# kdu3613/Multimodal_GAR

Hardware: AMD Instinct MI355X
Metric: clips/sec (fwd+bwd) at 32 actors x 16k pts x 15 frames (higher is better)
Workload: dtype f32; 1 GPU; c3: 8 clips x 15 frames x 32 actors x 16384 pts, 720x1280 RGB, fp32 fwd+bwd+Adam, LiDAR route pointnet2, GAT on; global_clips=8, clips_per_gpu=8, parallelism=dp1, launch=hip_graph, geometry=in step, gradient_exchange=none, trainable_params=29692332

## Files before the change

include/mgar_ops.h:

```cpp
#ifndef MGAR_OPS_H
#define MGAR_OPS_H

#ifdef __cplusplus
extern "C" {
#endif

#define MGAR_OK 0
#define MGAR_EINVAL (-1)
#define MGAR_ELAUNCH (-2)
#define MGAR_EUNSUPPORTED (-3)

#define MGAR_MAX_NSAMPLE 128

int mgar_abi_version(void);
const char *mgar_last_error(void);

int mgar_ktimer_enable(int on);
int mgar_ktimer_count(void);
const char *mgar_ktimer_name(int id);
int mgar_ktimer_read(int id, double *total_ms, long long *launches, double *total_bytes, double *total_flops,
                     int reset);
int mgar_ktimer_add_flops(int id, double flops);
int mgar_ktimer_add_bytes(int id, double bytes);


int mgar_ball_query_batch(int b, int n, int m, float radius, int nsample,
                          const float *new_xyz, const float *xyz, int *idx, void *stream);

int mgar_ball_query_multi_batch(int b, int n, int m, int nr, const float *radii, const int *nsamples,
                                const float *new_xyz, const float *xyz, int *const *idx, void *stream);
int mgar_ball_query_multi_stack(int B, int M, int nr, const float *radii, const int *nsamples, const float *new_xyz,
                                const int *new_xyz_batch_cnt, const float *xyz, const int *xyz_batch_cnt,
                                int *const *idx, void *stream);

int mgar_group_points_batch(int b, int c, int n, int npoints, int nsample,
                            const float *points, const int *idx, float *out, void *stream);
int mgar_group_points_grad_batch(int b, int c, int n, int npoints, int nsample,
                                 const float *grad_out, const int *idx, float *grad_points, void *stream);

int mgar_gather_points_batch(int b, int c, int n, int npoints,
                             const float *points, const int *idx, float *out, void *stream);
int mgar_gather_points_grad_batch(int b, int c, int n, int npoints,
                                  const float *grad_out, const int *idx, float *grad_points, void *stream);

int mgar_fps_batch(int b, int n, int m, const float *points, float *temp, int *idx, void *stream);

int mgar_morton_codes(int b, int n, const float *points, int *codes, void *stream);
int mgar_fps_batch_perm(int b, int n, int m, const float *points, float *temp, const int *perm, int *idx,
                        void *stream);
long long mgar_fps_batch_buckets_workspace_floats(int b, int n);
int mgar_fps_batch_buckets(int b, int n, int m, const float *points, float *temp, const int *perm, float *workspace, int *idx,
                           void *stream);

long long mgar_point_grid_workspace_bytes(int B, long long n_total);
int mgar_point_grid_build(int B, int n_batch, long long n_total, const float *xyz, const int *xyz_batch_cnt, float cell,
                          void *workspace, void *stream);
int mgar_ball_query_grid_batch(int b, int n, int m, float radius, int nsample, const float *new_xyz, const void *grid, int *idx,
                               void *stream);
int mgar_ball_query_grid_stack(int B, int M, long long n_total, float radius, int nsample, const float *new_xyz,
                               const int *new_xyz_batch_cnt, const void *grid, int *idx, void *stream);
int mgar_three_nn_grid_batch(int b, int n, int m, const float *unknown, const void *grid, float *dist2, int *idx, void *stream);
int mgar_three_nn_grid_stack(int B, int N, long long m_total, const float *unknown, const int *unknown_batch_cnt, const void *grid,
                             float *dist2, int *idx, void *stream);

int mgar_three_nn_batch(int b, int n, int m, const float *unknown, const float *known,
                        float *dist2, int *idx, void *stream);

int mgar_three_interpolate_batch(int b, int c, int m, int n, const float *points, const int *idx,
                                 const float *weight, float *out, void *stream);
int mgar_three_interpolate_grad_batch(int b, int c, int n, int m, const float *grad_out, const int *idx,
                                      const float *weight, float *grad_points, void *stream);

int mgar_three_interpolate_grad_sorted_batch(int b, int c, int n, int m, const float *grad_out, const int *list,
                                             float *grad_points, void *stream);
int mgar_three_interpolate_batch_into(int b, int c, int m, int n, const float *points, const int *idx, const float *weight,
                                      float *out, long long out_bstride, void *stream);
int mgar_three_interpolate_batch_add(int b, int c, int m, int n, const float *points, const int *idx, const float *weight,
                                     float *out, void *stream);
int mgar_three_interpolate_grad_batch_strided(int b, int c, int n, int m, const float *grad_out, long long grad_out_bstride,
                                              const int *idx, const float *weight, float *grad_points, void *stream);
int mgar_three_interpolate_grad_sorted_batch_strided(int b, int c, int n, int m, const float *grad_out,
                                                     long long grad_out_bstride, const int *list, float *grad_points,
                                                     void *stream);


int mgar_ball_query_stack(int B, int M, float radius, int nsample,
                          const float *new_xyz, const int *new_xyz_batch_cnt,
                          const float *xyz, const int *xyz_batch_cnt, int *idx, void *stream);

int mgar_voxel_query_stack(int M, int R1, int R2, int R3, int nsample, float radius,
                           int z_range, int y_range, int x_range,
                           const float *new_xyz, const float *xyz, const int *new_coords,
                           const int *point_indices, int *idx, void *stream);

int mgar_voxel_query_hash_stack(int M, int R1, int R2, int R3, int nsample, float radius,
                                int z_range, int y_range, int x_range,
                                const float *new_xyz, const float *xyz, const int *new_coords,
                                const long long *table_keys, const int *table_vals, int capacity, int *idx,
                                void *stream);

int mgar_fps_stack(int batch_size, int N, const float *points, float *temp, const int *xyz_batch_cnt,
                   int *idx, const int *num_sampled_points, void *stream);

int mgar_group_points_stack(int B, int M, int C, int nsample, const float *features,
                            const int *features_batch_cnt, const int *idx, const int *idx_batch_cnt,
                            float *out, void *stream);
int mgar_group_points_grad_stack(int B, int M, int C, int N, int nsample, const float *grad_out,
                                 const int *idx, const int *idx_batch_cnt, const int *features_batch_cnt,
                                 float *grad_features, void *stream);

int mgar_three_nn_stack(int batch_size, int N, int M, const float *unknown, const int *unknown_batch_cnt,
                        const float *known, const int *known_batch_cnt, float *dist2, int *idx, void *stream);

int mgar_three_interpolate_stack(int N, int C, const float *features, const int *idx, const float *weight,
                                 float *out, void *stream);
int mgar_three_interpolate_grad_stack(int N, int C, const float *grad_out, const int *idx, const float *weight,
                                      float *grad_features, void *stream);


int mgar_query_group_batch_fwd(int b, int c, int n, int npoints, int nsample, const float *xyz,
                               const float *new_xyz, const float *features, const int *idx, float *out,
                               void *stream);
int mgar_query_group_batch_bwd(int b, int c, int n, int npoints, int nsample, const float *grad_out,
                               const int *idx, float *grad_features, void *stream);

int mgar_query_group_stack_fwd(int B, int M, int C, int nsample, const float *xyz, const int *xyz_batch_cnt,
                               const float *new_xyz, const int *new_xyz_batch_cnt, const float *features,
                               const int *idx, float *out, void *stream);
int mgar_query_group_stack_bwd(int B, int M, int C, int nsample, const float *grad_out, const int *idx,
                               const int *new_xyz_batch_cnt, const int *xyz_batch_cnt, float *grad_features,
                               void *stream);

int mgar_query_group_proj_batch_fwd(int b, int c, int n, int npoints, int nsample, const float *xyz,
                                    const float *new_xyz, const float *zf, const float *wx, const int *idx,
                                    float *rel_out, float *y_out, void *stream);
int mgar_query_group_proj_batch_bwd(int b, int c, int n, int npoints, int nsample, const float *grad_y,
                                    const int *idx, float *grad_zf, void *stream);
int mgar_query_group_proj_stack_fwd(int B, int M, int C, int nsample, const float *xyz, const int *xyz_batch_cnt,
                                    const float *new_xyz, const int *new_xyz_batch_cnt, const float *zf, int zf_ld,
                                    const float *wx, const int *idx, float *rel_out, float *y_out, void *stream);
int mgar_query_group_proj_stack_fwd_stats(int B, int M, int C, int nsample, const float *xyz, const int *xyz_batch_cnt,
                                          const float *new_xyz, const int *new_xyz_batch_cnt, const float *zf, int zf_ld,
                                          const float *wx, const int *idx, float *rel_out, float *y_out, float *out_stats,
                                          void *stream);
int mgar_query_group_proj_stack_bwd(int B, int M, int C, int nsample, const float *grad_y, const int *idx,
                                    const int *new_xyz_batch_cnt, const int *xyz_batch_cnt, float *grad_zf,
                                    int zf_ld, void *stream);
long long mgar_query_group_stack_inverse_items(int B, int N, long long total);
long long mgar_query_group_stack_inverse_workspace_ints(int B, int N, long long total);
int mgar_query_group_stack_inverse_index(int B, int M, int nsample, int N, const int *idx, const int *new_xyz_batch_cnt,
                                         const int *xyz_batch_cnt, int *workspace, int *list, int *items, int *row_item,
                                         void *stream);
int mgar_query_group_stack_bwd_rows(int n_items, int N, int C, int nsample, const int *workspace, const int *items,
                                    const int *row_item, const int *list, const float *g_t, const float *xyz,
                                    const float *new_xyz, float *grad_zf, int zf_ld, float *part_rows, float *wx_part,
                                    long long total, void *stream);

int mgar_rowmajor_dw_workspace_floats(long long N, int Co, int Ci);
int mgar_rowmajor_dw(const float *a, int lda, const float *f, int ldf, long long N, int Co, int Ci,
                     float *workspace, float *dw, void *stream);


int mgar_bn_workspace_floats(int B, int C, int P);
int mgar_bn_train_stats(const float *x, int B, int C, int P, float eps, float momentum, float *workspace,
                        float *mean, float *invstd, float *running_mean, float *running_var,
                        long long *num_batches_tracked, void *stream);
int mgar_bn_train_stats_grouped(const float *x, int G, int C, int P, float eps, float momentum, float *workspace,
                                float *mean, float *invstd, float *running_mean, float *running_var,
                                long long *num_batches_tracked, void *stream);
int mgar_bn_act_fwd_grouped(const float *x, int G, int C, int P, const float *mean, const float *invstd,
                            const float *gamma, const float *beta, int relu, float *y, void *stream);
int mgar_bn_act_fwd(const float *x, int B, int C, int P, const float *mean, const float *invstd,
                    const float *gamma, const float *beta, int relu, float *y, void *stream);
long long mgar_bn_cl_workspace_floats(int S, int R, int C, int per_sample);
int mgar_bn_cl_train_stats(const float *x, int S, int R, int C, int per_sample, float eps, float momentum, float *workspace,
                           float *mean, float *invstd, float *running_mean, float *running_var,
                           long long *num_batches_tracked, void *stream);
int mgar_bn_cl_act_fwd(const float *x, int S, int R, int C, int per_sample, const float *mean, const float *invstd,
                       const float *gamma, const float *beta, int relu, float *y, int ldy, void *stream);
long long mgar_bn_rows_bwd_workspace_floats(int rows, int C);
int mgar_bn_rows_bwd(const float *dy, const float *x, int rows, int C, const float *mean, const float *invstd, const float *gamma,
                     const float *beta, int relu, float *workspace, float *dgamma, float *dbeta, float *dx, void *stream);
int mgar_bn_act_fwd_to_cl(const float *x, int S, int C, int R, int per_sample, const float *mean, const float *invstd,
                          const float *gamma, const float *beta, int relu, float *y, int ldy, void *stream);
int mgar_maxpool3d_same_fwd_cl(const float *x, int N, int T, int H, int W, int C, int kt, int kh, int kw, int st, int sh, int sw,
                               float *y, void *stream);
int mgar_bn_act_small(const float *x, int B, int C, int P, int per_sample, float eps, float momentum, const float *gamma,
                      const float *beta, int relu, float *workspace, float *mean, float *invstd, float *running_mean,
                      float *running_var, long long *num_batches_tracked, float *y, long long y_bstride, void *stream);
int mgar_bn_act_fwd_into(const float *x, int B, int C, int P, const float *mean, const float *invstd, const float *gamma,
                         const float *beta, int relu, int stats_per_sample, float *y, long long y_bstride, void *stream);
int mgar_bn_act_maxpool_fwd(const float *x, int B, int C, int M, int nsample, const float *mean,
                            const float *invstd, const float *gamma, const float *beta, int relu, float *out,
                            unsigned char *arg, float *xarg, void *stream);
int mgar_bn_act_bwd(const float *dy, const float *x, int B, int C, int P, const float *mean, const float *invstd,
                    const float *gamma, const float *beta, int relu, float *workspace, float *dgamma,
                    float *dbeta, float *dx, void *stream);
long long mgar_bn_stats_from_partials_workspace_floats(int nchunk, int C);
int mgar_bn_stats_from_partials(const float *partial, int nchunk, int C, long long n, int chunk, float eps, float momentum,
                                float *workspace, float *mean, float *invstd, float *running_mean, float *running_var,
                                long long *num_batches_tracked, void *stream);
int mgar_bn_act_maxpool_bwd_strided(const float *dpool, long long sb, long long sc, long long sm, const float *pooled,
                                    const unsigned char *arg, const float *x, const float *xarg, int B, int C, int M,
                                    int nsample, const float *mean, const float *invstd, const float *gamma, int relu,
                                    float *workspace, float *dgamma, float *dbeta, float *dx, void *stream);
int mgar_bn_act_bwd_apply(const float *dy, const float *x, int B, int C, int P, const float *mean, const float *invstd,
                          const float *gamma, const float *beta, int relu, const float *coef, int rowmajor, float *dx,
                          void *stream);
int mgar_bn_act_bwd_rowmajor(const float *dy, const float *x, int B, int C, int P, const float *mean, const float *invstd,
                             const float *gamma, const float *beta, int relu, float *workspace, float *dgamma,
                             float *dbeta, float *dx_t, void *stream);
int mgar_bn_act_maxpool_bwd(const float *dpool, const float *pooled, const unsigned char *arg, const float *x,
                            const float *xarg, int B, int C, int M, int nsample, const float *mean, const float *invstd,
                            const float *gamma, int relu, float *workspace, float *dgamma, float *dbeta,
                            float *dx, void *stream);

int mgar_pointwise_dw_workspace_floats(int B, int Cin, int Cout, int P);
int mgar_pointwise_conv_dw(const float *x, const float *dy, int B, int Cin, int Cout, int P, float *workspace,
                           float *dw, void *stream);

int mgar_pointwise_conv_dw_act(const float *x, const float *dy, int B, int Cin, int Cout, int P,
                               const float *in_mean, const float *in_invstd, const float *in_gamma,
                               const float *in_beta, int in_relu, float *workspace, float *dw, void *stream);

int mgar_pointwise_conv_fwd(const float *x, int B, int Cin, int P, const float *w, int w_row_stride,
                            int w_col_stride, int Cout, const float *in_mean, const float *in_invstd,
                            const float *in_gamma, const float *in_beta, int in_relu, float *y, void *stream);
int mgar_pointwise_dw_bnbwd_workspace_floats(int B, int Cin, int Cout, int P);
int mgar_pointwise_conv_dw_bnbwd(const float *x, const float *dy, const float *w, int B, int Cin, int Cout, int P,
                                 const float *in_mean, const float *in_invstd, const float *in_gamma, const float *in_beta,
                                 int in_relu, float *workspace, float *dw, float *dgamma, float *dbeta, float *coef, void *stream);
int mgar_pointwise_conv_fwd_stats(const float *x, int B, int Cin, int P, const float *w, int w_row_stride, int w_col_stride,
                                  int Cout, const float *in_mean, const float *in_invstd, const float *in_gamma,
                                  const float *in_beta, int in_relu, float *y, float *out_stats, void *stream);

int mgar_maxpool3d_same_fwd(const float *x, int NC, int T, int H, int W, int kt, int kh, int kw, int st, int sh,
                            int sw, float *y, void *stream);
int mgar_maxpool3d_valid_fwd(const float *x, int NC, int T, int H, int W, int kt, int kh, int kw, int st, int sh, int sw, float *y,
                             void *stream);

int mgar_stem_conv3d_workspace_floats(void);
int mgar_stem_conv3d_fwd(const float *x, int N, int T, int H, int W, const float *w, float *w_packed, float *y,
                         void *stream);
int mgar_stem_conv3d_set_minimal_filtering(int on);

long long mgar_conv3d_k3_workspace_floats(int Cin, int Cout);
int mgar_conv3d_k3_set_lds_pad(int bytes);
int mgar_conv3d_k3_fwd(const float *x, int N, int Cin, int D, int H, int W, const float *w, int Cout, float *w_packed, float *y,
                       void *stream);

int mgar_delay_us(int us, void *stream);


int mgar_roi_align_fwd(const float *input, int N, int C, int H, int W, const float *rois, int K,
                       int pooled_h, int pooled_w, float spatial_scale, int sampling_ratio, int aligned,
                       float *out, void *stream);
int mgar_roi_align_bwd(const float *grad_out, int N, int C, int H, int W, const float *rois, int K,
                       int pooled_h, int pooled_w, float spatial_scale, int sampling_ratio, int aligned,
                       float *grad_input, void *stream);

#define MGAR_DAFM_MAX_N 128
int mgar_dafm_attn_fwd(int S, int total_rows, int D, const int *scene_off, const int *de_off, const float *q, const float *k,
                       const float *v, const float *de, float sigma, float scale, float *att, float *out,
                       void *stream);
int mgar_dafm_attn_bwd(int S, int total_rows, int D, const int *scene_off, const int *de_off, const float *q, const float *k,
                       const float *v, const float *de, float sigma, float scale, const float *att,
                       const float *grad_out, float *gmat, float *grad_q, float *grad_k, float *grad_v,
                       void *stream);

int mgar_gatv2_fwd(int n_nodes, int H, int C, const int *rowptr, const int *col, const float *xl,
                   const float *xr, const float *att, float slope, const float *edge_scale, float *alpha,
                   float *out, void *stream);
int mgar_gatv2_bwd(int n_nodes, int H, int C, const int *rowptr, const int *col, const int *src_rowptr, const int *src_edge,
                   const int *src_dst, const float *xl, const float *xr, const float *att, float slope, const float *edge_scale,
                   const float *alpha, const float *grad_out, float *workspace, float *grad_xl, float *grad_xr, float *grad_att,
                   void *stream);
long long mgar_gatv2_bwd_workspace_floats(int n_nodes, int H, int C, int n_edges);

long long mgar_voxel_roi_pool_stats_workspace_doubles(int M, int nsample);
long long mgar_voxel_roi_pool_bwd_workspace_floats(int M, int C);
int mgar_voxel_roi_pool_stats(int M, int nsample, int C, const float *xyz, const float *new_xyz, const int *idx,
                              const float *w_pos, float eps, float momentum, double *workspace, double *moments,
                              float *mean, float *invstd, float *running_mean, float *running_var,
                              long long *num_batches_tracked, void *stream);
int mgar_voxel_roi_pool_fwd(int M, int nsample, int C, const float *xyz, const float *new_xyz, const float *feats,
                            int ld_f, const int *idx, const float *w_pos, const float *mean, const float *invstd,
                            const float *gamma, const float *beta, float *pooled, unsigned char *arg, void *stream);
int mgar_voxel_roi_pool_bwd(int M, int nsample, int C, const float *xyz, const float *new_xyz, const int *idx,
                            const float *w_pos, const float *mean, const float *invstd, const float *gamma,
                            const double *moments, int train_stats, const float *dpooled, const float *pooled,
                            const unsigned char *arg, float *workspace, float *dfeats, int ld_f, float *dgamma,
                            float *dbeta, float *dw_pos, void *stream);

int mgar_voxel_hash_build(int N, const int *coords, int Z, int Y, int X, long long *table_keys, int *table_vals,
                          int capacity, void *stream);
int mgar_voxel_hash_lookup(int M, const int *coords, int Z, int Y, int X, const long long *table_keys,
                           const int *table_vals, int capacity, int *rows, void *stream);
int mgar_spconv_rulebook(int n_sites, const int *site_coords, const int *geom, const long long *table_keys,
                         const int *table_vals, int capacity, int inverse, int *nbr, void *stream);
int mgar_spconv_output_keys(int n_in, const int *in_coords, const int *geom, long long *keys, void *stream);
int mgar_spconv_gather_gemm(int No, int K, int Cin, int Cout, const float *in, const int *nbr, const float *w,
                            int flip_k, float *out, void *stream);
int mgar_spconv_dw_chunks(int No);
int mgar_spconv_set_register_gather(int on);
int mgar_spconv_pair_chunk(void);
int mgar_spconv_pairs_blocks(int No);
int mgar_spconv_pairs_count(int No, int K, const int *nbr, int *blk, int *total, void *stream);
int mgar_spconv_pairs_fill(int No, int K, const int *nbr, const int *blk, const long long *offset_start, int *pair_i, int *pair_o,
                           void *stream);
int mgar_spconv_pairs_gemm(int K, int Cs, int Cd, const float *src, const int *pair_src, const int *pair_dst, const int *items,
                           const int *item_start_host, const float *w, float *dst, void *stream);
int mgar_spconv_pairs_dw(int n_items, int K, int Cin, int Cout, const float *in, const float *dout, const int *pair_i,
                         const int *pair_o, const int *items, const int *item_start, float *partial, float *dw, void *stream);
int mgar_spconv_dw(int No, int K, int Cin, int Cout, const float *in, const int *nbr, const float *dout,
                   float *partial, void *stream);

int mgar_points_in_boxes(int batch_size, int boxes_num, int pts_num, const float *boxes, const float *pts,
                         int *box_idx_of_points, void *stream);
int mgar_roipoint_pool3d_fwd(int batch_size, int pts_num, int boxes_num, int feature_in_len, int sampled_pts_num,
                             const float *xyz, const float *boxes3d, const float *pts_feature, float *pooled_features,
                             int *pooled_empty_flag, void *stream);

int mgar_image_resample_ksize(int in_size, int out_size);
int mgar_image_resample_coeffs(int in_size, int out_size, int *bounds, int *kk);
int mgar_image_resize_normalize_u8(int frames, int in_h, int in_w, int out_h, int out_w, const unsigned char *src,
                                   const int *xbounds, const int *xkk, const int *ybounds, const int *ykk, const float *lut,
                                   void *dst, long long dst_frame_stride, long long dst_channel_stride, int dst_kind,
                                   void *stream);
long long mgar_velodyne_merge_crop_workspace_ints(int n_upper, int n_lower);
int mgar_velodyne_merge_crop(int n_upper, int n_lower, int C, const float *upper, const float *lower, const float *tf_upper,
                             const float *tf_lower, const float *xy_range, int *workspace, float *out, int *count,
                             void *stream);

int mgar_query_group_batch_fwd_bf16(int b, int c, int n, int npoints, int nsample, const float *xyz, const float *new_xyz,
                                    const void *features, const int *idx, void *out, void *stream);
int mgar_query_group_stack_fwd_bf16(int B, int M, int C, int nsample, const float *xyz, const int *xyz_batch_cnt,
                                    const float *new_xyz, const int *new_xyz_batch_cnt, const void *features,
                                    const int *idx, void *out, void *stream);
int mgar_query_group_proj_batch_fwd_bf16(int b, int c, int n, int npoints, int nsample, const float *xyz,
                                         const float *new_xyz, const void *zf, const float *wx, const int *idx,
                                         void *rel_out, void *y_out, void *stream);
int mgar_query_group_proj_stack_fwd_bf16(int B, int M, int C, int nsample, const float *xyz, const int *xyz_batch_cnt,
                                         const float *new_xyz, const int *new_xyz_batch_cnt, const void *zf, int zf_ld,
                                         const float *wx, const int *idx, void *rel_out, void *y_out, void *stream);
int mgar_bn_train_stats_bf16(const void *x, int B, int C, int P, float eps, float momentum, float *workspace,
                             float *mean, float *invstd, float *running_mean, float *running_var,
                             long long *num_batches_tracked, void *stream);
int mgar_bn_train_stats_grouped_bf16(const void *x, int G, int C, int P, float eps, float momentum, float *workspace,
                                     float *mean, float *invstd, float *running_mean, float *running_var,
                                     long long *num_batches_tracked, void *stream);
int mgar_bn_act_fwd_bf16(const void *x, int B, int C, int P, const float *mean, const float *invstd,
                         const float *gamma, const float *beta, int relu, void *y, void *stream);
int mgar_three_interpolate_batch_into_bf16(int b, int c, int m, int n, const void *points, const int *idx, const float *weight,
                                           void *out, long long out_bstride, void *stream);
int mgar_three_interpolate_batch_add_bf16(int b, int c, int m, int n, const void *points, const int *idx, const float *weight,
                                          void *out, void *stream);
int mgar_bn_cl_train_stats_bf16(const void *x, int S, int R, int C, int per_sample, float eps, float momentum, float *workspace,
                                float *mean, float *invstd, float *running_mean, float *running_var,
                                long long *num_batches_tracked, void *stream);
int mgar_bn_cl_act_fwd_bf16(const void *x, int S, int R, int C, int per_sample, const float *mean, const float *invstd,
                            const float *gamma, const float *beta, int relu, void *y, int ldy, void *stream);
int mgar_bn_act_fwd_to_cl_bf16(const void *x, int S, int C, int R, int per_sample, const float *mean, const float *invstd,
                               const float *gamma, const float *beta, int relu, void *y, int ldy, void *stream);
int mgar_maxpool3d_same_fwd_cl_bf16(const void *x, int N, int T, int H, int W, int C, int kt, int kh, int kw, int st, int sh,
                                    int sw, void *y, void *stream);
int mgar_bn_act_small_bf16(const void *x, int B, int C, int P, int per_sample, float eps, float momentum, const float *gamma,
                           const float *beta, int relu, float *workspace, float *mean, float *invstd, float *running_mean,
                           float *running_var, long long *num_batches_tracked, void *y, long long y_bstride, void *stream);
int mgar_bn_act_fwd_into_bf16(const void *x, int B, int C, int P, const float *mean, const float *invstd, const float *gamma,
                              const float *beta, int relu, int stats_per_sample, void *y, long long y_bstride, void *stream);
int mgar_bn_act_fwd_grouped_bf16(const void *x, int G, int C, int P, const float *mean, const float *invstd,
                                 const float *gamma, const float *beta, int relu, void *y, void *stream);
int mgar_bn_act_maxpool_fwd_bf16(const void *x, int B, int C, int M, int nsample, const float *mean,
                                 const float *invstd, const float *gamma, const float *beta, int relu, void *out,
                                 unsigned char *arg, void *xarg, void *stream);
int mgar_bn_act_bwd_bf16(const void *dy, const void *x, int B, int C, int P, const float *mean, const float *invstd,
                         const float *gamma, const float *beta, int relu, float *workspace, float *dgamma,
                         float *dbeta, void *dx, void *stream);
int mgar_bn_act_maxpool_bwd_bf16(const void *dpool, const void *pooled, const unsigned char *arg, const void *x,
                                 const void *xarg, int B, int C, int M, int nsample, const float *mean, const float *invstd,
                                 const float *gamma, int relu, float *workspace, float *dgamma, float *dbeta,
                                 void *dx, void *stream);
int mgar_pointwise_conv_fwd_bf16(const void *x, int B, int Cin, int P, const float *w, int w_row_stride,
                                 int w_col_stride, int Cout, const float *in_mean, const float *in_invstd,
                                 const float *in_gamma, const float *in_beta, int in_relu, void *y, void *stream);
int mgar_three_interpolate_batch_bf16(int b, int c, int m, int n, const void *points, const int *idx,
                                      const float *weight, void *out, void *stream);
int mgar_three_interpolate_stack_bf16(int N, int C, const void *features, const int *idx, const float *weight,
                                      void *out, void *stream);
int mgar_maxpool3d_same_fwd_bf16(const void *x, int NC, int T, int H, int W, int kt, int kh, int kw, int st, int sh,
                                 int sw, void *y, void *stream);
int mgar_maxpool3d_valid_fwd_bf16(const void *x, int NC, int T, int H, int W, int kt, int kh, int kw, int st, int sh, int sw, void *y,
                                  void *stream);
int mgar_roi_align_fwd_bf16(const void *input, int N, int C, int H, int W, const float *rois, int K,
                            int pooled_h, int pooled_w, float spatial_scale, int sampling_ratio, int aligned,
                            void *out, void *stream);
int mgar_stem_conv3d_fwd_bf16(const void *x, int N, int T, int H, int W, const float *w, float *w_packed, void *y,
                              void *stream);
int mgar_voxel_roi_pool_fwd_bf16(int M, int nsample, int C, const float *xyz, const float *new_xyz, const void *feats,
                                 int ld_f, const int *idx, const float *w_pos, const float *mean, const float *invstd,
                                 const float *gamma, const float *beta, void *pooled, unsigned char *arg, void *stream);

#ifdef __cplusplus
}
#endif
#endif
```

multimodal_gar_amd/_lib.py:

```python
import ctypes
import os

import torch

_HERE = os.path.dirname(os.path.abspath(__file__))
LIB_PATH = os.path.join(_HERE, "csrc", "libmgar_hip.so")
ABI_VERSION = 12

if not os.path.exists(LIB_PATH):
    raise ImportError(
        "multimodal_gar_amd: %s is missing -- build it with `python -m multimodal_gar_amd.build` "
        "(hipcc --offload-arch=gfx950). There is no CPU fallback." % LIB_PATH)

_cdll = ctypes.CDLL(LIB_PATH)

_I, _F, _P, _LL = ctypes.c_int, ctypes.c_float, ctypes.c_void_p, ctypes.c_longlong

_PROTOS = {
    "mgar_ball_query_batch": [_I, _I, _I, _F, _I, _P, _P, _P, _P],
    "mgar_group_points_batch": [_I, _I, _I, _I, _I, _P, _P, _P, _P],
    "mgar_group_points_grad_batch": [_I, _I, _I, _I, _I, _P, _P, _P, _P],
    "mgar_gather_points_batch": [_I, _I, _I, _I, _P, _P, _P, _P],
    "mgar_gather_points_grad_batch": [_I, _I, _I, _I, _P, _P, _P, _P],
    "mgar_ball_query_multi_batch": [_I, _I, _I, _I, _P, _P, _P, _P, _P, _P],
    "mgar_ball_query_multi_stack": [_I, _I, _I, _P, _P, _P, _P, _P, _P, _P, _P],
    "mgar_fps_batch": [_I, _I, _I, _P, _P, _P, _P],
    "mgar_morton_codes": [_I, _I, _P, _P, _P],
    "mgar_fps_batch_perm": [_I, _I, _I, _P, _P, _P, _P, _P],
    "mgar_point_grid_workspace_bytes": [_I, ctypes.c_longlong],
    "mgar_point_grid_build": [_I, _I, ctypes.c_longlong, _P, _P, _F, _P, _P],
    "mgar_ball_query_grid_batch": [_I, _I, _I, _F, _I, _P, _P, _P, _P],
    "mgar_ball_query_grid_stack": [_I, _I, ctypes.c_longlong, _F, _I, _P, _P, _P, _P, _P],
    "mgar_three_nn_grid_batch": [_I, _I, _I, _P, _P, _P, _P, _P],
    "mgar_three_nn_grid_stack": [_I, _I, ctypes.c_longlong, _P, _P, _P, _P, _P, _P],
    "mgar_fps_batch_buckets": [_I, _I, _I, _P, _P, _P, _P, _P, _P],
    "mgar_fps_batch_buckets_workspace_floats": [_I, _I],
    "mgar_three_nn_batch": [_I, _I, _I, _P, _P, _P, _P, _P],
    "mgar_three_interpolate_batch": [_I, _I, _I, _I, _P, _P, _P, _P, _P],
    "mgar_three_interpolate_batch_add": [_I, _I, _I, _I, _P, _P, _P, _P, _P],
    "mgar_three_interpolate_grad_batch": [_I, _I, _I, _I, _P, _P, _P, _P, _P],
    "mgar_three_interpolate_grad_sorted_batch": [_I, _I, _I, _I, _P, _P, _P, _P],
    "mgar_three_interpolate_batch_into": [_I, _I, _I, _I, _P, _P, _P, _P, _LL, _P],
    "mgar_three_interpolate_grad_batch_strided": [_I, _I, _I, _I, _P, _LL, _P, _P, _P, _P],
    "mgar_three_interpolate_grad_sorted_batch_strided": [_I, _I, _I, _I, _P, _LL, _P, _P, _P],
    "mgar_ball_query_stack": [_I, _I, _F, _I, _P, _P, _P, _P, _P, _P],
    "mgar_voxel_query_stack": [_I, _I, _I, _I, _I, _F, _I, _I, _I, _P, _P, _P, _P, _P, _P],
    "mgar_voxel_query_hash_stack": [_I, _I, _I, _I, _I, _F, _I, _I, _I, _P, _P, _P, _P, _P, _I, _P, _P],
    "mgar_fps_stack": [_I, _I, _P, _P, _P, _P, _P, _P],
    "mgar_group_points_stack": [_I, _I, _I, _I, _P, _P, _P, _P, _P, _P],
    "mgar_group_points_grad_stack": [_I, _I, _I, _I, _I, _P, _P, _P, _P, _P, _P],
    "mgar_three_nn_stack": [_I, _I, _I, _P, _P, _P, _P, _P, _P, _P],
    "mgar_three_interpolate_stack": [_I, _I, _P, _P, _P, _P, _P],
    "mgar_three_interpolate_grad_stack": [_I, _I, _P, _P, _P, _P, _P],
    "mgar_query_group_batch_fwd": [_I, _I, _I, _I, _I, _P, _P, _P, _P, _P, _P],
    "mgar_query_group_batch_bwd": [_I, _I, _I, _I, _I, _P, _P, _P, _P],
    "mgar_query_group_stack_fwd": [_I, _I, _I, _I, _P, _P, _P, _P, _P, _P, _P, _P],
    "mgar_query_group_stack_bwd": [_I, _I, _I, _I, _P, _P, _P, _P, _P, _P],
    "mgar_query_group_proj_batch_fwd": [_I, _I, _I, _I, _I, _P, _P, _P, _P, _P, _P, _P, _P],
    "mgar_query_group_proj_batch_bwd": [_I, _I, _I, _I, _I, _P, _P, _P, _P],
    "mgar_query_group_proj_stack_fwd": [_I, _I, _I, _I, _P, _P, _P, _P, _P, _I, _P, _P, _P, _P, _P],
    "mgar_query_group_proj_stack_bwd": [_I, _I, _I, _I, _P, _P, _P, _P, _P, _I, _P],
    "mgar_rowmajor_dw_workspace_floats": [_LL, _I, _I],
    "mgar_ktimer_enable": [_I],
    "mgar_ktimer_count": [],
    "mgar_ktimer_add_flops": [_I, ctypes.c_double],
    "mgar_ktimer_add_bytes": [_I, ctypes.c_double],
    "mgar_ktimer_read": [_I, _P, _P, _P, _P, _I],
    "mgar_rowmajor_dw": [_P, _I, _P, _I, _LL, _I, _I, _P, _P, _P],
    "mgar_bn_workspace_floats": [_I, _I, _I],
    "mgar_bn_train_stats": [_P, _I, _I, _I, _F, _F, _P, _P, _P, _P, _P, _P, _P],
    "mgar_bn_train_stats_grouped": [_P, _I, _I, _I, _F, _F, _P, _P, _P, _P, _P, _P, _P],
    "mgar_bn_act_fwd_grouped": [_P, _I, _I, _I, _P, _P, _P, _P, _I, _P, _P],
    "mgar_bn_act_fwd": [_P, _I, _I, _I, _P, _P, _P, _P, _I, _P, _P],
    "mgar_bn_act_maxpool_fwd": [_P, _I, _I, _I, _I, _P, _P, _P, _P, _I, _P, _P, _P, _P],
    "mgar_bn_act_bwd": [_P, _P, _I, _I, _I, _P, _P, _P, _P, _I, _P, _P, _P, _P, _P],
    "mgar_bn_stats_from_partials_workspace_floats": [_I, _I],
    "mgar_bn_stats_from_partials": [_P, _I, _I, _LL, _I, _F, _F, _P, _P, _P, _P, _P, _P, _P],
    "mgar_pointwise_conv_fwd_stats": [_P, _I, _I, _I, _P, _I, _I, _I, _P, _P, _P, _P, _I, _P, _P, _P],
    "mgar_query_group_proj_stack_fwd_stats": [_I, _I, _I, _I, _P, _P, _P, _P, _P, _I, _P, _P, _P, _P, _P, _P],
    "mgar_bn_act_maxpool_bwd_strided": [_P, _LL, _LL, _LL, _P, _P, _P, _P, _I, _I, _I, _I, _P, _P, _P, _I, _P, _P, _P, _P, _P],
    "mgar_bn_cl_workspace_floats": [_I, _I, _I, _I],
    "mgar_bn_cl_train_stats": [_P, _I, _I, _I, _I, _F, _F, _P, _P, _P, _P, _P, _P, _P],
    "mgar_bn_cl_act_fwd": [_P, _I, _I, _I, _I, _P, _P, _P, _P, _I, _P, _I, _P],
    "mgar_bn_rows_bwd_workspace_floats": [_I, _I],
    "mgar_bn_rows_bwd": [_P, _P, _I, _I, _P, _P, _P, _P, _I, _P, _P, _P, _P, _P],
    "mgar_bn_act_fwd_to_cl": [_P, _I, _I, _I, _I, _P, _P, _P, _P, _I, _P, _I, _P],
    "mgar_maxpool3d_same_fwd_cl": [_P, _I, _I, _I, _I, _I, _I, _I, _I, _I, _I, _I, _P, _P],
    "mgar_bn_act_small": [_P, _I, _I, _I, _I, _F, _F, _P, _P, _I, _P, _P, _P, _P, _P, _P, _P, _LL, _P],
    "mgar_bn_act_fwd_into": [_P, _I, _I, _I, _P, _P, _P, _P, _I, _I, _P, _LL, _P],
    "mgar_bn_act_bwd_rowmajor": [_P, _P, _I, _I, _I, _P, _P, _P, _P, _I, _P, _P, _P, _P, _P],
    "mgar_query_group_stack_inverse_items": [_I, _I, _LL],
    "mgar_query_group_stack_inverse_workspace_ints": [_I, _I, _LL],
    "mgar_query_group_stack_inverse_index": [_I, _I, _I, _I, _P, _P, _P, _P, _P, _P, _P, _P],
    "mgar_query_group_stack_bwd_rows": [_I, _I, _I, _I, _P, _P, _P, _P, _P, _P, _P, _P, _I, _P, _P, _LL, _P],
    "mgar_bn_act_maxpool_bwd": [_P, _P, _P, _P, _P, _I, _I, _I, _I, _P, _P, _P, _I, _P, _P, _P, _P, _P],
    "mgar_pointwise_conv_dw": [_P, _P, _I, _I, _I, _I, _P, _P, _P],
    "mgar_pointwise_dw_workspace_floats": [_I, _I, _I, _I],
    "mgar_pointwise_dw_bnbwd_workspace_floats": [_I, _I, _I, _I],
    "mgar_pointwise_conv_dw_bnbwd": [_P, _P, _P, _I, _I, _I, _I, _P, _P, _P, _P, _I, _P, _P, _P, _P, _P, _P],
    "mgar_bn_act_bwd_apply": [_P, _P, _I, _I, _I, _P, _P, _P, _P, _I, _P, _I, _P, _P],
    "mgar_pointwise_conv_dw_act": [_P, _P, _I, _I, _I, _I, _P, _P, _P, _P, _I, _P, _P, _P],
    "mgar_pointwise_conv_fwd": [_P, _I, _I, _I, _P, _I, _I, _I, _P, _P, _P, _P, _I, _P, _P],
    "mgar_stem_conv3d_workspace_floats": [],
    "mgar_stem_conv3d_set_minimal_filtering": [_I],
    "mgar_stem_conv3d_fwd": [_P, _I, _I, _I, _I, _P, _P, _P, _P],
    "mgar_delay_us": [_I, _P],
    "mgar_conv3d_k3_workspace_floats": [_I, _I],
    "mgar_conv3d_k3_set_lds_pad": [_I],
    "mgar_conv3d_k3_fwd": [_P, _I, _I, _I, _I, _I, _P, _I, _P, _P, _P],
    "mgar_maxpool3d_same_fwd": [_P, _I, _I, _I, _I, _I, _I, _I, _I, _I, _I, _P, _P],
    "mgar_maxpool3d_valid_fwd": [_P, _I, _I, _I, _I, _I, _I, _I, _I, _I, _I, _P, _P],
    "mgar_roi_align_fwd": [_P, _I, _I, _I, _I, _P, _I, _I, _I, _F, _I, _I, _P, _P],
    "mgar_roi_align_bwd": [_P, _I, _I, _I, _I, _P, _I, _I, _I, _F, _I, _I, _P, _P],
    "mgar_dafm_attn_fwd": [_I, _I, _I, _P, _P, _P, _P, _P, _P, _F, _F, _P, _P, _P],
    "mgar_dafm_attn_bwd": [_I, _I, _I, _P, _P, _P, _P, _P, _P, _F, _F, _P, _P, _P, _P, _P, _P, _P],
    "mgar_gatv2_fwd": [_I, _I, _I, _P, _P, _P, _P, _P, _F, _P, _P, _P, _P],
    "mgar_gatv2_bwd": [_I, _I, _I, _P, _P, _P, _P, _P, _P, _P, _P, _F, _P, _P, _P, _P, _P, _P, _P, _P],
    "mgar_gatv2_bwd_workspace_floats": [_I, _I, _I, _I],
    "mgar_points_in_boxes": [_I, _I, _I, _P, _P, _P, _P],
    "mgar_roipoint_pool3d_fwd": [_I, _I, _I, _I, _I, _P, _P, _P, _P, _P, _P],
    "mgar_image_resample_ksize": [_I, _I],
    "mgar_image_resample_coeffs": [_I, _I, _P, _P],
    "mgar_image_resize_normalize_u8": [_I, _I, _I, _I, _I, _P, _P, _P, _P, _P, _P, _P, _LL, _LL, _I, _P],
    "mgar_velodyne_merge_crop_workspace_ints": [_I, _I],
    "mgar_velodyne_merge_crop": [_I, _I, _I, _P, _P, _P, _P, _P, _P, _P, _P, _P],
    "mgar_voxel_hash_build": [_I, _P, _I, _I, _I, _P, _P, _I, _P],
    "mgar_voxel_hash_lookup": [_I, _P, _I, _I, _I, _P, _P, _I, _P, _P],
    "mgar_spconv_rulebook": [_I, _P, _P, _P, _P, _I, _I, _P, _P],
    "mgar_spconv_output_keys": [_I, _P, _P, _P, _P],
    "mgar_spconv_gather_gemm": [_I, _I, _I, _I, _P, _P, _P, _I, _P, _P],
    "mgar_spconv_dw_chunks": [_I],
    "mgar_spconv_pair_chunk": [],
    "mgar_spconv_set_register_gather": [_I],
    "mgar_spconv_pairs_blocks": [_I],
    "mgar_spconv_pairs_count": [_I, _I, _P, _P, _P, _P],
    "mgar_spconv_pairs_fill": [_I, _I, _P, _P, _P, _P, _P, _P],
    "mgar_spconv_pairs_gemm": [_I, _I, _I, _P, _P, _P, _P, _P, _P, _P, _P],
    "mgar_spconv_pairs_dw": [_I, _I, _I, _I, _P, _P, _P, _P, _P, _P, _P, _P, _P],
    "mgar_spconv_dw": [_I, _I, _I, _I, _P, _P, _P, _P, _P],
    "mgar_voxel_roi_pool_stats_workspace_doubles": [_I, _I],
    "mgar_voxel_roi_pool_bwd_workspace_floats": [_I, _I],
    "mgar_voxel_roi_pool_stats": [_I, _I, _I, _P, _P, _P, _P, _F, _F, _P, _P, _P, _P, _P, _P, _P, _P],
    "mgar_voxel_roi_pool_fwd": [_I, _I, _I, _P, _P, _P, _I, _P, _P, _P, _P, _P, _P, _P, _P, _P],
    "mgar_voxel_roi_pool_bwd": [_I, _I, _I, _P, _P, _P, _P, _P, _P, _P, _P, _I, _P, _P, _P, _P, _P, _I, _P, _P, _P, _P],
}
for _n in ("mgar_query_group_batch_fwd", "mgar_query_group_stack_fwd", "mgar_query_group_proj_batch_fwd",
           "mgar_query_group_proj_stack_fwd", "mgar_bn_train_stats", "mgar_bn_train_stats_grouped", "mgar_bn_act_fwd",
           "mgar_bn_act_fwd_grouped", "mgar_bn_act_fwd_into", "mgar_bn_act_small", "mgar_bn_cl_train_stats", "mgar_bn_cl_act_fwd", "mgar_bn_act_fwd_to_cl",
           "mgar_maxpool3d_same_fwd_cl", "mgar_bn_act_maxpool_fwd", "mgar_bn_act_bwd", "mgar_bn_act_maxpool_bwd",
           "mgar_pointwise_conv_fwd", "mgar_three_interpolate_batch", "mgar_three_interpolate_batch_into", "mgar_three_interpolate_batch_add", "mgar_three_interpolate_stack",
           "mgar_maxpool3d_same_fwd", "mgar_maxpool3d_valid_fwd", "mgar_roi_align_fwd", "mgar_voxel_roi_pool_fwd", "mgar_stem_conv3d_fwd"):
    _PROTOS[_n + "_bf16"] = _PROTOS[_n]
BF16_TWINS = frozenset(n[:-5] for n in _PROTOS if n.endswith("_bf16"))

_LONGLONG_RESULTS = frozenset((
    "mgar_query_group_stack_inverse_items", "mgar_query_group_stack_inverse_workspace_ints", "mgar_bn_cl_workspace_floats",
    "mgar_bn_stats_from_partials_workspace_floats", "mgar_voxel_roi_pool_stats_workspace_doubles",
    "mgar_voxel_roi_pool_bwd_workspace_floats", "mgar_velodyne_merge_crop_workspace_ints", "mgar_gatv2_bwd_workspace_floats",
    "mgar_fps_batch_buckets_workspace_floats", "mgar_point_grid_workspace_bytes",
    "mgar_bn_rows_bwd_workspace_floats", "mgar_conv3d_k3_workspace_floats"))

_fns = {}
for _name, _args in _PROTOS.items():
    _fn = getattr(_cdll, _name)
    _fn.argtypes = _args
    _fn.restype = ctypes.c_longlong if _name in _LONGLONG_RESULTS else ctypes.c_int
    _fns[_name] = _fn

_cdll.mgar_abi_version.restype = ctypes.c_int
_cdll.mgar_last_error.restype = ctypes.c_char_p
if _cdll.mgar_abi_version() != ABI_VERSION:
    raise ImportError("libmgar_hip.so ABI %d != expected %d: rebuild" % (_cdll.mgar_abi_version(), ABI_VERSION))


class MgarError(RuntimeError):
    pass


def dev_ptr(t, dtype=None):
    if t is None:
        return None
    if not t.is_cuda:
        raise MgarError("expected a device (HIP) tensor, got %s -- there is no CPU path" % t.device)
    if not t.is_contiguous():
        raise MgarError("tensor must be contiguous")
    if dtype is not None and t.dtype != dtype:
        raise MgarError("expected dtype %s, got %s" % (dtype, t.dtype))
    return t.data_ptr()


def fptr(t):
    return dev_ptr(t, torch.float32)


def pptr(t, dtype):
    return dev_ptr(t, dtype)


def payload_call(name, dtype, *args):
    if dtype == torch.float32:
        return call(name, *args)
    if dtype == torch.bfloat16 and name in BF16_TWINS:
        return call(name + "_bf16", *args)
    raise MgarError("%s: unsupported payload dtype %s" % (name, dtype))


def iptr(t):
    return dev_ptr(t, torch.int32)


def stream_of(t):
    return torch.cuda.current_stream(t.device).cuda_stream


def raw(name, *args):
    return _fns[name](*args)


def call(name, *args):
    rc = _fns[name](*args)
    if rc != 0:
        raise MgarError("%s failed with code %d: %s" % (name, rc, _cdll.mgar_last_error().decode()))
    return rc


def host_arrays(radii, nsamples, idx_tensors):
    n = len(radii)
    fa = (ctypes.c_float * n)(*[float(r) for r in radii])
    ia = (ctypes.c_int * n)(*[int(s) for s in nsamples])
    pa = (ctypes.c_void_p * n)(*[iptr(t) for t in idx_tensors])
    return fa, ia, pa


def kernel_timers(enable=None, reset=True):
    if enable is not None:
        call("mgar_ktimer_enable", int(bool(enable)))
        _KT_STATE["on"] = bool(enable)
        return None
    _cdll.mgar_ktimer_name.restype = ctypes.c_char_p
    _cdll.mgar_ktimer_name.argtypes = [ctypes.c_int]
    out = {}
    for i in range(raw("mgar_ktimer_count")):
        ms, by, fl, n = ctypes.c_double(), ctypes.c_double(), ctypes.c_double(), ctypes.c_longlong()
        call("mgar_ktimer_read", i, ctypes.byref(ms), ctypes.byref(n), ctypes.byref(by), ctypes.byref(fl), int(reset))
        if n.value:
            out[_cdll.mgar_ktimer_name(i).decode()] = (ms.value, n.value, by.value, fl.value)
    return out


_KT_IDS = {}


_KT_STATE = {"on": False}


def note_work(kernel, flops=0.0, nbytes=0.0):
    if not _KT_STATE["on"]:
        return
    if not _KT_IDS:
        _cdll.mgar_ktimer_name.restype = ctypes.c_char_p
        _cdll.mgar_ktimer_name.argtypes = [ctypes.c_int]
        for i in range(raw("mgar_ktimer_count")):
            _KT_IDS[_cdll.mgar_ktimer_name(i).decode()] = i
    if flops:
        call("mgar_ktimer_add_flops", _KT_IDS[kernel], float(flops))
    if nbytes:
        call("mgar_ktimer_add_bytes", _KT_IDS[kernel], float(nbytes))


def kernel_timing_on():
    return _KT_STATE["on"]


def note_pair_tests(kernel, pairs):
    note_work(kernel, flops=float(pairs) * 8.0)


def exported_symbols():
    return sorted(_PROTOS) + ["mgar_abi_version", "mgar_last_error", "mgar_ktimer_name"]
```

multimodal_gar_amd/bn_ops.py:

```python
import torch
import torch.nn as nn
from torch.autograd import Function
from torch.autograd.function import once_differentiable

from . import _lib as L


def _u8ptr(t):
    return L.dev_ptr(t, torch.uint8)


def _workspace(x, b, c, p):
    return torch.empty((L.raw("mgar_bn_workspace_floats", b, c, p),), dtype=torch.float32, device=x.device)


_PAYLOADS = (torch.float32, torch.bfloat16)


def _f32(t):
    return t if t is None or t.dtype == torch.float32 else t.float()


STATS_TILE = 128


def stats_partial_buffer(x_like, c, n_per_channel):
    if x_like.dtype != torch.float32 or not x_like.is_cuda or n_per_channel % STATS_TILE != 0 or n_per_channel == 0:
        return None
    return torch.empty((c, n_per_channel // STATS_TILE, 2), dtype=torch.float32, device=x_like.device)


def _train_stats(x3, bn, partial=None):
    b, c, p = x3.shape
    mean = torch.empty((c,), dtype=torch.float32, device=x3.device)
    invstd = torch.empty_like(mean)
    track = bn.track_running_stats and bn.running_mean is not None
    if partial is not None and tuple(partial.shape) == (c, (b * p) // STATS_TILE, 2) and (b * p) % STATS_TILE == 0:
        nws = L.raw("mgar_bn_stats_from_partials_workspace_floats", partial.shape[1], c)
        ws = torch.empty((nws,), dtype=torch.float32, device=x3.device) if nws else None
        L.call("mgar_bn_stats_from_partials", L.fptr(partial), partial.shape[1], c, b * p, STATS_TILE, float(bn.eps),
               float(bn.momentum if bn.momentum is not None else 0.1), L.fptr(ws) if ws is not None else None, L.fptr(mean), L.fptr(invstd),
               L.fptr(bn.running_mean) if track else None, L.fptr(bn.running_var) if track else None,
               L.dev_ptr(bn.num_batches_tracked, torch.int64) if track and bn.num_batches_tracked is not None else None,
               L.stream_of(x3))
        return mean, invstd
    ws = _workspace(x3, b, c, p)
    L.payload_call("mgar_bn_train_stats", x3.dtype, L.pptr(x3, x3.dtype), b, c, p, float(bn.eps),
                   float(bn.momentum if bn.momentum is not None else 0.1),
                   L.fptr(ws), L.fptr(mean), L.fptr(invstd), L.fptr(bn.running_mean) if track else None,
                   L.fptr(bn.running_var) if track else None,
                   L.dev_ptr(bn.num_batches_tracked, torch.int64) if track and bn.num_batches_tracked is not None else None,
                   L.stream_of(x3))
    return mean, invstd


ROWMAJOR_GRAD_MAX_CHANNELS = 64


def _bwd_rowmajor(dy, x3, mean, invstd, gamma, beta, relu, ws, dgamma, dbeta):
    b, c, p = x3.shape
    dx_t = torch.empty((b, p, c), dtype=torch.float32, device=x3.device)
    L.call("mgar_bn_act_bwd_rowmajor", L.fptr(dy), L.fptr(x3), b, c, p, L.fptr(mean), L.fptr(invstd), L.fptr(gamma), L.fptr(beta),
           int(relu), L.fptr(ws), L.fptr(dgamma), L.fptr(dbeta), L.fptr(dx_t), L.stream_of(x3))
    return dx_t.permute(0, 2, 1)


class _BnAct(Function):

    @staticmethod
    def forward(ctx, x3, gamma, beta, mean, invstd, relu, rowmajor_grad=False):
        b, c, p = x3.shape
        ctx.rowmajor = bool(rowmajor_grad) and x3.dtype == torch.float32 and c <= ROWMAJOR_GRAD_MAX_CHANNELS
        y = torch.empty_like(x3)
        dt = x3.dtype
        L.payload_call("mgar_bn_act_fwd", dt, L.pptr(x3, dt), b, c, p, L.fptr(mean), L.fptr(invstd), L.fptr(gamma), L.fptr(beta),
                       int(relu), L.pptr(y, dt), L.stream_of(x3))
        ctx.save_for_backward(x3, gamma, beta, mean, invstd)
        ctx.relu = bool(relu)
        return y

    @staticmethod
    @once_differentiable
    def backward(ctx, dy):
        x3, gamma, beta, mean, invstd = ctx.saved_tensors
        b, c, p = x3.shape
        dgamma, dbeta = torch.empty_like(gamma), torch.empty_like(beta)
        dt = x3.dtype
        dy_c, ws = dy.contiguous().to(dt), _workspace(x3, b, c, p)
        if ctx.rowmajor:
            return _bwd_rowmajor(dy_c, x3, mean, invstd, gamma, beta, ctx.relu, ws, dgamma, dbeta), dgamma, dbeta, None, None, None, None
        dx = torch.empty_like(x3)
        L.payload_call("mgar_bn_act_bwd", dt, L.pptr(dy_c, dt), L.pptr(x3, dt), b, c, p, L.fptr(mean), L.fptr(invstd), L.fptr(gamma),
                       L.fptr(beta), int(ctx.relu), L.fptr(ws), L.fptr(dgamma), L.fptr(dbeta), L.pptr(dx, dt), L.stream_of(x3))
        return dx, dgamma, dbeta, None, None, None, None


class _BnActMaxPool(Function):

    @staticmethod
    def forward(ctx, x4, gamma, beta, mean, invstd, relu):
        b, c, m, ns = x4.shape
        dt = x4.dtype
        out = torch.empty((b, c, m), dtype=dt, device=x4.device)
        arg = torch.empty((b, c, m), dtype=torch.uint8, device=x4.device)
        xarg = torch.empty((b, c, m), dtype=dt, device=x4.device) if x4.requires_grad or gamma.requires_grad else None
        L.payload_call("mgar_bn_act_maxpool_fwd", dt, L.pptr(x4, dt), b, c, m, ns, L.fptr(mean), L.fptr(invstd), L.fptr(gamma),
                       L.fptr(beta), int(relu), L.pptr(out, dt), _u8ptr(arg), L.pptr(xarg, dt) if xarg is not None else None,
                       L.stream_of(x4))
        ctx.save_for_backward(x4, gamma, mean, invstd, out, arg, xarg)
        ctx.relu = bool(relu)
        ctx.mark_non_differentiable(arg)
        return out, arg

    @staticmethod
    @once_differentiable
    def backward(ctx, dpool, darg=None):
        x4, gamma, mean, invstd, out, arg, xarg = ctx.saved_tensors
        b, c, m, ns = x4.shape
        dx = torch.empty_like(x4)
        dgamma, dbeta = torch.empty_like(gamma), torch.empty_like(gamma)
        dt = x4.dtype
        ws = _workspace(x4, b, c, m * ns)
        if dt == torch.float32 and dpool.dtype == dt and dpool.dim() == 3 and not dpool.is_contiguous() \
                and (b == 1 or dpool.stride(0) >= 0) and min(dpool.stride(1), dpool.stride(2)) >= 1:
            L.call("mgar_bn_act_maxpool_bwd_strided", dpool.data_ptr(), dpool.stride(0) if b > 1 else 0, dpool.stride(1), dpool.stride(2),
                   L.fptr(out), _u8ptr(arg), L.fptr(x4), L.fptr(xarg) if xarg is not None else None, b, c, m, ns, L.fptr(mean),
                   L.fptr(invstd), L.fptr(gamma), int(ctx.relu), L.fptr(ws), L.fptr(dgamma), L.fptr(dbeta), L.fptr(dx), L.stream_of(x4))
            return dx, dgamma, dbeta, None, None, None
        dpool_c = dpool.contiguous().to(dt)
        L.payload_call("mgar_bn_act_maxpool_bwd", dt, L.pptr(dpool_c, dt), L.pptr(out, dt), _u8ptr(arg), L.pptr(x4, dt),
                       L.pptr(xarg, dt) if xarg is not None else None, b, c, m, ns, L.fptr(mean), L.fptr(invstd), L.fptr(gamma),
                       int(ctx.relu), L.fptr(ws), L.fptr(dgamma), L.fptr(dbeta), L.pptr(dx, dt), L.stream_of(x4))
        return dx, dgamma, dbeta, None, None, None


class _BnActConv(Function):

    @staticmethod
    def forward(ctx, x3, gamma, beta, mean, invstd, relu, w, rowmajor_grad=False, out_stats=None):
        b, c, p = x3.shape
        ctx.rowmajor = bool(rowmajor_grad) and x3.dtype == torch.float32 and c <= ROWMAJOR_GRAD_MAX_CHANNELS
        cout = w.shape[0]
        w = w.contiguous()
        dt = x3.dtype
        y = torch.empty((b, cout, p), dtype=dt, device=x3.device)
        if out_stats is not None:
            L.call("mgar_pointwise_conv_fwd_stats", L.fptr(x3), b, c, p, L.fptr(w), c, 1, cout, L.fptr(mean), L.fptr(invstd),
                   L.fptr(gamma), L.fptr(beta), int(relu), L.fptr(y), L.fptr(out_stats), L.stream_of(x3))
        else:
            L.payload_call("mgar_pointwise_conv_fwd", dt, L.pptr(x3, dt), b, c, p, L.fptr(w), c, 1, cout, L.fptr(mean), L.fptr(invstd),
                           L.fptr(gamma), L.fptr(beta), int(relu), L.pptr(y, dt), L.stream_of(x3))
        ctx.save_for_backward(x3, gamma, beta, mean, invstd, w)
        ctx.relu = relu
        return y

    @staticmethod
    @once_differentiable
    def backward(ctx, gy):
        x3, gamma, beta, mean, invstd, w = ctx.saved_tensors
        b, c, p = x3.shape
        cout = w.shape[0]
        gy = gy.contiguous()
        st = L.stream_of(x3)
        ga = torch.empty_like(x3)
        L.call("mgar_pointwise_conv_fwd", L.fptr(gy), b, cout, p, L.fptr(w), 1, c, c, None, None, None, None, 0,
               L.fptr(ga), st)
        dgamma, dbeta = torch.empty_like(gamma), torch.empty_like(gamma)
        if FUSED_DW_BN_REDUCE and ctx.needs_input_grad[6]:
            dw = torch.empty_like(w)
            coef = torch.empty((2 * c,), dtype=torch.float32, device=x3.device)
            wsd = torch.empty((max(1, L.raw("mgar_pointwise_dw_bnbwd_workspace_floats", b, c, cout, p)),), dtype=torch.float32,
                              device=x3.device)
            L.call("mgar_pointwise_conv_dw_bnbwd", L.fptr(x3), L.fptr(gy), L.fptr(w), b, c, cout, p, L.fptr(mean), L.fptr(invstd),
                   L.fptr(gamma), L.fptr(beta), int(ctx.relu), L.fptr(wsd), L.fptr(dw), L.fptr(dgamma), L.fptr(dbeta), L.fptr(coef), st)
            dx = torch.empty((b, p, c) if ctx.rowmajor else (b, c, p), dtype=torch.float32, device=x3.device)
            L.call("mgar_bn_act_bwd_apply", L.fptr(ga), L.fptr(x3), b, c, p, L.fptr(mean), L.fptr(invstd), L.fptr(gamma), L.fptr(beta),
                   int(ctx.relu), L.fptr(coef), int(ctx.rowmajor), L.fptr(dx), st)
            return (dx.permute(0, 2, 1) if ctx.rowmajor else dx), dgamma, dbeta, None, None, None, dw, None, None
        dw = None
        if ctx.needs_input_grad[6]:
            dw = torch.empty_like(w)
            wsd = torch.empty((max(1, L.raw("mgar_pointwise_dw_workspace_floats", b, c, cout, p)),), dtype=torch.float32,
                              device=x3.device)
            L.call("mgar_pointwise_conv_dw_act", L.fptr(x3), L.fptr(gy), b, c, cout, p, L.fptr(mean), L.fptr(invstd),
                   L.fptr(gamma), L.fptr(beta), int(ctx.relu), L.fptr(wsd), L.fptr(dw), st)
        ws = _workspace(x3, b, c, p)
        if ctx.rowmajor:
            return _bwd_rowmajor(ga, x3, mean, invstd, gamma, beta, ctx.relu, ws, dgamma, dbeta), dgamma, dbeta, None, None, None, dw, None, None
        dx = torch.empty_like(x3)
        L.call("mgar_bn_act_bwd", L.fptr(ga), L.fptr(x3), b, c, p, L.fptr(mean), L.fptr(invstd), L.fptr(gamma),
               L.fptr(beta), int(ctx.relu), L.fptr(ws), L.fptr(dgamma), L.fptr(dbeta), L.fptr(dx), st)
        return dx, dgamma, dbeta, None, None, None, dw, None, None


class _PlainConv(Function):

    @staticmethod
    def forward(ctx, x3, w, out_stats=None):
        b, c, p = x3.shape
        cout = w.shape[0]
        w = w.contiguous()
        dt = x3.dtype
        y = torch.empty((b, cout, p), dtype=dt, device=x3.device)
        if out_stats is not None:
            L.call("mgar_pointwise_conv_fwd_stats", L.fptr(x3), b, c, p, L.fptr(w), c, 1, cout, None, None, None, None, 0,
                   L.fptr(y), L.fptr(out_stats), L.stream_of(x3))
        else:
            L.payload_call("mgar_pointwise_conv_fwd", dt, L.pptr(x3, dt), b, c, p, L.fptr(w), c, 1, cout, None, None, None, None, 0,
                           L.pptr(y, dt), L.stream_of(x3))
        ctx.save_for_backward(x3, w)
        return y

    @staticmethod
    @once_differentiable
    def backward(ctx, gy):
        x3, w = ctx.saved_tensors
        b, c, p = x3.shape
        cout = w.shape[0]
        gy = gy.contiguous()
        dx = dw = None
        if ctx.needs_input_grad[0]:
            dx = torch.empty_like(x3)
            L.call("mgar_pointwise_conv_fwd", L.fptr(gy), b, cout, p, L.fptr(w), 1, c, c, None, None, None, None, 0, L.fptr(dx),
                   L.stream_of(x3))
        if ctx.needs_input_grad[1]:
            dw = torch.empty_like(w)
            wsd = torch.empty((max(1, L.raw("mgar_pointwise_dw_workspace_floats", b, c, cout, p)),), dtype=torch.float32,
                              device=x3.device)
            L.call("mgar_pointwise_conv_dw", L.fptr(x3), L.fptr(gy), b, c, cout, p, L.fptr(wsd), L.fptr(dw), L.stream_of(x3))
        return dx, dw, None


PLAIN_CONV_MAX_OUT = 32
PLAIN_CONV_MAX_IN = 32


def plain_conv(x, conv, want_out_stats=False):
    if not (x.is_cuda and x.dtype in _PAYLOADS and x.dim() >= 3 and conv.bias is None):
        return None
    if x.dtype != torch.float32 and torch.is_grad_enabled() and (x.requires_grad or conv.weight.requires_grad):
        return None
    c, cout = x.shape[1], conv.out_channels
    x3 = x.contiguous().flatten(2)
    if c > PLAIN_CONV_MAX_IN or cout > PLAIN_CONV_MAX_OUT or x3.shape[2] % 4 != 0 or x3.shape[0] * x3.shape[2] < (1 << 16):
        return None
    out_stats = stats_partial_buffer(x3, cout, x3.shape[0] * x3.shape[2]) if want_out_stats and x3.shape[2] % STATS_TILE == 0 else None
    y = _PlainConv.apply(x3, _f32(conv.weight).view(cout, c), out_stats).view(x.shape[0], cout, *x.shape[2:])
    return (y, out_stats) if want_out_stats else y


FUSED_DW_BN_REDUCE = False
FUSED_CONV_MAX_CHANNELS = 64


FUSED_STATS_MAX_CHANNELS = 32


def bn_act_conv(x, bn, relu, conv, rowmajor_grad=False, in_stats=None, want_out_stats=False):
    if not (x.is_cuda and x.dtype in _PAYLOADS and bn.training and x.dim() >= 3 and conv.bias is None):
        return None
    if x.dtype != torch.float32 and torch.is_grad_enabled() and (x.requires_grad or conv.weight.requires_grad):
        return None
    c, cout = x.shape[1], conv.out_channels
    x3 = x.contiguous().flatten(2)
    if c > FUSED_CONV_MAX_CHANNELS or cout > FUSED_CONV_MAX_CHANNELS or x3.shape[2] % 4 != 0 \
            or x3.shape[0] * x3.shape[2] < (1 << 16):
        return None
    mean, invstd = _stats(x3, bn, in_stats)
    gamma, beta = _affine(bn, c, x.device)
    out_stats = stats_partial_buffer(x3, cout, x3.shape[0] * x3.shape[2]) \
        if want_out_stats and cout <= FUSED_STATS_MAX_CHANNELS and x3.shape[2] % STATS_TILE == 0 else None
    y = _BnActConv.apply(x3, gamma, beta, mean, invstd, relu, _f32(conv.weight).view(cout, c), rowmajor_grad, out_stats)
    y = y.view(x.shape[0], cout, *x.shape[2:])
    return (y, out_stats) if want_out_stats else y


def _affine(bn, c, device):
    if bn.affine:
        return _f32(bn.weight), _f32(bn.bias)
    return torch.ones(c, device=device), torch.zeros(c, device=device)


def _stats(x3, bn, partial=None):
    if bn.training or not bn.track_running_stats:
        return _train_stats(x3, bn, partial)
    return _f32(bn.running_mean), torch.rsqrt(_f32(bn.running_var) + bn.eps)


def _slice_stride(out, x):
    if out is None or out.shape != x.shape or out.dtype != x.dtype or not out.is_cuda:
        return None
    inner = 1
    for size, stride in zip(reversed(out.shape[1:]), reversed(out.stride()[1:])):
        if size != 1 and stride != inner:
            return None
        inner *= size
    return out.stride(0) if out.stride(0) >= inner else None


def is_channels_last_3d(x):
    return x.dim() == 5 and not x.is_contiguous() and x.is_contiguous(memory_format=torch.channels_last_3d)


def _cl_out_slice(out, x):
    if out is None or out.shape != x.shape or out.dtype != x.dtype or not out.is_cuda:
        return None
    n, c, t, h, w = out.shape
    ld = out.stride(4)
    ok = out.stride(1) == 1 and ld >= c and out.stride(3) == w * ld and out.stride(2) == h * w * ld and out.stride(0) == t * h * w * ld
    return ld if ok and ld % 4 == 0 and (out.data_ptr() // out.element_size()) % 4 == 0 else None


def _cl_stats(x, bn, per_sample):
    n, c, t, h, w = x.shape
    r = t * h * w
    rows = n * c if per_sample else c
    mean = torch.empty((rows,), dtype=torch.float32, device=x.device)
    invstd = torch.empty_like(mean)
    ws = torch.empty((max(L.raw("mgar_bn_cl_workspace_floats", n, r, c, int(per_sample)), 1),), dtype=torch.float32, device=x.device)
    track = bn.track_running_stats and bn.running_mean is not None
    L.payload_call("mgar_bn_cl_train_stats", x.dtype, x.data_ptr(), n, r, c, int(per_sample), float(bn.eps),
                   float(bn.momentum if bn.momentum is not None else 0.1), L.fptr(ws), L.fptr(mean), L.fptr(invstd),
                   L.fptr(bn.running_mean) if track else None, L.fptr(bn.running_var) if track else None,
                   L.dev_ptr(bn.num_batches_tracked, torch.int64) if track and bn.num_batches_tracked is not None else None,
                   L.stream_of(x))
    return mean, invstd


def bn_act_channels_last(x, bn, relu, per_sample, out=None):
    n, c, t, h, w = x.shape
    if c % 4 != 0 or c > 1024 or x.dtype not in _PAYLOADS or (per_sample and n * c > 65535) or not bn.training:
        return None
    mean, invstd = _cl_stats(x, bn, per_sample)
    gamma, beta = _affine(bn, c, x.device)
    ld = _cl_out_slice(out, x)
    y = out if ld is not None else torch.empty_like(x)
    L.payload_call("mgar_bn_cl_act_fwd", x.dtype, x.data_ptr(), n, t * h * w, c, int(per_sample), L.fptr(mean), L.fptr(invstd),
                   L.fptr(gamma), L.fptr(beta), int(relu), y.data_ptr(), ld if ld is not None else c, L.stream_of(x))
    return y


def bn_act_to_channels_last(x, bn, relu, per_sample):
    x = x.contiguous()
    n, c, t, h, w = x.shape
    if x.dtype not in _PAYLOADS or not bn.training or (per_sample and n * c > 65535):
        return None
    x3 = x.flatten(2)
    if per_sample:
        mean = torch.empty((n * c,), dtype=torch.float32, device=x.device)
        invstd = torch.empty_like(mean)
        track = bn.track_running_stats and bn.running_mean is not None
        ws = _workspace(x3, 1, n * c, x3.shape[2])
        L.payload_call("mgar_bn_train_stats_grouped", x.dtype, L.pptr(x3, x.dtype), n, c, x3.shape[2], float(bn.eps),
                       float(bn.momentum if bn.momentum is not None else 0.1), L.fptr(ws), L.fptr(mean), L.fptr(invstd),
                       L.fptr(bn.running_mean) if track else None, L.fptr(bn.running_var) if track else None,
                       L.dev_ptr(bn.num_batches_tracked, torch.int64) if track and bn.num_batches_tracked is not None else None,
                       L.stream_of(x))
    else:
        mean, invstd = _train_stats(x3, bn)
    gamma, beta = _affine(bn, c, x.device)
    y = torch.empty(x.shape, dtype=x.dtype, device=x.device, memory_format=torch.channels_last_3d)
    L.payload_call("mgar_bn_act_fwd_to_cl", x.dtype, L.pptr(x3, x.dtype), n, c, t * h * w, int(per_sample), L.fptr(mean), L.fptr(invstd),
                   L.fptr(gamma), L.fptr(beta), int(relu), y.data_ptr(), c, L.stream_of(x))
    return y


class _BnActRows(Function):

    @staticmethod
    def forward(ctx, x, gamma, beta, mean, invstd, relu):
        rows, c = x.shape
        y = torch.empty_like(x)
        L.call("mgar_bn_cl_act_fwd", L.fptr(x), 1, rows, c, 0, L.fptr(mean), L.fptr(invstd), L.fptr(gamma), L.fptr(beta), int(relu),
               L.fptr(y), c, L.stream_of(x))
        ctx.save_for_backward(x, gamma, beta, mean, invstd)
        ctx.relu = bool(relu)
        return y

    @staticmethod
    @once_differentiable
    def backward(ctx, dy):
        x, gamma, beta, mean, invstd = ctx.saved_tensors
        rows, c = x.shape
        dy = dy.contiguous()
        dx, dgamma, dbeta = torch.empty_like(x), torch.empty_like(gamma), torch.empty_like(gamma)
        ws = torch.empty((L.raw("mgar_bn_rows_bwd_workspace_floats", rows, c),), dtype=torch.float32, device=x.device)
        L.call("mgar_bn_rows_bwd", L.fptr(dy), L.fptr(x), rows, c, L.fptr(mean), L.fptr(invstd), L.fptr(gamma), L.fptr(beta),
               int(ctx.relu), L.fptr(ws), L.fptr(dgamma), L.fptr(dbeta), L.fptr(dx), L.stream_of(x))
        return dx, dgamma, dbeta, None, None, None


def bn_act_rows(x, bn, relu):
    if not (x.is_cuda and x.dim() == 2 and x.dtype == torch.float32 and bn.training and x.shape[1] % 4 == 0 and x.shape[1] <= 1024
            and x.shape[0] > 0):
        return None
    x = x.contiguous()
    rows, c = x.shape
    mean = torch.empty((c,), dtype=torch.float32, device=x.device)
    invstd = torch.empty_like(mean)
    ws = torch.empty((max(L.raw("mgar_bn_cl_workspace_floats", 1, rows, c, 0), 1),), dtype=torch.float32, device=x.device)
    track = bn.track_running_stats and bn.running_mean is not None
    L.call("mgar_bn_cl_train_stats", L.fptr(x), 1, rows, c, 0, float(bn.eps), float(bn.momentum if bn.momentum is not None else 0.1),
           L.fptr(ws), L.fptr(mean), L.fptr(invstd), L.fptr(bn.running_mean) if track else None, L.fptr(bn.running_var) if track else None,
           L.dev_ptr(bn.num_batches_tracked, torch.int64) if track and bn.num_batches_tracked is not None else None, L.stream_of(x))
    gamma, beta = _affine(bn, c, x.device)
    return _BnActRows.apply(x, gamma, beta, mean, invstd, relu)


SMALL_CHANNEL_MAX = 16384


def _small_fused(x, x3, bn, relu, per_sample, out):
    b, c, p = x3.shape
    if (p if per_sample else b * p) > SMALL_CHANNEL_MAX or p % 4 != 0 or x3.dtype not in _PAYLOADS:
        return None
    bstride = _slice_stride(out, x)
    y = out if bstride is not None else torch.empty_like(x)
    track = bn.track_running_stats and bn.running_mean is not None
    rows = b * c if per_sample else c
    need = per_sample and track
    mean = torch.empty((rows,), dtype=torch.float32, device=x.device) if need else None
    ws = torch.empty((rows,), dtype=torch.float32, device=x.device) if need else None
    gamma, beta = _affine(bn, c, x.device)
    dt = x3.dtype
    L.payload_call("mgar_bn_act_small", dt, L.pptr(x3, dt), b, c, p, int(per_sample), float(bn.eps),
                   float(bn.momentum if bn.momentum is not None else 0.1), L.fptr(gamma), L.fptr(beta), int(relu),
                   L.fptr(ws) if ws is not None else None, L.fptr(mean) if mean is not None else None, None,
                   L.fptr(bn.running_mean) if track else None, L.fptr(bn.running_var) if track else None,
                   L.dev_ptr(bn.num_batches_tracked, torch.int64) if track and bn.num_batches_tracked is not None else None,
                   y.data_ptr(), bstride if bstride is not None else -1, L.stream_of(x3))
    return y


def _apply_into(x3, bn, relu, mean, invstd, per_sample, out, bstride):
    b, c, p = x3.shape
    gamma, beta = _affine(bn, c, x3.device)
    dt = x3.dtype
    L.payload_call("mgar_bn_act_fwd_into", dt, L.pptr(x3, dt), b, c, p, L.fptr(mean), L.fptr(invstd), L.fptr(gamma), L.fptr(beta),
                   int(relu), int(per_sample), out.data_ptr(), bstride, L.stream_of(x3))
    return out


def bn_act(x, bn, relu, rowmajor_grad=False, out=None, in_stats=None, to_channels_last=False):
    if x.is_cuda and x.dim() == 5 and not (torch.is_grad_enabled() and (x.requires_grad or (bn.affine and bn.weight.requires_grad))):
        y = bn_act_channels_last(x, bn, relu, False, out) if is_channels_last_3d(x) else \
            (bn_act_to_channels_last(x, bn, relu, False) if to_channels_last else None)
        if y is not None:
            return y
    x3 = x.contiguous().flatten(2) if x.dim() > 2 else x.contiguous().unsqueeze(-1)
    if not bn.training and torch.is_grad_enabled() and x.requires_grad:
        return None
    forward_only = not (torch.is_grad_enabled() and (x.requires_grad or (bn.affine and bn.weight.requires_grad)))
    if forward_only and bn.training and x.is_cuda and in_stats is None:
        y = _small_fused(x, x3, bn, relu, False, out)
        if y is not None:
            return y
    mean, invstd = _stats(x3, bn, in_stats)
    bstride = _slice_stride(out, x)
    if bstride is not None and x.dtype in _PAYLOADS and not (torch.is_grad_enabled() and (x.requires_grad or bn.weight.requires_grad)):
        return _apply_into(x3, bn, relu, mean, invstd, False, out, bstride)
    gamma, beta = _affine(bn, x3.shape[1], x.device)
    return _BnAct.apply(x3, gamma, beta, mean, invstd, relu, rowmajor_grad).view(x.shape)


def bn_act_per_sample(x, bn, relu, out=None, to_channels_last=False):
    if not (x.is_cuda and x.dtype in _PAYLOADS and bn.training and x.dim() >= 3) or (torch.is_grad_enabled() and
                                                                                        (x.requires_grad or bn.weight.requires_grad)):
        return None
    if x.dim() == 5:
        y = bn_act_channels_last(x, bn, relu, True, out) if is_channels_last_3d(x) else \
            (bn_act_to_channels_last(x, bn, relu, True) if to_channels_last else None)
        if y is not None:
            return y
    x3 = x.contiguous().flatten(2)
    g, c, p = x3.shape
    if g * c > 65535:
        return None
    y = _small_fused(x, x3, bn, relu, True, out)
    if y is not None:
        return y
    mean = torch.empty((g * c,), dtype=torch.float32, device=x.device)
    invstd = torch.empty_like(mean)
    track = bn.track_running_stats and bn.running_mean is not None
    ws = _workspace(x3, 1, g * c, p)
    st = L.stream_of(x3)
    dt = x3.dtype
    L.payload_call("mgar_bn_train_stats_grouped", dt, L.pptr(x3, dt), g, c, p, float(bn.eps),
                   float(bn.momentum if bn.momentum is not None else 0.1),
                   L.fptr(ws), L.fptr(mean), L.fptr(invstd), L.fptr(bn.running_mean) if track else None,
                   L.fptr(bn.running_var) if track else None,
                   L.dev_ptr(bn.num_batches_tracked, torch.int64) if track and bn.num_batches_tracked is not None else None, st)
    bstride = _slice_stride(out, x)
    if bstride is not None:
        return _apply_into(x3, bn, relu, mean, invstd, True, out, bstride)
    gamma, beta = _affine(bn, c, x.device)
    y = torch.empty_like(x3)
    L.payload_call("mgar_bn_act_fwd_grouped", dt, L.pptr(x3, dt), g, c, p, L.fptr(mean), L.fptr(invstd), L.fptr(gamma), L.fptr(beta),
                   int(relu), L.pptr(y, dt), st)
    return y.view(x.shape)


def bn_train_stats_only(x, bn, per_sample=False):
    x3 = x.contiguous().flatten(2)
    g, c, p = x3.shape
    if not per_sample:
        return _train_stats(x3, bn)
    if g * c > 65535:
        return None
    mean = torch.empty((g * c,), dtype=torch.float32, device=x.device)
    invstd = torch.empty_like(mean)
    track = bn.track_running_stats and bn.running_mean is not None
    ws = _workspace(x3, 1, g * c, p)
    dt = x3.dtype
    L.payload_call("mgar_bn_train_stats_grouped", dt, L.pptr(x3, dt), g, c, p, float(bn.eps),
                   float(bn.momentum if bn.momentum is not None else 0.1),
                   L.fptr(ws), L.fptr(mean), L.fptr(invstd), L.fptr(bn.running_mean) if track else None,
                   L.fptr(bn.running_var) if track else None,
                   L.dev_ptr(bn.num_batches_tracked, torch.int64) if track and bn.num_batches_tracked is not None else None, L.stream_of(x3))
    return mean, invstd


def bn_apply_with_stats(x, bn, relu, stats, per_sample=False):
    mean, invstd = stats
    x3 = x.contiguous().flatten(2)
    g, c, p = x3.shape
    gamma, beta = _affine(bn, c, x.device)
    y = torch.empty_like(x3)
    dt = x3.dtype
    if per_sample:
        L.payload_call("mgar_bn_act_fwd_grouped", dt, L.pptr(x3, dt), g, c, p, L.fptr(mean), L.fptr(invstd), L.fptr(gamma), L.fptr(beta),
                       int(relu), L.pptr(y, dt), L.stream_of(x3))
    else:
        L.payload_call("mgar_bn_act_fwd", dt, L.pptr(x3, dt), g, c, p, L.fptr(mean), L.fptr(invstd), L.fptr(gamma), L.fptr(beta),
                       int(relu), L.pptr(y, dt), L.stream_of(x3))
    return y.view(x.shape)


def bn_act_maxpool(x, bn, relu, in_stats=None):
    x4 = x.contiguous()
    if x4.shape[-1] > 255 or (not bn.training and torch.is_grad_enabled() and x.requires_grad):
        return None
    mean, invstd = _stats(x4.flatten(2), bn, in_stats)
    gamma, beta = _affine(bn, x4.shape[1], x.device)
    return _BnActMaxPool.apply(x4, gamma, beta, mean, invstd, relu)[0]
```

multimodal_gar_amd/csrc/bn_act.hip:

```cpp
#include "common.hpp"
#include "payload.hpp"

namespace mgar {

constexpr int BN_THREADS = 256;
constexpr int BN_CHUNK = 65536;

__device__ __forceinline__ float block_sum(float v, float *scratch) {
    v = wave_sum(v);
    const int lane = threadIdx.x & 63, w = threadIdx.x >> 6;
    __syncthreads();
    if (lane == 0) scratch[w] = v;
    __syncthreads();
    float t = 0.f;
    for (int i = 0; i < BN_THREADS / 64; ++i) t += scratch[i];
    return t;
}

__device__ __forceinline__ size_t chan_off(long long e, int c, int C, int P) {
    const long long b = e / P;
    return ((size_t)b * C + c) * P + (size_t)(e - b * P);
}

template <typename T>
__global__ __launch_bounds__(BN_THREADS) void bn_partial_kernel(const T *__restrict__ x, int B, int C, int P, int chunk,
                                                                float *__restrict__ partial) {
    __shared__ float scratch[BN_THREADS / 64];
    const int c = blockIdx.y;
    const long long n = (long long)B * P;
    const long long e0 = (long long)blockIdx.x * chunk;
    const long long e1 = min(e0 + chunk, n);
    const long long npiv = min((long long)BN_THREADS, e1 - e0);
    float pv = threadIdx.x < npiv ? Payload<T>::ld(x + chan_off(e0 + threadIdx.x, c, C, P)) : 0.f;
    const float pivot = block_sum(pv, scratch) / (float)npiv;
    float s = 0.f, q = 0.f;
    if ((P & 3) == 0) {
#pragma unroll 4
        for (long long e = e0 + (long long)threadIdx.x * 4; e < e1; e += BN_THREADS * 4) {
            float4 v = Payload<T>::ld4(x + chan_off(e, c, C, P));
            v.x -= pivot; v.y -= pivot; v.z -= pivot; v.w -= pivot;
            s += (v.x + v.y) + (v.z + v.w);
            q += (v.x * v.x + v.y * v.y) + (v.z * v.z + v.w * v.w);
        }
    } else {
        for (long long e = e0 + threadIdx.x; e < e1; e += BN_THREADS) {
            const float v = Payload<T>::ld(x + chan_off(e, c, C, P)) - pivot;
            s += v;
            q += v * v;
        }
    }
    s = block_sum(s, scratch);
    q = block_sum(q, scratch);
    if (threadIdx.x == 0) {
        const double nk = (double)(e1 - e0), sd = (double)s;
        double m2 = (double)q - sd * sd / nk;
        if (m2 < 0.0) m2 = 0.0;
        partial[((size_t)c * gridDim.x + blockIdx.x) * 2 + 0] = (float)((double)pivot + sd / nk);
        partial[((size_t)c * gridDim.x + blockIdx.x) * 2 + 1] = (float)m2;
    }
}

__device__ __forceinline__ double wave_sum_f64(double v) {
#pragma unroll
    for (int d = 32; d >= 1; d >>= 1) v += __shfl_xor(v, d);
    return v;
}
__global__ __launch_bounds__(64) void bn_finalize_kernel(const float *__restrict__ partial, int nchunk, int C, double n, int chunk,
                                                         float eps, float momentum, float *__restrict__ mean,
                                                         float *__restrict__ invstd, float *__restrict__ running_mean,
                                                         float *__restrict__ running_var,
                                                         long long *__restrict__ num_batches_tracked,
                                                         float *__restrict__ var_out) {
    const int c = blockIdx.x;
    auto count = [&](int i) { return i + 1 < nchunk ? (double)chunk : n - (double)chunk * (nchunk - 1); };
    double s = 0.0;
    for (int i = threadIdx.x; i < nchunk; i += 64) s += count(i) * (double)partial[((size_t)c * nchunk + i) * 2 + 0];
    const double m = wave_sum_f64(s) / n;
    double q = 0.0;
    for (int i = threadIdx.x; i < nchunk; i += 64) {
        const double d = (double)partial[((size_t)c * nchunk + i) * 2 + 0] - m;
        q += (double)partial[((size_t)c * nchunk + i) * 2 + 1] + count(i) * d * d;
    }
    q = wave_sum_f64(q);
    if (threadIdx.x != 0) return;
    double var = q / n;
    if (var < 0.0) var = 0.0;
    mean[c] = (float)m;
    invstd[c] = (float)(1.0 / sqrt(var + (double)eps));
    if (var_out) var_out[c] = (float)var;
    if (running_mean) running_mean[c] = (1.f - momentum) * running_mean[c] + momentum * (float)m;
    if (running_var) running_var[c] = (1.f - momentum) * running_var[c] + momentum * (float)(n > 1.0 ? var * n / (n - 1.0) : var);
    if (num_batches_tracked && c == 0) *num_batches_tracked += 1;
}

constexpr int BN_SMALL_V = 16, BN_SMALL_MAX = BN_THREADS * 4 * BN_SMALL_V;
template <bool RELU, typename T>
__global__ __launch_bounds__(BN_THREADS) void bn_small_fused_kernel(const T *__restrict__ x, int B, int C, int P, int per_sample,
                                                                    float eps, float momentum, const float *__restrict__ gamma,
                                                                    const float *__restrict__ beta, float *__restrict__ mean_out,
                                                                    float *__restrict__ invstd_out, float *__restrict__ var_out,
                                                                    float *__restrict__ running_mean, float *__restrict__ running_var,
                                                                    long long *__restrict__ num_batches_tracked, T *__restrict__ y,
                                                                    long long y_bstride) {
    __shared__ float scratch[BN_THREADS / 64];
    const int row = blockIdx.x;
    const int c = per_sample ? row % C : row;
    const int nb = per_sample ? 1 : B;
    const long long n = (long long)nb * P;
    float4 v[BN_SMALL_V];
    float s = 0.f;
#pragma unroll
    for (int u = 0; u < BN_SMALL_V; ++u) {
        const long long e = ((long long)u * BN_THREADS + threadIdx.x) * 4;
        if (e < n) {
            const size_t o = per_sample ? (size_t)row * P + e : chan_off(e, c, C, P);
            v[u] = Payload<T>::ld4(x + o);
            s += (v[u].x + v[u].y) + (v[u].z + v[u].w);
        } else {
            v[u] = make_float4(0.f, 0.f, 0.f, 0.f);
        }
    }
    const float mu = block_sum(s, scratch) / (float)n;
    float q = 0.f;
#pragma unroll
    for (int u = 0; u < BN_SMALL_V; ++u) {
        const long long e = ((long long)u * BN_THREADS + threadIdx.x) * 4;
        if (e < n) {
            const float dx = v[u].x - mu, dy = v[u].y - mu, dz = v[u].z - mu, dw = v[u].w - mu;
            q += (dx * dx + dy * dy) + (dz * dz + dw * dw);
        }
    }
    __syncthreads();
    const float var = fmaxf(block_sum(q, scratch) / (float)n, 0.f);
    const float is = (float)(1.0 / sqrt((double)var + (double)eps));
    if (threadIdx.x == 0) {
        if (mean_out) mean_out[row] = mu;
        if (invstd_out) invstd_out[row] = is;
        if (var_out) var_out[row] = var;
        if (!per_sample) {
            if (running_mean) running_mean[c] = (1.f - momentum) * running_mean[c] + momentum * mu;
            if (running_var) running_var[c] = (1.f - momentum) * running_var[c] + momentum * (n > 1 ? var * (float)n / (float)(n - 1) : var);
            if (num_batches_tracked && c == 0) *num_batches_tracked += 1;
        }
    }
    const float sc = is * (gamma ? gamma[c] : 1.f), sh = beta ? beta[c] : 0.f;
#pragma unroll
    for (int u = 0; u < BN_SMALL_V; ++u) {
        const long long e = ((long long)u * BN_THREADS + threadIdx.x) * 4;
        if (e < n) {
            float4 r = v[u];
            r.x = (r.x - mu) * sc + sh; r.y = (r.y - mu) * sc + sh; r.z = (r.z - mu) * sc + sh; r.w = (r.w - mu) * sc + sh;
            if (RELU) { r.x = fmaxf(r.x, 0.f); r.y = fmaxf(r.y, 0.f); r.z = fmaxf(r.z, 0.f); r.w = fmaxf(r.w, 0.f); }
            size_t o;
            if (per_sample) {
                o = (size_t)(row / C) * y_bstride + (size_t)c * P + e;
            } else {
                const long long b = e / P;
                o = (size_t)b * y_bstride + (size_t)c * P + (size_t)(e - b * P);
            }
            Payload<T>::st4(y + o, r);
        }
    }
}

constexpr int BN_APPLY_V = 4;

template <bool RELU, typename T>
__global__ __launch_bounds__(BN_THREADS) void bn_apply_kernel(const T *__restrict__ x, int C, int P,
                                                              const float *__restrict__ mean, const float *__restrict__ invstd,
                                                              const float *__restrict__ gamma, const float *__restrict__ beta,
                                                              T *__restrict__ y, int stats_per_row, long long y_bstride) {
    const int row = blockIdx.x;
    const int c = row % C;
    const int sidx = stats_per_row ? row : c;
    const float sc = invstd[sidx] * (gamma ? gamma[c] : 1.f);
    const float mu = mean[sidx], sh = beta ? beta[c] : 0.f;
    const T *xr = x + (size_t)row * P;
    T *yr = y + (size_t)(row / C) * y_bstride + (size_t)c * P;
    const int base = blockIdx.y * (BN_THREADS * 4 * BN_APPLY_V);
    if ((P & 3) == 0) {
#pragma unroll
        for (int u = 0; u < BN_APPLY_V; ++u) {
            const int p = base + (u * BN_THREADS + threadIdx.x) * 4;
            if (p < P) {
                float4 v = Payload<T>::ld4(xr + p);
                v.x = (v.x - mu) * sc + sh; v.y = (v.y - mu) * sc + sh; v.z = (v.z - mu) * sc + sh; v.w = (v.w - mu) * sc + sh;
                if (RELU) { v.x = fmaxf(v.x, 0.f); v.y = fmaxf(v.y, 0.f); v.z = fmaxf(v.z, 0.f); v.w = fmaxf(v.w, 0.f); }
                Payload<T>::st4(yr + p, v);
            }
        }
    } else {
        for (int p = base + threadIdx.x; p < min(P, base + BN_THREADS * 4 * BN_APPLY_V); p += BN_THREADS) {
            float v = (Payload<T>::ld(xr + p) - mu) * sc + sh;
            Payload<T>::st(yr + p, RELU ? fmaxf(v, 0.f) : v);
        }
    }
}

__device__ __forceinline__ void max_pair(float &v, int &i, float ov, int oi) {
    if (ov > v || (ov == v && oi < i)) { v = ov; i = oi; }
}

template <int CTRL>
__device__ __forceinline__ void dpp_max_step(float &v, int &i) {
    const float ov = __builtin_bit_cast(float, __builtin_amdgcn_update_dpp(0, __builtin_bit_cast(int, v), CTRL, 0xF, 0xF, false));
    const int oi = __builtin_amdgcn_update_dpp(0, i, CTRL, 0xF, 0xF, false);
    max_pair(v, i, ov, oi);
}

constexpr int BN_MAX_V = 4;

template <bool RELU, int G, typename T>
__global__ __launch_bounds__(BN_THREADS) void bn_max_vec_kernel(const T *__restrict__ x, int C, int M, int NS,
                                                                const float *__restrict__ mean, const float *__restrict__ invstd,
                                                                const float *__restrict__ gamma, const float *__restrict__ beta,
                                                                T *__restrict__ out, unsigned char *__restrict__ arg,
                                                                T *__restrict__ xarg) {
    const int row = blockIdx.x;
    const int c = row % C;
    const float sc = invstd[c] * (gamma ? gamma[c] : 1.f);
    const float mu = mean[c], sh = beta ? beta[c] : 0.f;
    const long long nq = (long long)M * G;
    const T *xr = x + (size_t)row * M * NS;
    float4 v[BN_MAX_V];
    long long qs[BN_MAX_V];
#pragma unroll
    for (int u = 0; u < BN_MAX_V; ++u) {
        qs[u] = ((long long)blockIdx.y * BN_MAX_V + u) * BN_THREADS + threadIdx.x;
        v[u] = qs[u] < nq ? Payload<T>::ld4(xr + qs[u] * 4) : make_float4(0.f, 0.f, 0.f, 0.f);
    }
#pragma unroll
    for (int u = 0; u < BN_MAX_V; ++u) {
        const long long q = qs[u];
        const bool live = q < nq;
        float best = -__builtin_inff();
        int bi = 0;
        if (live) {
            const int s0 = (int)(q % G) * 4;
            const float a[4] = {(v[u].x - mu) * sc + sh, (v[u].y - mu) * sc + sh, (v[u].z - mu) * sc + sh, (v[u].w - mu) * sc + sh};
#pragma unroll
            for (int w = 0; w < 4; ++w)
                if (a[w] > best) { best = a[w]; bi = s0 + w; }
        }
        if (G >= 2) dpp_max_step<0xB1>(best, bi);
        if (G >= 4) dpp_max_step<0x4E>(best, bi);
        if (G >= 8) dpp_max_step<0x141>(best, bi);
        if (G >= 16) dpp_max_step<0x140>(best, bi);
        if (live && (threadIdx.x & (G - 1)) == 0) {
            const long long m = q / G;
            Payload<T>::st(out + (size_t)row * M + m, RELU ? fmaxf(best, 0.f) : best);
            arg[(size_t)row * M + m] = (unsigned char)bi;
            if (xarg) xarg[(size_t)row * M + m] = xr[m * NS + bi];
        }
    }
}

template <bool RELU, typename T>
__global__ __launch_bounds__(BN_THREADS) void bn_max_kernel(const T *__restrict__ x, int C, int M, int NS,
                                                            const float *__restrict__ mean, const float *__restrict__ invstd,
                                                            const float *__restrict__ gamma, const float *__restrict__ beta,
                                                            T *__restrict__ out, unsigned char *__restrict__ arg,
                                                            T *__restrict__ xarg) {
    const int row = blockIdx.x;
    const int m = blockIdx.y * BN_THREADS + threadIdx.x;
    if (m >= M) return;
    const int c = row % C;
    const float sc = invstd[c] * (gamma ? gamma[c] : 1.f);
    const float mu = mean[c], sh = beta ? beta[c] : 0.f;
    const T *xr = x + ((size_t)row * M + m) * NS;
    float best = -__builtin_inff();
    int bi = 0;
    for (int s = 0; s < NS; ++s) {
        const float a = (Payload<T>::ld(xr + s) - mu) * sc + sh;
        if (a > best) { best = a; bi = s; }
    }
    Payload<T>::st(out + (size_t)row * M + m, RELU ? fmaxf(best, 0.f) : best);
    arg[(size_t)row * M + m] = (unsigned char)bi;
    if (xarg) xarg[(size_t)row * M + m] = xr[bi];
}

template <bool RELU, typename T>
__global__ __launch_bounds__(BN_THREADS) void bn_bwd_partial_kernel(const T *__restrict__ dy, const T *__restrict__ x,
                                                                    int B, int C, int P, const float *__restrict__ mean,
                                                                    const float *__restrict__ invstd,
                                                                    const float *__restrict__ gamma,
                                                                    const float *__restrict__ beta, float *__restrict__ partial,
                                                                    int chunk) {
    __shared__ float scratch[BN_THREADS / 64];
    const int c = blockIdx.y;
    const float mu = mean[c], is = invstd[c];
    const float g = gamma ? gamma[c] : 1.f, b = beta ? beta[c] : 0.f;
    const long long n = (long long)B * P;
    const long long e0 = (long long)blockIdx.x * chunk;
    const long long e1 = min(e0 + chunk, n);
    float s = 0.f, q = 0.f;
    const float sc = is * g;
    auto acc = [&](float xv, float d) {
        const float xh = (xv - mu) * is;
        if (RELU && !((xv - mu) * sc + b > 0.f)) d = 0.f;
        s += d;
        q += d * xh;
    };
    if ((P & 3) == 0) {
        for (long long e = e0 + (long long)threadIdx.x * 4; e < e1; e += BN_THREADS * 4) {
            const size_t o = chan_off(e, c, C, P);
            const float4 xv = Payload<T>::ld4(x + o);
            const float4 dv = Payload<T>::ld4(dy + o);
            acc(xv.x, dv.x); acc(xv.y, dv.y); acc(xv.z, dv.z); acc(xv.w, dv.w);
        }
    } else {
        for (long long e = e0 + threadIdx.x; e < e1; e += BN_THREADS) {
            const size_t o = chan_off(e, c, C, P);
            acc(Payload<T>::ld(x + o), Payload<T>::ld(dy + o));
        }
    }
    s = block_sum(s, scratch);
    q = block_sum(q, scratch);
    if (threadIdx.x == 0) {
        partial[((size_t)c * gridDim.x + blockIdx.x) * 2 + 0] = s;
        partial[((size_t)c * gridDim.x + blockIdx.x) * 2 + 1] = q;
    }
}

struct DpoolStrides {
    long long b, c, m;
};

template <bool RELU, typename T>
__global__ __launch_bounds__(BN_THREADS) void bn_max_bwd_partial_kernel(const T *__restrict__ dpool,
                                                                        const T *__restrict__ pooled,
                                                                        const unsigned char *__restrict__ arg,
                                                                        const T *__restrict__ x,
                                                                        const T *__restrict__ xarg, int B, int C, int M, int NS,
                                                                        const float *__restrict__ mean,
                                                                        const float *__restrict__ invstd,
                                                                        float *__restrict__ partial, DpoolStrides ds, int chunk) {
    __shared__ float scratch[BN_THREADS / 64];
    const int c = blockIdx.y;
    const float mu = mean[c], is = invstd[c];
    const long long n = (long long)B * M;
    const long long e0 = (long long)blockIdx.x * chunk;
    const long long e1 = min(e0 + chunk, n);
    float s = 0.f, q = 0.f;
    for (long long e = e0 + threadIdx.x; e < e1; e += BN_THREADS) {
        const size_t o = chan_off(e, c, C, M);
        const long long eb = e / M;
        float d = Payload<T>::ld(dpool + eb * ds.b + c * ds.c + (e - eb * M) * ds.m);
        if (RELU && !(Payload<T>::ld(pooled + o) > 0.f)) d = 0.f;
        const float xh = ((xarg ? Payload<T>::ld(xarg + o) : Payload<T>::ld(x + o * NS + arg[o])) - mu) * is;
        s += d;
        q += d * xh;
    }
    s = block_sum(s, scratch);
    q = block_sum(q, scratch);
    if (threadIdx.x == 0) {
        partial[((size_t)c * gridDim.x + blockIdx.x) * 2 + 0] = s;
        partial[((size_t)c * gridDim.x + blockIdx.x) * 2 + 1] = q;
    }
}

__global__ __launch_bounds__(64) void bn_bwd_finalize_kernel(const float *__restrict__ partial, int nchunk, int C, double n,
                                                             float *__restrict__ dgamma, float *__restrict__ dbeta,
                                                             float *__restrict__ coef) {
    const int c = blockIdx.x;
    double s = 0.0, q = 0.0;
    for (int i = threadIdx.x; i < nchunk; i += 64) {
        s += (double)partial[((size_t)c * nchunk + i) * 2 + 0];
        q += (double)partial[((size_t)c * nchunk + i) * 2 + 1];
    }
    s = wave_sum_f64(s);
    q = wave_sum_f64(q);
    if (threadIdx.x != 0) return;
    if (dbeta) dbeta[c] = (float)s;
    if (dgamma) dgamma[c] = (float)q;
    coef[2 * c + 0] = (float)(s / n);
    coef[2 * c + 1] = (float)(q / n);
}

template <bool RELU, typename T>
__global__ __launch_bounds__(BN_THREADS) void bn_bwd_apply_kernel(const T *__restrict__ dy, const T *__restrict__ x, int C,
                                                                  int P, const float *__restrict__ mean,
                                                                  const float *__restrict__ invstd, const float *__restrict__ gamma,
                                                                  const float *__restrict__ beta, const float *__restrict__ coef,
                                                                  T *__restrict__ dx) {
    const int row = blockIdx.x;
    const int c = row % C;
    const float mu = mean[c], is = invstd[c];
    const float g = gamma ? gamma[c] : 1.f, b = beta ? beta[c] : 0.f;
    const float m0 = coef[2 * c], m1 = coef[2 * c + 1];
    const float k = is * g;
    const size_t ro = (size_t)row * P;
    auto one = [&](float xv, float d) {
        const float xh = (xv - mu) * is;
        if (RELU && !((xv - mu) * k + b > 0.f)) d = 0.f;
        return k * (d - m0 - xh * m1);
    };
    if ((P & 3) == 0) {
        const int p0 = (blockIdx.y * BN_THREADS + threadIdx.x) * 4;
        if (p0 >= P) return;
        const float4 xv = Payload<T>::ld4(x + ro + p0);
        const float4 dv = Payload<T>::ld4(dy + ro + p0);
        float4 r;
        r.x = one(xv.x, dv.x); r.y = one(xv.y, dv.y); r.z = one(xv.z, dv.z); r.w = one(xv.w, dv.w);
        Payload<T>::st4(dx + ro + p0, r);
    } else {
        const int p0 = blockIdx.y * BN_THREADS + threadIdx.x;
        if (p0 < P) Payload<T>::st(dx + ro + p0, one(Payload<T>::ld(x + ro + p0), Payload<T>::ld(dy + ro + p0)));
    }
}

template <bool RELU>
__global__ __launch_bounds__(BN_THREADS) void bn_bwd_apply_t_kernel(const float *__restrict__ dy, const float *__restrict__ x, int C,
                                                                    int P, const float *__restrict__ mean,
                                                                    const float *__restrict__ invstd, const float *__restrict__ gamma,
                                                                    const float *__restrict__ beta, const float *__restrict__ coef,
                                                                    float *__restrict__ dx_t) {
    __shared__ float tile[64][65];
    const int b = blockIdx.y, p0 = blockIdx.x * 64;
    const int np = min(64, P - p0);
    for (int e = threadIdx.x; e < C * 64; e += BN_THREADS) {
        const int c = e >> 6, pl = e & 63;
        if (pl >= np) continue;
        const size_t o = ((size_t)b * C + c) * P + p0 + pl;
        const float mu = mean[c], is = invstd[c];
        const float g = gamma ? gamma[c] : 1.f, bt = beta ? beta[c] : 0.f;
        const float k = is * g;
        const float xv = x[o];
        float d = dy[o];
        const float xh = (xv - mu) * is;
        if (RELU && !((xv - mu) * k + bt > 0.f)) d = 0.f;
        tile[pl][c] = k * (d - coef[2 * c] - xh * coef[2 * c + 1]);
    }
    __syncthreads();
    float *dst = dx_t + ((size_t)b * P + p0) * C;
    for (int e = threadIdx.x; e < np * C; e += BN_THREADS) dst[e] = tile[e / C][e % C];
}

template <bool RELU, typename T>
__global__ __launch_bounds__(BN_THREADS) void bn_max_bwd_apply_kernel(const T *__restrict__ dpool,
                                                                      const T *__restrict__ pooled,
                                                                      const unsigned char *__restrict__ arg,
                                                                      const T *__restrict__ x, int C, int M, int NS,
                                                                      const float *__restrict__ mean,
                                                                      const float *__restrict__ invstd,
                                                                      const float *__restrict__ gamma,
                                                                      const float *__restrict__ coef, T *__restrict__ dx,
                                                                      DpoolStrides ds) {
    const int row = blockIdx.x;
    const int c = row % C;
    const float mu = mean[c], is = invstd[c];
    const float k = (gamma ? gamma[c] : 1.f) * is;
    const float m0 = coef[2 * c], m1 = coef[2 * c + 1];
    const long long P = (long long)M * NS;
    const size_t ro = (size_t)row * P;
    const size_t go = (size_t)row * M;
    const int step = (NS & 3) == 0 ? 4 : 1;
    const long long p0 = ((long long)blockIdx.y * BN_THREADS + threadIdx.x) * step;
    if (p0 >= P) return;
    const int m = (int)(p0 / NS), s0 = (int)(p0 - (long long)m * NS);
    float d = Payload<T>::ld(dpool + (long long)(row / C) * ds.b + c * ds.c + m * ds.m);
    if (RELU && !(Payload<T>::ld(pooled + go + m) > 0.f)) d = 0.f;
    const int a = arg[go + m];
    if (step == 4) {
        const float4 xv = Payload<T>::ld4(x + ro + p0);
        float4 r;
        r.x = k * ((s0 + 0 == a ? d : 0.f) - m0 - (xv.x - mu) * is * m1);
        r.y = k * ((s0 + 1 == a ? d : 0.f) - m0 - (xv.y - mu) * is * m1);
        r.z = k * ((s0 + 2 == a ? d : 0.f) - m0 - (xv.z - mu) * is * m1);
        r.w = k * ((s0 + 3 == a ? d : 0.f) - m0 - (xv.w - mu) * is * m1);
        Payload<T>::st4(dx + ro + p0, r);
    } else {
        Payload<T>::st(dx + ro + p0, k * ((s0 == a ? d : 0.f) - m0 - (Payload<T>::ld(x + ro + p0) - mu) * is * m1));
    }
}

static inline int bn_chunk(int B, int C, long long P) {
    const long long n = (long long)B * P;
    int chunk = BN_CHUNK;
    while (chunk > 4096 && ((n + chunk - 1) / chunk) * C < 2048) chunk >>= 1;
    return chunk;
}
static inline int bn_nchunk_fwd(int B, int C, long long P) {
    const int chunk = bn_chunk(B, C, P);
    return (int)(((long long)B * P + chunk - 1) / chunk);
}
static inline int bn_nchunk(int B, int P) { return (int)(((long long)B * P + BN_CHUNK - 1) / BN_CHUNK); }
static inline int bn_chunk_bwd(int C, long long n) {
    int chunk = BN_CHUNK;
    while (chunk > 4096 && ((n + chunk - 1) / chunk) * C < 2048) chunk >>= 1;
    return chunk;
}

}

using namespace mgar;

#define BN_API extern "C" __attribute__((visibility("default")))

BN_API int mgar_bn_workspace_floats(int B, int C, int P) {
    if (B < 0 || C < 0 || P < 0) return MGAR_EINVAL;
    int nc = bn_nchunk_fwd(B, C, P) > bn_nchunk(B, P) ? bn_nchunk_fwd(B, C, P) : bn_nchunk(B, P);
    const int small = 4096 / (C > 0 ? C : 1) + 2;
    if (nc < small) nc = small;
    return 2 * C * (nc > 0 ? nc : 1) + 2 * C;
}

static int bn_sizes_ok(int B, int C, long long P) { return B >= 0 && C >= 0 && P >= 0 && (long long)B * C <= 2147483647LL; }

template <typename T>
static int bn_train_stats_impl(const T *x, int B, int C, int P, float eps, float momentum, float *workspace, float *mean,
                               float *invstd, float *running_mean, float *running_var, long long *num_batches_tracked,
                               void *stream) {
    MGAR_REQUIRE(bn_sizes_ok(B, C, P), "bn_train_stats: bad sizes");
    if ((long long)B * C * P == 0) return MGAR_OK;
    MGAR_REQUIRE(x && workspace && mean && invstd, "bn_train_stats: null pointer");
    MGAR_REQUIRE(C <= 65535, "bn_train_stats: C > 65535");
    const int chunk = bn_chunk(B, C, P), nchunk = bn_nchunk_fwd(B, C, P);
    hipStream_t st = (hipStream_t)stream;
    { KtScope kt(KT_BN_STATS, st, (double)sizeof(T) * B * C * P);
    hipLaunchKernelGGL(bn_partial_kernel<T>, dim3(nchunk, C), dim3(BN_THREADS), 0, st, x, B, C, P, chunk, workspace);
    }
    hipLaunchKernelGGL(bn_finalize_kernel, dim3(C), dim3(64), 0, st, workspace, nchunk, C, (double)B * P, chunk, eps,
                       momentum, mean, invstd, running_mean, running_var, num_batches_tracked, (float *)nullptr);
    return check_launch("bn_train_stats: launch failed");
}

template <typename T>
static int bn_act_fwd_impl(const T *x, int B, int C, int P, const float *mean, const float *invstd, const float *gamma,
                           const float *beta, int relu, T *y, int stats_per_row, void *stream, long long y_bstride = -1) {
    MGAR_REQUIRE(bn_sizes_ok(B, C, P), "bn_act_fwd: bad sizes");
    if (y_bstride < 0) y_bstride = (long long)C * P;
    MGAR_REQUIRE(y_bstride >= (long long)C * P, "bn_act_fwd: output batch stride smaller than a sample");
    MGAR_REQUIRE((P & 3) != 0 || ((y_bstride * (long long)sizeof(T)) % 16 == 0 && (uintptr_t)y % 16 == 0),
                 "bn_act_fwd: output slice not 16-byte aligned");
    if ((long long)B * C * P == 0) return MGAR_OK;
    MGAR_REQUIRE(x && y && mean && invstd, "bn_act_fwd: null pointer");
    MGAR_REQUIRE((long long)P <= 65535LL * BN_THREADS * 4, "bn_act_fwd: P too large");
    dim3 grid(B * C, ceil_div(P, BN_THREADS * 4 * BN_APPLY_V));
    hipStream_t st = (hipStream_t)stream;
    { KtScope kt(KT_BN_APPLY, st, 2.0 * sizeof(T) * (double)B * C * P);
    if (relu) hipLaunchKernelGGL((bn_apply_kernel<true, T>), grid, dim3(BN_THREADS), 0, st, x, C, P, mean, invstd, gamma, beta, y, stats_per_row, y_bstride);
    else hipLaunchKernelGGL((bn_apply_kernel<false, T>), grid, dim3(BN_THREADS), 0, st, x, C, P, mean, invstd, gamma, beta, y, stats_per_row, y_bstride);
    }
    return check_launch("bn_act_fwd: launch failed");
}

__global__ void bn_running_update_grouped_kernel(const float *__restrict__ mean, const float *__restrict__ var, int G, int C,
                                                 double n, float momentum, float *__restrict__ running_mean,
                                                 float *__restrict__ running_var, long long *__restrict__ num_batches_tracked) {
    const int c = blockIdx.x * blockDim.x + threadIdx.x;
    if (c == 0 && num_batches_tracked) *num_batches_tracked += G;
    if (c >= C) return;
    float rm = running_mean ? running_mean[c] : 0.f, rv = running_var ? running_var[c] : 0.f;
    for (int g = 0; g < G; ++g) {
        rm = (1.f - momentum) * rm + momentum * mean[(size_t)g * C + c];
        const double v = (double)var[(size_t)g * C + c];
        rv = (1.f - momentum) * rv + momentum * (float)(n > 1.0 ? v * n / (n - 1.0) : v);
    }
    if (running_mean) running_mean[c] = rm;
    if (running_var) running_var[c] = rv;
}

template <typename T>
static int bn_train_stats_grouped_impl(const T *x, int G, int C, int P, float eps, float momentum, float *workspace,
                                       float *mean, float *invstd, float *running_mean, float *running_var,
                                       long long *num_batches_tracked, void *stream) {
    MGAR_REQUIRE(bn_sizes_ok(G, C, P), "bn_train_stats_grouped: bad sizes");
    if ((long long)G * C * P == 0) return MGAR_OK;
    MGAR_REQUIRE(x && workspace && mean && invstd, "bn_train_stats_grouped: null pointer");
    const int rows = G * C;
    MGAR_REQUIRE(rows <= 65535, "bn_train_stats_grouped: G*C > 65535");
    const int chunk = bn_chunk(1, rows, P), nchunk = bn_nchunk_fwd(1, rows, P);
    hipStream_t st = (hipStream_t)stream;
    float *var = workspace + (size_t)2 * rows * nchunk;
    { KtScope kt(KT_BN_STATS, st, (double)sizeof(T) * G * C * P);
    hipLaunchKernelGGL(bn_partial_kernel<T>, dim3(nchunk, rows), dim3(BN_THREADS), 0, st, x, 1, rows, P, chunk, workspace);
    }
    hipLaunchKernelGGL(bn_finalize_kernel, dim3(rows), dim3(64), 0, st, workspace, nchunk, rows, (double)P, chunk, eps, momentum, mean,
                       invstd, (float *)nullptr, (float *)nullptr, (long long *)nullptr, var);
    if (running_mean || running_var || num_batches_tracked)
        hipLaunchKernelGGL(bn_running_update_grouped_kernel, dim3(ceil_div(C, 64)), dim3(64), 0, st, mean, var, G, C, (double)P,
                           momentum, running_mean, running_var, num_batches_tracked);
    return check_launch("bn_train_stats_grouped: launch failed");
}

template <typename T>
static int bn_act_maxpool_fwd_impl(const T *x, int B, int C, int M, int nsample, const float *mean, const float *invstd,
                                   const float *gamma, const float *beta, int relu, T *out, unsigned char *arg,
                                   T *xarg, void *stream) {
    MGAR_REQUIRE(bn_sizes_ok(B, C, (long long)M * nsample) && nsample >= 1 && nsample <= 255, "bn_act_maxpool_fwd: bad sizes");
    if ((long long)B * C * M == 0) return MGAR_OK;
    MGAR_REQUIRE(x && out && arg && mean && invstd, "bn_act_maxpool_fwd: null pointer");
    MGAR_REQUIRE((long long)M <= 65535LL * BN_THREADS, "bn_act_maxpool_fwd: M too large");
    hipStream_t st = (hipStream_t)stream;
    KtScope kt(KT_BN_MAX, st, (double)B * C * M * ((double)sizeof(T) * nsample + sizeof(T) + 1.0));
#define BN_MAX_VEC(G)                                                                                                  \
    {                                                                                                                  \
        dim3 gv(B * C, ceil_div((long long)M * (G), BN_THREADS * BN_MAX_V));                                                      \
        if (relu) hipLaunchKernelGGL((bn_max_vec_kernel<true, G, T>), gv, dim3(BN_THREADS), 0, st, x, C, M, nsample, mean, invstd, gamma, beta, out, arg, xarg); \
        else hipLaunchKernelGGL((bn_max_vec_kernel<false, G, T>), gv, dim3(BN_THREADS), 0, st, x, C, M, nsample, mean, invstd, gamma, beta, out, arg, xarg);     \
    }
    if (nsample == 4) BN_MAX_VEC(1)
    else if (nsample == 8) BN_MAX_VEC(2)
    else if (nsample == 16) BN_MAX_VEC(4)
    else if (nsample == 32) BN_MAX_VEC(8)
    else if (nsample == 64) BN_MAX_VEC(16)
    else {
        dim3 grid(B * C, ceil_div(M, BN_THREADS));
        if (relu) hipLaunchKernelGGL((bn_max_kernel<true, T>), grid, dim3(BN_THREADS), 0, st, x, C, M, nsample, mean, invstd, gamma, beta, out, arg, xarg);
        else hipLaunchKernelGGL((bn_max_kernel<false, T>), grid, dim3(BN_THREADS), 0, st, x, C, M, nsample, mean, invstd, gamma, beta, out, arg, xarg);
    }
#undef BN_MAX_VEC
    return check_launch("bn_act_maxpool_fwd: launch failed");
}

template <typename T>
static int bn_act_bwd_impl(const T *dy, const T *x, int B, int C, int P, const float *mean, const float *invstd,
                           const float *gamma, const float *beta, int relu, float *workspace, float *dgamma, float *dbeta,
                           T *dx, void *stream) {
    MGAR_REQUIRE(bn_sizes_ok(B, C, P), "bn_act_bwd: bad sizes");
    if ((long long)B * C * P == 0) return MGAR_OK;
    MGAR_REQUIRE(dy && x && mean && invstd && workspace && dx, "bn_act_bwd: null pointer");
    MGAR_REQUIRE(C <= 65535 && (long long)P <= 65535LL * BN_THREADS * ((P & 3) == 0 ? 4 : 1), "bn_act_bwd: C > 65535 or P too large");
    const int chunk = bn_chunk_bwd(C, (long long)B * P), nchunk = (int)(((long long)B * P + chunk - 1) / chunk);
    float *coef = workspace + (size_t)2 * C * nchunk;
    hipStream_t st = (hipStream_t)stream;
    { KtScope kt(KT_BN_BWD_REDUCE, st, 2.0 * sizeof(T) * (double)B * C * P);
    if (relu) hipLaunchKernelGGL((bn_bwd_partial_kernel<true, T>), dim3(nchunk, C), dim3(BN_THREADS), 0, st, dy, x, B, C, P, mean, invstd, gamma, beta, workspace, chunk);
    else hipLaunchKernelGGL((bn_bwd_partial_kernel<false, T>), dim3(nchunk, C), dim3(BN_THREADS), 0, st, dy, x, B, C, P, mean, invstd, gamma, beta, workspace, chunk);
    }
    hipLaunchKernelGGL(bn_bwd_finalize_kernel, dim3(C), dim3(64), 0, st, workspace, nchunk, C, (double)B * P, dgamma, dbeta, coef);
    dim3 grid(B * C, ceil_div(P, BN_THREADS * ((P & 3) == 0 ? 4 : 1)));
    { KtScope kt(KT_BN_BWD_APPLY, st, 3.0 * sizeof(T) * (double)B * C * P);
    if (relu) hipLaunchKernelGGL((bn_bwd_apply_kernel<true, T>), grid, dim3(BN_THREADS), 0, st, dy, x, C, P, mean, invstd, gamma, beta, coef, dx);
    else hipLaunchKernelGGL((bn_bwd_apply_kernel<false, T>), grid, dim3(BN_THREADS), 0, st, dy, x, C, P, mean, invstd, gamma, beta, coef, dx);
    }
    return check_launch("bn_act_bwd: launch failed");
}

template <typename T>
static int bn_act_maxpool_bwd_impl(const T *dpool, const T *pooled, const unsigned char *arg, const T *x,
                                   const T *xarg, int B, int C, int M, int nsample, const float *mean, const float *invstd,
                                   const float *gamma, int relu, float *workspace, float *dgamma, float *dbeta, T *dx,
                                   void *stream, long long dp_bs = -1, long long dp_cs = -1, long long dp_ms = 1) {
    MGAR_REQUIRE(bn_sizes_ok(B, C, (long long)M * nsample) && nsample >= 1 && nsample <= 255, "bn_act_maxpool_bwd: bad sizes");
    const DpoolStrides ds{dp_bs < 0 ? (long long)C * M : dp_bs, dp_cs < 0 ? (long long)M : dp_cs, dp_ms};
    MGAR_REQUIRE(ds.b >= 0 && ds.c >= 1 && ds.m >= 1, "bn_act_maxpool_bwd: bad dpool strides");
    if ((long long)B * C * M == 0) return MGAR_OK;
    MGAR_REQUIRE(dpool && pooled && arg && x && mean && invstd && workspace && dx, "bn_act_maxpool_bwd: null pointer");
    MGAR_REQUIRE(C <= 65535 && (long long)M * nsample <= 65535LL * BN_THREADS * ((nsample & 3) == 0 ? 4 : 1),
                 "bn_act_maxpool_bwd: C > 65535 or M*nsample too large");
    const int chunk = bn_chunk_bwd(C, (long long)B * M), nchunk = (int)(((long long)B * M + chunk - 1) / chunk);
    float *coef = workspace + (size_t)2 * C * nchunk;
    hipStream_t st = (hipStream_t)stream;
    { KtScope kt(KT_BN_MAX_BWD_REDUCE, st, (3.0 * sizeof(T) + 1.0) * (double)B * C * M);
    if (relu) hipLaunchKernelGGL((bn_max_bwd_partial_kernel<true, T>), dim3(nchunk, C), dim3(BN_THREADS), 0, st, dpool, pooled, arg, x, xarg, B, C, M, nsample, mean, invstd, workspace, ds, chunk);
    else hipLaunchKernelGGL((bn_max_bwd_partial_kernel<false, T>), dim3(nchunk, C), dim3(BN_THREADS), 0, st, dpool, pooled, arg, x, xarg, B, C, M, nsample, mean, invstd, workspace, ds, chunk);
    }
    hipLaunchKernelGGL(bn_bwd_finalize_kernel, dim3(C), dim3(64), 0, st, workspace, nchunk, C, (double)B * M * nsample, dgamma, dbeta, coef);
    dim3 grid(B * C, ceil_div((long long)M * nsample, BN_THREADS * ((nsample & 3) == 0 ? 4 : 1)));
    { KtScope kt(KT_BN_MAX_BWD_APPLY, st, (double)B * C * M * (2.0 * sizeof(T) * nsample + 2.0 * sizeof(T) + 1.0));
    if (relu) hipLaunchKernelGGL((bn_max_bwd_apply_kernel<true, T>), grid, dim3(BN_THREADS), 0, st, dpool, pooled, arg, x, C, M, nsample, mean, invstd, gamma, coef, dx, ds);
    else hipLaunchKernelGGL((bn_max_bwd_apply_kernel<false, T>), grid, dim3(BN_THREADS), 0, st, dpool, pooled, arg, x, C, M, nsample, mean, invstd, gamma, coef, dx, ds);
    }
    return check_launch("bn_act_maxpool_bwd: launch failed");
}

#define BN_BOTH(NAME, PARAMS_F, PARAMS_B, CALL_F, CALL_B)      \
    BN_API int NAME PARAMS_F { return CALL_F; }                  \
    BN_API int NAME##_bf16 PARAMS_B { return CALL_B; }
typedef const bf16_t *cbf;
typedef bf16_t *mbf;

BN_BOTH(mgar_bn_train_stats,
        (const float *x, int B, int C, int P, float eps, float momentum, float *workspace, float *mean, float *invstd,
         float *running_mean, float *running_var, long long *num_batches_tracked, void *stream),
        (const void *x, int B, int C, int P, float eps, float momentum, float *workspace, float *mean, float *invstd,
         float *running_mean, float *running_var, long long *num_batches_tracked, void *stream),
        bn_train_stats_impl<float>(x, B, C, P, eps, momentum, workspace, mean, invstd, running_mean, running_var, num_batches_tracked, stream),
        bn_train_stats_impl<bf16_t>((cbf)x, B, C, P, eps, momentum, workspace, mean, invstd, running_mean, running_var, num_batches_tracked, stream))
BN_BOTH(mgar_bn_train_stats_grouped,
        (const float *x, int G, int C, int P, float eps, float momentum, float *workspace, float *mean, float *invstd,
         float *running_mean, float *running_var, long long *num_batches_tracked, void *stream),
        (const void *x, int G, int C, int P, float eps, float momentum, float *workspace, float *mean, float *invstd,
         float *running_mean, float *running_var, long long *num_batches_tracked, void *stream),
        bn_train_stats_grouped_impl<float>(x, G, C, P, eps, momentum, workspace, mean, invstd, running_mean, running_var, num_batches_tracked, stream),
        bn_train_stats_grouped_impl<bf16_t>((cbf)x, G, C, P, eps, momentum, workspace, mean, invstd, running_mean, running_var, num_batches_tracked, stream))
BN_BOTH(mgar_bn_act_fwd,
        (const float *x, int B, int C, int P, const float *mean, const float *invstd, const float *gamma, const float *beta,
         int relu, float *y, void *stream),
        (const void *x, int B, int C, int P, const float *mean, const float *invstd, const float *gamma, const float *beta,
         int relu, void *y, void *stream),
        bn_act_fwd_impl<float>(x, B, C, P, mean, invstd, gamma, beta, relu, y, 0, stream),
        bn_act_fwd_impl<bf16_t>((cbf)x, B, C, P, mean, invstd, gamma, beta, relu, (mbf)y, 0, stream))
BN_BOTH(mgar_bn_act_fwd_grouped,
        (const float *x, int G, int C, int P, const float *mean, const float *invstd, const float *gamma, const float *beta,
         int relu, float *y, void *stream),
        (const void *x, int G, int C, int P, const float *mean, const float *invstd, const float *gamma, const float *beta,
         int relu, void *y, void *stream),
        bn_act_fwd_impl<float>(x, G, C, P, mean, invstd, gamma, beta, relu, y, 1, stream),
        bn_act_fwd_impl<bf16_t>((cbf)x, G, C, P, mean, invstd, gamma, beta, relu, (mbf)y, 1, stream))
template <typename T>
static int bn_act_small_impl(const T *x, int B, int C, int P, int per_sample, float eps, float momentum, const float *gamma,
                             const float *beta, int relu, float *workspace, float *mean, float *invstd, float *running_mean,
                             float *running_var, long long *num_batches_tracked, T *y, long long y_bstride, void *stream) {
    MGAR_REQUIRE(bn_sizes_ok(B, C, P), "bn_act_small: bad sizes");
    if ((long long)B * C * P == 0) return MGAR_OK;
    const long long n = per_sample ? P : (long long)B * P;
    if (n > BN_SMALL_MAX || (P & 3) != 0) {
        set_error("bn_act_small: needs at most 16384 elements per channel and P % 4 == 0");
        return MGAR_EUNSUPPORTED;
    }
    MGAR_REQUIRE(x && y, "bn_act_small: null pointer");
    if (y_bstride < 0) y_bstride = (long long)C * P;
    MGAR_REQUIRE(y_bstride >= (long long)C * P && (y_bstride * (long long)sizeof(T)) % 16 == 0 && (uintptr_t)y % 16 == 0,
                 "bn_act_small: bad output slice");
    const int rows = per_sample ? B * C : C;
    const bool track = running_mean || running_var || num_batches_tracked;
    MGAR_REQUIRE(!(per_sample && track) || (workspace && mean), "bn_act_small: per-sample running update needs workspace and mean");
    hipStream_t st = (hipStream_t)stream;
    float *var = per_sample && track ? workspace : nullptr;
    if (relu) hipLaunchKernelGGL((bn_small_fused_kernel<true, T>), dim3(rows), dim3(BN_THREADS), 0, st, x, B, C, P, per_sample, eps, momentum, gamma, beta, mean, invstd, var, running_mean, running_var, num_batches_tracked, y, y_bstride);
    else hipLaunchKernelGGL((bn_small_fused_kernel<false, T>), dim3(rows), dim3(BN_THREADS), 0, st, x, B, C, P, per_sample, eps, momentum, gamma, beta, mean, invstd, var, running_mean, running_var, num_batches_tracked, y, y_bstride);
    if (per_sample && track)
        hipLaunchKernelGGL(bn_running_update_grouped_kernel, dim3(ceil_div(C, 64)), dim3(64), 0, st, mean, var, B, C, (double)P, momentum,
                           running_mean, running_var, num_batches_tracked);
    return check_launch("bn_act_small: launch failed");
}
BN_BOTH(mgar_bn_act_small,
        (const float *x, int B, int C, int P, int per_sample, float eps, float momentum, const float *gamma, const float *beta, int relu,
         float *workspace, float *mean, float *invstd, float *running_mean, float *running_var, long long *num_batches_tracked,
         float *y, long long y_bstride, void *stream),
        (const void *x, int B, int C, int P, int per_sample, float eps, float momentum, const float *gamma, const float *beta, int relu,
         float *workspace, float *mean, float *invstd, float *running_mean, float *running_var, long long *num_batches_tracked,
         void *y, long long y_bstride, void *stream),
        bn_act_small_impl<float>(x, B, C, P, per_sample, eps, momentum, gamma, beta, relu, workspace, mean, invstd, running_mean, running_var, num_batches_tracked, y, y_bstride, stream),
        bn_act_small_impl<bf16_t>((cbf)x, B, C, P, per_sample, eps, momentum, gamma, beta, relu, workspace, mean, invstd, running_mean, running_var, num_batches_tracked, (mbf)y, y_bstride, stream))
BN_BOTH(mgar_bn_act_fwd_into,
        (const float *x, int B, int C, int P, const float *mean, const float *invstd, const float *gamma, const float *beta,
         int relu, int stats_per_sample, float *y, long long y_bstride, void *stream),
        (const void *x, int B, int C, int P, const float *mean, const float *invstd, const float *gamma, const float *beta,
         int relu, int stats_per_sample, void *y, long long y_bstride, void *stream),
        bn_act_fwd_impl<float>(x, B, C, P, mean, invstd, gamma, beta, relu, y, stats_per_sample != 0, stream, y_bstride),
        bn_act_fwd_impl<bf16_t>((cbf)x, B, C, P, mean, invstd, gamma, beta, relu, (mbf)y, stats_per_sample != 0, stream, y_bstride))
BN_BOTH(mgar_bn_act_maxpool_fwd,
        (const float *x, int B, int C, int M, int nsample, const float *mean, const float *invstd, const float *gamma,
         const float *beta, int relu, float *out, unsigned char *arg, float *xarg, void *stream),
        (const void *x, int B, int C, int M, int nsample, const float *mean, const float *invstd, const float *gamma,
         const float *beta, int relu, void *out, unsigned char *arg, void *xarg, void *stream),
        bn_act_maxpool_fwd_impl<float>(x, B, C, M, nsample, mean, invstd, gamma, beta, relu, out, arg, xarg, stream),
        bn_act_maxpool_fwd_impl<bf16_t>((cbf)x, B, C, M, nsample, mean, invstd, gamma, beta, relu, (mbf)out, arg, (mbf)xarg, stream))
BN_BOTH(mgar_bn_act_bwd,
        (const float *dy, const float *x, int B, int C, int P, const float *mean, const float *invstd, const float *gamma,
         const float *beta, int relu, float *workspace, float *dgamma, float *dbeta, float *dx, void *stream),
        (const void *dy, const void *x, int B, int C, int P, const float *mean, const float *invstd, const float *gamma,
         const float *beta, int relu, float *workspace, float *dgamma, float *dbeta, void *dx, void *stream),
        bn_act_bwd_impl<float>(dy, x, B, C, P, mean, invstd, gamma, beta, relu, workspace, dgamma, dbeta, dx, stream),
        bn_act_bwd_impl<bf16_t>((cbf)dy, (cbf)x, B, C, P, mean, invstd, gamma, beta, relu, workspace, dgamma, dbeta, (mbf)dx, stream))
BN_BOTH(mgar_bn_act_maxpool_bwd,
        (const float *dpool, const float *pooled, const unsigned char *arg, const float *x, const float *xarg, int B, int C,
         int M, int nsample, const float *mean, const float *invstd, const float *gamma, int relu, float *workspace,
         float *dgamma, float *dbeta, float *dx, void *stream),
        (const void *dpool, const void *pooled, const unsigned char *arg, const void *x, const void *xarg, int B, int C,
         int M, int nsample, const float *mean, const float *invstd, const float *gamma, int relu, float *workspace,
         float *dgamma, float *dbeta, void *dx, void *stream),
        bn_act_maxpool_bwd_impl<float>(dpool, pooled, arg, x, xarg, B, C, M, nsample, mean, invstd, gamma, relu, workspace, dgamma, dbeta, dx, stream),
        bn_act_maxpool_bwd_impl<bf16_t>((cbf)dpool, (cbf)pooled, arg, (cbf)x, (cbf)xarg, B, C, M, nsample, mean, invstd, gamma, relu, workspace, dgamma, dbeta, (mbf)dx, stream))

BN_API int mgar_bn_act_bwd_rowmajor(const float *dy, const float *x, int B, int C, int P, const float *mean, const float *invstd,
                                    const float *gamma, const float *beta, int relu, float *workspace, float *dgamma, float *dbeta,
                                    float *dx_t, void *stream) {
    MGAR_REQUIRE(bn_sizes_ok(B, C, P), "bn_act_bwd_rowmajor: bad sizes");
    if (C > 64) {
        set_error("bn_act_bwd_rowmajor: C <= 64");
        return MGAR_EUNSUPPORTED;
    }
    if ((long long)B * C * P == 0) return MGAR_OK;
    MGAR_REQUIRE(dy && x && mean && invstd && workspace && dx_t, "bn_act_bwd_rowmajor: null pointer");
    MGAR_REQUIRE(B <= 65535, "bn_act_bwd_rowmajor: B > 65535");
    const int chunk = bn_chunk_bwd(C, (long long)B * P), nchunk = (int)(((long long)B * P + chunk - 1) / chunk);
    float *coef = workspace + (size_t)2 * C * nchunk;
    hipStream_t st = (hipStream_t)stream;
    { KtScope kt(KT_BN_BWD_REDUCE, st, 8.0 * (double)B * C * P);
    if (relu) hipLaunchKernelGGL((bn_bwd_partial_kernel<true, float>), dim3(nchunk, C), dim3(BN_THREADS), 0, st, dy, x, B, C, P, mean, invstd, gamma, beta, workspace, chunk);
    else hipLaunchKernelGGL((bn_bwd_partial_kernel<false, float>), dim3(nchunk, C), dim3(BN_THREADS), 0, st, dy, x, B, C, P, mean, invstd, gamma, beta, workspace, chunk);
    }
    hipLaunchKernelGGL(bn_bwd_finalize_kernel, dim3(C), dim3(64), 0, st, workspace, nchunk, C, (double)B * P, dgamma, dbeta, coef);
    dim3 grid(ceil_div(P, 64), B);
    { KtScope kt(KT_BN_BWD_APPLY, st, 12.0 * (double)B * C * P);
    if (relu) hipLaunchKernelGGL(bn_bwd_apply_t_kernel<true>, grid, dim3(BN_THREADS), 0, st, dy, x, C, P, mean, invstd, gamma, beta, coef, dx_t);
    else hipLaunchKernelGGL(bn_bwd_apply_t_kernel<false>, grid, dim3(BN_THREADS), 0, st, dy, x, C, P, mean, invstd, gamma, beta, coef, dx_t);
    }
    return check_launch("bn_act_bwd_rowmajor: launch failed");
}

BN_API int mgar_bn_act_maxpool_bwd_strided(const float *dpool, long long sb, long long sc, long long sm, const float *pooled,
                                           const unsigned char *arg, const float *x, const float *xarg, int B, int C, int M,
                                           int nsample, const float *mean, const float *invstd, const float *gamma, int relu,
                                           float *workspace, float *dgamma, float *dbeta, float *dx, void *stream) {
    MGAR_REQUIRE(sb >= 0 && sc >= 1 && sm >= 1, "bn_act_maxpool_bwd_strided: bad strides");
    return bn_act_maxpool_bwd_impl<float>(dpool, pooled, arg, x, xarg, B, C, M, nsample, mean, invstd, gamma, relu, workspace, dgamma,
                                          dbeta, dx, stream, sb, sc, sm);
}

constexpr int BN_MERGE_PER_LANE = 4, BN_MERGE_G = 64 * BN_MERGE_PER_LANE;
__global__ __launch_bounds__(64) void bn_merge_partials_kernel(const float *__restrict__ in, int nchunk, double n, int chunk,
                                                              float *__restrict__ out) {
    const int c = blockIdx.y, g = blockIdx.x, ngroup = gridDim.x;
    const int i0 = g * BN_MERGE_G, i1 = min(i0 + BN_MERGE_G, nchunk);
    auto count = [&](int i) { return i + 1 < nchunk ? (double)chunk : n - (double)chunk * (nchunk - 1); };
    float2 v[BN_MERGE_PER_LANE];
    double cnt[BN_MERGE_PER_LANE], s = 0.0, tot = 0.0;
#pragma unroll
    for (int k = 0; k < BN_MERGE_PER_LANE; ++k) {
        const int i = i0 + k * 64 + (int)threadIdx.x;
        const bool ok = i < i1;
        v[k] = ok ? *reinterpret_cast<const float2 *>(in + ((size_t)c * nchunk + i) * 2) : make_float2(0.f, 0.f);
        cnt[k] = ok ? count(i) : 0.0;
        s += cnt[k] * (double)v[k].x;
        tot += cnt[k];
    }
    s = wave_sum_f64(s);
    tot = wave_sum_f64(tot);
    const double m = s / tot;
    double q = 0.0;
#pragma unroll
    for (int k = 0; k < BN_MERGE_PER_LANE; ++k) {
        const double d = (double)v[k].x - m;
        q += (double)v[k].y + cnt[k] * d * d;
    }
    q = wave_sum_f64(q);
    if (threadIdx.x == 0) *reinterpret_cast<float2 *>(out + ((size_t)c * ngroup + g) * 2) = make_float2((float)m, (float)q);
}

BN_API long long mgar_bn_stats_from_partials_workspace_floats(int nchunk, int C) {
    if (nchunk < 0 || C < 0) return -1;
    return nchunk > 4 * BN_MERGE_G ? 2ll * C * ((nchunk + BN_MERGE_G - 1) / BN_MERGE_G) : 0;
}
BN_API int mgar_bn_stats_from_partials(const float *partial, int nchunk, int C, long long n, int chunk, float eps, float momentum,
                                       float *workspace, float *mean, float *invstd, float *running_mean, float *running_var,
                                       long long *num_batches_tracked, void *stream) {
    MGAR_REQUIRE(nchunk >= 0 && C >= 0 && n >= 0 && chunk >= 1, "bn_stats_from_partials: bad sizes");
    if (C == 0 || n == 0) return MGAR_OK;
    MGAR_REQUIRE(partial && mean && invstd, "bn_stats_from_partials: null pointer");
    MGAR_REQUIRE((long long)nchunk * chunk >= n && (long long)(nchunk - 1) * chunk < n, "bn_stats_from_partials: nchunk * chunk does not cover n");
    MGAR_REQUIRE(C <= 65535, "bn_stats_from_partials: C > 65535");
    if (nchunk > 4 * BN_MERGE_G) {
        MGAR_REQUIRE(workspace, "bn_stats_from_partials: null workspace");
        MGAR_REQUIRE((long long)chunk * BN_MERGE_G <= 2147483647LL, "bn_stats_from_partials: chunk too large");
        const int ngroup = (nchunk + BN_MERGE_G - 1) / BN_MERGE_G;
        hipLaunchKernelGGL(bn_merge_partials_kernel, dim3(ngroup, C), dim3(64), 0, (hipStream_t)stream, partial, nchunk, (double)n, chunk,
                           workspace);
        partial = workspace;
        nchunk = ngroup;
        chunk *= BN_MERGE_G;
    }
    hipLaunchKernelGGL(bn_finalize_kernel, dim3(C), dim3(64), 0, (hipStream_t)stream, partial, nchunk, C, (double)n, chunk, eps, momentum,
                       mean, invstd, running_mean, running_var, num_batches_tracked, (float *)nullptr);
    return check_launch("bn_stats_from_partials: launch failed");
}

BN_API int mgar_bn_act_bwd_apply(const float *dy, const float *x, int B, int C, int P, const float *mean, const float *invstd,
                                 const float *gamma, const float *beta, int relu, const float *coef, int rowmajor, float *dx,
                                 void *stream) {
    MGAR_REQUIRE(bn_sizes_ok(B, C, P), "bn_act_bwd_apply: bad sizes");
    if ((long long)B * C * P == 0) return MGAR_OK;
    MGAR_REQUIRE(dy && x && mean && invstd && coef && dx, "bn_act_bwd_apply: null pointer");
    hipStream_t st = (hipStream_t)stream;
    KtScope kt(KT_BN_BWD_APPLY, st, 12.0 * (double)B * C * P);
    if (rowmajor) {
        if (C > 64) {
            set_error("bn_act_bwd_apply: rowmajor needs C <= 64");
            return MGAR_EUNSUPPORTED;
        }
        MGAR_REQUIRE(B <= 65535, "bn_act_bwd_apply: B > 65535");
        dim3 grid(ceil_div(P, 64), B);
        if (relu) hipLaunchKernelGGL(bn_bwd_apply_t_kernel<true>, grid, dim3(BN_THREADS), 0, st, dy, x, C, P, mean, invstd, gamma, beta, coef, dx);
        else hipLaunchKernelGGL(bn_bwd_apply_t_kernel<false>, grid, dim3(BN_THREADS), 0, st, dy, x, C, P, mean, invstd, gamma, beta, coef, dx);
    } else {
        MGAR_REQUIRE(C <= 65535 && (long long)P <= 65535LL * BN_THREADS * ((P & 3) == 0 ? 4 : 1), "bn_act_bwd_apply: C > 65535 or P too large");
        dim3 grid(B * C, ceil_div(P, BN_THREADS * ((P & 3) == 0 ? 4 : 1)));
        if (relu) hipLaunchKernelGGL((bn_bwd_apply_kernel<true, float>), grid, dim3(BN_THREADS), 0, st, dy, x, C, P, mean, invstd, gamma, beta, coef, dx);
        else hipLaunchKernelGGL((bn_bwd_apply_kernel<false, float>), grid, dim3(BN_THREADS), 0, st, dy, x, C, P, mean, invstd, gamma, beta, coef, dx);
    }
    return check_launch("bn_act_bwd_apply: launch failed");
}

#include "channels_last.hpp"
```

multimodal_gar_amd/csrc/errors.hip:

```cpp
#include "common.hpp"

#include <mutex>
#include <vector>

namespace mgar {
static thread_local const char *g_last_error = "";
void set_error(const char *msg) { g_last_error = msg; }

int g_kt_on = 0;
namespace {
struct KtLaunch { hipEvent_t a, b; };
struct KtSlot {
    std::vector<KtLaunch> pending;
    hipEvent_t open = nullptr;
    double ms = 0.0, bytes = 0.0, flops = 0.0;
    long long launches = 0;
};
KtSlot g_kt[KT_COUNT];
std::mutex g_kt_mu;
const char *const kKtNames[KT_COUNT] = {
    "fps_kernel", "ball_query_kernel", "three_nn_kernel", "three_interp_fwd", "three_interp_bwd", "query_group_fwd",
    "query_group_bwd", "bn_partial_kernel", "bn_apply_kernel", "bn_max_vec_kernel", "bn_bwd_partial_kernel",
    "bn_bwd_apply_kernel", "bn_max_bwd_partial_kernel", "bn_max_bwd_apply_kernel", "pointwise_fwd_kernel",
    "pointwise_dw_kernel", "rowmajor_dw_kernel", "maxpool3d_same_kernel", "voxel_roi_pool_fwd", "voxel_roi_pool_bwd", "stem_conv3d_kernel", "query_group_inverse_index",
    "image_resize_normalize",
    "dafm_attn_fwd", "dafm_attn_bwd", "gatv2_fwd", "gatv2_bwd", "roi_align_fwd", "roi_align_bwd", "voxel_query_kernel", "points_in_boxes_kernel",
    "roipoint_pool3d_kernel", "spconv_index", "spconv_gemm", "spconv_dw", "point_grid_build", "ball_query_grid_kernel", "three_nn_grid_kernel", "conv3d_wino_kernel"};
}

void kt_begin(int id, hipStream_t st) {
    std::lock_guard<std::mutex> lk(g_kt_mu);
    KtSlot &s = g_kt[id];
    if (hipEventCreate(&s.open) != hipSuccess) { s.open = nullptr; return; }
    (void)hipEventRecord(s.open, st);
}
void kt_end(int id, hipStream_t st, double bytes, double flops) {
    std::lock_guard<std::mutex> lk(g_kt_mu);
    KtSlot &s = g_kt[id];
    if (!s.open) return;
    hipEvent_t b;
    if (hipEventCreate(&b) != hipSuccess) { (void)hipEventDestroy(s.open); s.open = nullptr; return; }
    (void)hipEventRecord(b, st);
    s.pending.push_back({s.open, b});
    s.open = nullptr;
    s.bytes += bytes;
    s.flops += flops;
    s.launches += 1;
}
}

using namespace mgar;

extern "C" __attribute__((visibility("default"))) int mgar_abi_version(void) { return 12; }
extern "C" __attribute__((visibility("default"))) const char *mgar_last_error(void) { return mgar::g_last_error; }

extern "C" __attribute__((visibility("default"))) int mgar_ktimer_enable(int on) {
    g_kt_on = on ? 1 : 0;
    return MGAR_OK;
}
extern "C" __attribute__((visibility("default"))) int mgar_ktimer_count(void) { return KT_COUNT; }
extern "C" __attribute__((visibility("default"))) const char *mgar_ktimer_name(int id) {
    return id >= 0 && id < KT_COUNT ? kKtNames[id] : "";
}
extern "C" __attribute__((visibility("default"))) int mgar_ktimer_add_flops(int id, double flops) {
    MGAR_REQUIRE(id >= 0 && id < KT_COUNT, "ktimer_add_flops: bad kernel id");
    if (!g_kt_on) return MGAR_OK;
    std::lock_guard<std::mutex> lk(g_kt_mu);
    g_kt[id].flops += flops;
    return MGAR_OK;
}
extern "C" __attribute__((visibility("default"))) int mgar_ktimer_add_bytes(int id, double bytes) {
    MGAR_REQUIRE(id >= 0 && id < KT_COUNT, "ktimer_add_bytes: bad kernel id");
    if (!g_kt_on) return MGAR_OK;
    std::lock_guard<std::mutex> lk(g_kt_mu);
    g_kt[id].bytes += bytes;
    return MGAR_OK;
}
extern "C" __attribute__((visibility("default"))) int mgar_ktimer_read(int id, double *total_ms, long long *launches,
                                                                      double *total_bytes, double *total_flops, int reset) {
    MGAR_REQUIRE(id >= 0 && id < KT_COUNT, "ktimer_read: bad kernel id");
    std::lock_guard<std::mutex> lk(g_kt_mu);
    KtSlot &s = g_kt[id];
    for (KtLaunch &l : s.pending) {
        float ms = 0.f;
        if (hipEventSynchronize(l.b) == hipSuccess && hipEventElapsedTime(&ms, l.a, l.b) == hipSuccess) s.ms += ms;
        (void)hipEventDestroy(l.a);
        (void)hipEventDestroy(l.b);
    }
    s.pending.clear();
    if (total_ms) *total_ms = s.ms;
    if (launches) *launches = s.launches;
    if (total_bytes) *total_bytes = s.bytes;
    if (total_flops) *total_flops = s.flops;
    if (reset) { s.ms = s.bytes = s.flops = 0.0; s.launches = 0; }
    return MGAR_OK;
}

namespace mgar {
__global__ void delay_kernel(long long ticks) {
    const long long t0 = wall_clock64();
    while (wall_clock64() - t0 < ticks) __builtin_amdgcn_s_sleep(32);
}
}
extern "C" __attribute__((visibility("default"))) int mgar_delay_us(int us, void *stream) {
    MGAR_REQUIRE(us >= 0 && us <= 1000, "delay_us: 0 .. 1000 microseconds");
    if (us == 0) return MGAR_OK;
    hipLaunchKernelGGL(mgar::delay_kernel, dim3(1), dim3(64), 0, (hipStream_t)stream, (long long)us * 100);
    return check_launch("delay_us: launch failed");
}
```

multimodal_gar_amd/csrc/pointwise_dw.hip:

```cpp
#include "common.hpp"

namespace mgar {

typedef float __attribute__((ext_vector_type(16))) f32x16;

constexpr int DW_TP = 128;
constexpr int DW_LD = DW_TP + 1;

struct DwAct {
    const float *mean, *invstd, *gamma, *beta;
    int relu;
    int pair;
};

template <int OB, int IB>
__global__ __launch_bounds__(256) void pointwise_dw_kernel(const float *__restrict__ x, const float *__restrict__ dy, int B, int Cin,
                                                           int Cout, int P, DwAct act, float *__restrict__ partial) {
    extern __shared__ float lds[];
    __shared__ float act_sc[IB * 32], act_sh[IB * 32], act_mu[IB * 32];
    __shared__ float act_is[IB * 32];
    float *sy = lds;
    float *sx = lds + OB * 32 * DW_LD;
    const int o_base = blockIdx.y * OB * 32, i_base = blockIdx.z * IB * 32;
    const bool has_act = act.mean != nullptr;
    const bool pair = act.pair != 0;
    const int CinV = pair ? 2 * Cin : Cin;
    if (has_act) {
        for (int r = threadIdx.x; r < IB * 32; r += 256) {
            const int chv = i_base + r, ch = (pair && chv >= Cin) ? chv - Cin : chv;
            float sc = 1.f, sh = 0.f, mu = 0.f, is = 0.f;
            if (chv < CinV) {
                sc = act.invstd[ch] * (act.gamma ? act.gamma[ch] : 1.f);
                sh = act.beta ? act.beta[ch] : 0.f;
                mu = act.mean[ch];
                is = act.invstd[ch];
            }
            act_sc[r] = sc;
            act_sh[r] = sh;
            act_mu[r] = mu;
            act_is[r] = is;
        }
        __syncthreads();
    }
    auto pair_of = [&](float v, int r, bool kind) {
        const float mu = act_mu[r];
        const bool on = !act.relu || (v - mu) * act_sc[r] + act_sh[r] > 0.f;
        return on ? (kind ? (v - mu) * act_is[r] : 1.f) : 0.f;
    };
    const int lane = threadIdx.x & 63, wave = threadIdx.x >> 6;
    const int tiles_per_b = (P + DW_TP - 1) / DW_TP;
    const long long total_tiles = (long long)B * tiles_per_b;
    const bool vec = (P & 3) == 0;

    f32x16 acc[OB][IB];
#pragma unroll
    for (int a = 0; a < OB; ++a)
#pragma unroll
        for (int c = 0; c < IB; ++c)
#pragma unroll
            for (int r = 0; r < 16; ++r) acc[a][c][r] = 0.f;

    constexpr int NV = (OB + IB) * 32 * (DW_TP / 4) / 256;
    float4 pre[NV];
    auto fetch = [&](long long tile) {
        const int b = (int)(tile / tiles_per_b);
        const int p0 = (int)(tile - (long long)b * tiles_per_b) * DW_TP;
#pragma unroll
        for (int u = 0; u < NV; ++u) {
            const int e = threadIdx.x + u * 256;
            const int row = e / (DW_TP / 4), c4 = (e - row * (DW_TP / 4)) * 4;
            const bool is_y = row < OB * 32;
            const int chv = is_y ? o_base + row : i_base + row - OB * 32;
            const int ch = (!is_y && pair && chv >= Cin) ? chv - Cin : chv;
            const int cmax = is_y ? Cout : Cin;
            pre[u] = (chv < (is_y ? Cout : CinV) && p0 + c4 < P)
                         ? *reinterpret_cast<const float4 *>((is_y ? dy : x) + ((size_t)b * cmax + ch) * P + p0 + c4)
                         : make_float4(0.f, 0.f, 0.f, 0.f);
        }
    };
    if (vec && (long long)blockIdx.x < total_tiles) fetch(blockIdx.x);

    for (long long tile = blockIdx.x; tile < total_tiles; tile += gridDim.x) {
        const int b = (int)(tile / tiles_per_b);
        const int p0 = (int)(tile - (long long)b * tiles_per_b) * DW_TP;
        if (vec) {
#pragma unroll
            for (int u = 0; u < NV; ++u) {
                const int e = threadIdx.x + u * 256;
                const int row = e / (DW_TP / 4), c4 = (e - row * (DW_TP / 4)) * 4;
                const bool is_y = row < OB * 32;
                const int ch = is_y ? o_base + row : i_base + row - OB * 32;
                float4 v = pre[u];
                if (has_act && !is_y && ch < CinV && p0 + c4 < P) {
                    const int r = row - OB * 32;
                    if (pair) {
                        const bool kind = ch >= Cin;
                        v.x = pair_of(v.x, r, kind); v.y = pair_of(v.y, r, kind); v.z = pair_of(v.z, r, kind); v.w = pair_of(v.w, r, kind);
                    } else {
                        const float sc = act_sc[r], sh = act_sh[r], mu = act_mu[r];
                        v.x = (v.x - mu) * sc + sh; v.y = (v.y - mu) * sc + sh; v.z = (v.z - mu) * sc + sh; v.w = (v.w - mu) * sc + sh;
                        if (act.relu) { v.x = fmaxf(v.x, 0.f); v.y = fmaxf(v.y, 0.f); v.z = fmaxf(v.z, 0.f); v.w = fmaxf(v.w, 0.f); }
                    }
                }
                float *d = lds + row * DW_LD + c4;
                d[0] = v.x; d[1] = v.y; d[2] = v.z; d[3] = v.w;
            }
        } else {
            for (int e = threadIdx.x; e < (OB + IB) * 32 * DW_TP; e += 256) {
                const int row = e / DW_TP, cc = e - row * DW_TP;
                const bool is_y = row < OB * 32;
                const int chv = is_y ? o_base + row : i_base + row - OB * 32;
                const int ch = (!is_y && pair && chv >= Cin) ? chv - Cin : chv;
                const int cmax = is_y ? Cout : Cin;
                float v = 0.f;
                if (chv < (is_y ? Cout : CinV) && p0 + cc < P) {
                    v = (is_y ? dy : x)[((size_t)b * cmax + ch) * P + p0 + cc];
                    if (has_act && !is_y) {
                        if (pair) {
                            v = pair_of(v, row - OB * 32, chv >= Cin);
                        } else {
                            v = (v - act_mu[row - OB * 32]) * act_sc[row - OB * 32] + act_sh[row - OB * 32];
                            if (act.relu) v = fmaxf(v, 0.f);
                        }
                    }
                }
                lds[row * DW_LD + cc] = v;
            }
        }
        __syncthreads();
        if (vec && tile + gridDim.x < total_tiles) fetch(tile + gridDim.x);
        const int colw = wave * 32 + (lane >> 5);
#pragma unroll 4
        for (int ks = 0; ks < 16; ++ks) {
            const int cc = colw + 2 * ks;
            float af[OB], bf[IB];
#pragma unroll
            for (int a = 0; a < OB; ++a) af[a] = sy[(a * 32 + (lane & 31)) * DW_LD + cc];
#pragma unroll
            for (int c = 0; c < IB; ++c) bf[c] = sx[(c * 32 + (lane & 31)) * DW_LD + cc];
#pragma unroll
            for (int a = 0; a < OB; ++a)
#pragma unroll
                for (int c = 0; c < IB; ++c)
                    acc[a][c] = __builtin_amdgcn_mfma_f32_32x32x2f32(af[a], bf[c], acc[a][c], 0, 0, 0);
        }
        __syncthreads();
    }
    if (wave > 0) {
#pragma unroll
        for (int a = 0; a < OB; ++a)
#pragma unroll
            for (int c = 0; c < IB; ++c)
#pragma unroll
                for (int r = 0; r < 16; ++r) lds[(((wave - 1) * OB * IB + a * IB + c) * 16 + r) * 64 + lane] = acc[a][c][r];
    }
    __syncthreads();
    if (wave > 0) return;
#pragma unroll
    for (int a = 0; a < OB; ++a)
#pragma unroll
        for (int c = 0; c < IB; ++c)
#pragma unroll
            for (int r = 0; r < 16; ++r) {
                float v = acc[a][c][r];
#pragma unroll
                for (int w = 0; w < 3; ++w) v += lds[((w * OB * IB + a * IB + c) * 16 + r) * 64 + lane];
                const int o = o_base + a * 32 + (r & 3) + 8 * (r >> 2) + 4 * (lane >> 5);
                const int i = i_base + c * 32 + (lane & 31);
                if (o < Cout && i < CinV) partial[((size_t)blockIdx.x * Cout + o) * CinV + i] = v;
            }
}

constexpr int DWR_SLICES = 16;
__global__ __launch_bounds__(64 * DWR_SLICES) void pointwise_dw_reduce_kernel(const float *__restrict__ partial, int gx, int n_out,
                                                                              float *__restrict__ dw) {
    __shared__ float part[DWR_SLICES][64];
    const int e = blockIdx.x * 64 + (threadIdx.x & 63), slice = threadIdx.x >> 6;
    const int per = (gx + DWR_SLICES - 1) / DWR_SLICES, g0 = min(slice * per, gx), g1 = min(g0 + per, gx);
    float s = 0.f;
    if (e < n_out) {
        int g = g0;
        for (; g + 8 <= g1; g += 8) {
            float v[8];
#pragma unroll
            for (int u = 0; u < 8; ++u) v[u] = partial[(size_t)(g + u) * n_out + e];
#pragma unroll
            for (int u = 0; u < 8; ++u) s += v[u];
        }
        for (; g < g1; ++g) s += partial[(size_t)g * n_out + e];
    }
    part[slice][threadIdx.x & 63] = s;
    __syncthreads();
    if (slice == 0 && e < n_out) {
        float t = 0.f;
#pragma unroll
        for (int i = 0; i < DWR_SLICES; ++i) t += part[i][threadIdx.x];
        dw[e] = t;
    }
}

__global__ void pointwise_dw_pair_finalize_kernel(const float *__restrict__ ab, const float *__restrict__ w, int Cin, int Cout, double n,
                                                  const float *__restrict__ gamma, const float *__restrict__ beta,
                                                  float *__restrict__ dw, float *__restrict__ dgamma, float *__restrict__ dbeta,
                                                  float *__restrict__ coef) {
    const int i = blockIdx.x * blockDim.x + threadIdx.x;
    if (i >= Cin) return;
    const float g = gamma ? gamma[i] : 1.f, b = beta ? beta[i] : 0.f;
    double s = 0.0, q = 0.0;
    for (int o = 0; o < Cout; ++o) {
        const float a = ab[(size_t)o * 2 * Cin + i], bb = ab[(size_t)o * 2 * Cin + Cin + i], wv = w[(size_t)o * Cin + i];
        if (dw) dw[(size_t)o * Cin + i] = g * bb + b * a;
        s += (double)wv * (double)a;
        q += (double)wv * (double)bb;
    }
    if (dbeta) dbeta[i] = (float)s;
    if (dgamma) dgamma[i] = (float)q;
    coef[2 * i + 0] = (float)(s / n);
    coef[2 * i + 1] = (float)(q / n);
}

static int dw_grid_x(int B, int Cin, int Cout, int P, int ob, int ib) {
    const long long tiles = (long long)B * ((P + DW_TP - 1) / DW_TP);
    const int gy = ceil_div(Cout, ob * 32), gz = ceil_div(Cin, ib * 32);
    long long gx = 2048 / (gy * gz);
    if (gx > (tiles + 3) / 4) gx = (tiles + 3) / 4;
    if (gx < 1) gx = 1;
    return (int)gx;
}
static void dw_blocks(int Cin, int Cout, int &ob, int &ib) {
    ob = Cout <= 32 ? 1 : 2;
    ib = Cin <= 32 ? 1 : (Cin <= 64 ? 2 : 4);
}

template <int OB, int IB>
static void launch_dw(const float *x, const float *dy, int B, int Cin, int Cout, int P, const DwAct &act, float *partial,
                      hipStream_t st) {
    static bool attr_set = false;
    const int lds = (OB + IB) * 32 * DW_LD * (int)sizeof(float);
    if (!attr_set) {
        (void)hipFuncSetAttribute((const void *)pointwise_dw_kernel<OB, IB>, hipFuncAttributeMaxDynamicSharedMemorySize, lds);
        attr_set = true;
    }
    const int CinV = act.pair ? 2 * Cin : Cin;
    const int gy = ceil_div(Cout, OB * 32), gz = ceil_div(CinV, IB * 32);
    const int gx = dw_grid_x(B, CinV, Cout, P, OB, IB);
    hipLaunchKernelGGL((pointwise_dw_kernel<OB, IB>), dim3((unsigned)gx, gy, gz), dim3(256), lds, st, x, dy, B, Cin, Cout, P, act, partial);
}

}

using namespace mgar;

extern "C" __attribute__((visibility("default"))) int mgar_pointwise_dw_workspace_floats(int B, int Cin, int Cout, int P) {
    if (B <= 0 || Cin <= 0 || Cout <= 0 || P <= 0) return 0;
    int ob, ib;
    dw_blocks(Cin, Cout, ob, ib);
    return dw_grid_x(B, Cin, Cout, P, ob, ib) * Cout * Cin;
}

extern "C" __attribute__((visibility("default"))) int mgar_pointwise_conv_dw_act(const float *x, const float *dy, int B, int Cin,
                                                                                int Cout, int P, const float *in_mean,
                                                                                const float *in_invstd, const float *in_gamma,
                                                                                const float *in_beta, int in_relu,
                                                                                float *workspace, float *dw, void *stream) {
    MGAR_REQUIRE(B >= 0 && Cin >= 0 && Cout >= 0 && P >= 0, "pointwise_conv_dw: negative size");
    if (Cin == 0 || Cout == 0) return MGAR_OK;
    MGAR_REQUIRE(dw, "pointwise_conv_dw: null pointer");
    MGAR_REQUIRE(in_mean == nullptr || in_invstd != nullptr, "pointwise_conv_dw: in_mean without in_invstd");
    hipStream_t st = (hipStream_t)stream;
    if ((long long)B * P == 0) {
        (void)hipMemsetAsync(dw, 0, sizeof(float) * Cout * Cin, st);
        return check_launch("pointwise_conv_dw: memset failed");
    }
    MGAR_REQUIRE(x && dy && workspace, "pointwise_conv_dw: null pointer");
    const DwAct act{in_mean, in_invstd, in_gamma, in_beta, in_relu, 0};
    int ob, ib;
    dw_blocks(Cin, Cout, ob, ib);
    {
    KtScope kt(KT_POINTWISE_DW, st, 4.0 * (double)B * P * (Cin + Cout), 2.0 * (double)B * P * Cin * Cout);
    if (ob == 1 && ib == 1) launch_dw<1, 1>(x, dy, B, Cin, Cout, P, act, workspace, st);
    else if (ob == 1 && ib == 2) launch_dw<1, 2>(x, dy, B, Cin, Cout, P, act, workspace, st);
    else if (ob == 1 && ib == 4) launch_dw<1, 4>(x, dy, B, Cin, Cout, P, act, workspace, st);
    else if (ob == 2 && ib == 1) launch_dw<2, 1>(x, dy, B, Cin, Cout, P, act, workspace, st);
    else if (ob == 2 && ib == 2) launch_dw<2, 2>(x, dy, B, Cin, Cout, P, act, workspace, st);
    else launch_dw<2, 4>(x, dy, B, Cin, Cout, P, act, workspace, st);
    }
    const int gx = dw_grid_x(B, Cin, Cout, P, ob, ib), n_out = Cout * Cin;
    hipLaunchKernelGGL(pointwise_dw_reduce_kernel, dim3(ceil_div(n_out, 64)), dim3(64 * DWR_SLICES), 0, st, workspace, gx, n_out, dw);
    return check_launch("pointwise_conv_dw: launch failed");
}

extern "C" __attribute__((visibility("default"))) int mgar_pointwise_conv_dw(const float *x, const float *dy, int B, int Cin,
                                                                            int Cout, int P, float *workspace, float *dw,
                                                                            void *stream) {
    return mgar_pointwise_conv_dw_act(x, dy, B, Cin, Cout, P, nullptr, nullptr, nullptr, nullptr, 0, workspace, dw, stream);
}

extern "C" __attribute__((visibility("default"))) int mgar_pointwise_dw_bnbwd_workspace_floats(int B, int Cin, int Cout, int P) {
    if (B <= 0 || Cin <= 0 || Cout <= 0 || P <= 0) return 0;
    int ob, ib;
    dw_blocks(2 * Cin, Cout, ob, ib);
    return dw_grid_x(B, 2 * Cin, Cout, P, ob, ib) * Cout * 2 * Cin + Cout * 2 * Cin;
}
extern "C" __attribute__((visibility("default"))) int mgar_pointwise_conv_dw_bnbwd(const float *x, const float *dy, const float *w, int B,
                                                                                  int Cin, int Cout, int P, const float *in_mean,
                                                                                  const float *in_invstd, const float *in_gamma,
                                                                                  const float *in_beta, int in_relu, float *workspace,
                                                                                  float *dw, float *dgamma, float *dbeta, float *coef,
                                                                                  void *stream) {
    MGAR_REQUIRE(B >= 0 && Cin >= 1 && Cout >= 1 && P >= 0, "pointwise_conv_dw_bnbwd: bad sizes");
    if (Cin > 64 || Cout > 64) {
        set_error("pointwise_conv_dw_bnbwd: Cin <= 64 and Cout <= 64");
        return MGAR_EUNSUPPORTED;
    }
    MGAR_REQUIRE((long long)B * P > 0, "pointwise_conv_dw_bnbwd: empty input");
    MGAR_REQUIRE(x && dy && w && in_mean && in_invstd && workspace && coef, "pointwise_conv_dw_bnbwd: null pointer");
    hipStream_t st = (hipStream_t)stream;
    const DwAct act{in_mean, in_invstd, in_gamma, in_beta, in_relu, 1};
    int ob, ib;
    dw_blocks(2 * Cin, Cout, ob, ib);
    const int gx = dw_grid_x(B, 2 * Cin, Cout, P, ob, ib), n_out = Cout * 2 * Cin;
    float *ab = workspace + (size_t)gx * n_out;
    {
        KtScope kt(KT_POINTWISE_DW, st, 4.0 * (double)B * P * (Cin + Cout), 4.0 * (double)B * P * Cin * Cout);
        if (ob == 1 && ib == 1) launch_dw<1, 1>(x, dy, B, Cin, Cout, P, act, workspace, st);
        else if (ob == 1 && ib == 2) launch_dw<1, 2>(x, dy, B, Cin, Cout, P, act, workspace, st);
        else if (ob == 1 && ib == 4) launch_dw<1, 4>(x, dy, B, Cin, Cout, P, act, workspace, st);
        else if (ob == 2 && ib == 1) launch_dw<2, 1>(x, dy, B, Cin, Cout, P, act, workspace, st);
        else if (ob == 2 && ib == 2) launch_dw<2, 2>(x, dy, B, Cin, Cout, P, act, workspace, st);
        else launch_dw<2, 4>(x, dy, B, Cin, Cout, P, act, workspace, st);
    }
    hipLaunchKernelGGL(pointwise_dw_reduce_kernel, dim3(ceil_div(n_out, 64)), dim3(64 * DWR_SLICES), 0, st, workspace, gx, n_out, ab);
    hipLaunchKernelGGL(pointwise_dw_pair_finalize_kernel, dim3(ceil_div(Cin, 64)), dim3(64), 0, st, ab, w, Cin, Cout, (double)B * P, in_gamma,
                       in_beta, dw, dgamma, dbeta, coef);
    return check_launch("pointwise_conv_dw_bnbwd: launch failed");
}
```

multimodal_gar_amd/csrc/pointwise_fwd.hip:

```cpp
#include <type_traits>

#include "common.hpp"
#include "payload.hpp"

namespace mgar {

typedef float __attribute__((ext_vector_type(16))) f32x16;

constexpr int PF_COLS = 128;
template <int OB> struct PfSlab { static constexpr int KC = OB == 1 ? 16 : 8; };

template <typename T>
struct PfArgs {
    const T *x;
    const float *w;
    const float *mean, *invstd, *gamma, *beta;
    T *y;
    int B, Cin, Cout, P;
    int w_rs, w_cs;
    int relu;
    float *stats;
};

template <int OB, typename T, bool STATS = false>
__global__ __launch_bounds__(256, 2) void pointwise_fwd_kernel(PfArgs<T> a) {
    constexpr int PF_KC = PfSlab<OB>::KC, KS = PF_KC / 2;
    constexpr int WLD = OB == 1 ? 32 : 96;
    extern __shared__ float lds[];
    const int nkc = (a.Cin + PF_KC - 1) / PF_KC;
    float *wl = lds;
    float *act = lds + (size_t)nkc * PF_KC * WLD;
    for (int e = threadIdx.x; e < nkc * PF_KC * WLD; e += 256) {
        const int ch = e / WLD, o = e - ch * WLD;
        wl[e] = (ch < a.Cin && o < a.Cout) ? a.w[(size_t)o * a.w_rs + (size_t)ch * a.w_cs] : 0.f;
    }
    for (int ch = threadIdx.x; ch < nkc * PF_KC; ch += 256) {
        float sc = 1.f, sh = 0.f, mu = 0.f;
        if (a.mean && ch < a.Cin) {
            sc = a.invstd[ch] * (a.gamma ? a.gamma[ch] : 1.f);
            sh = a.beta ? a.beta[ch] : 0.f;
            mu = a.mean[ch];
        }
        *reinterpret_cast<float4 *>(act + 4 * ch) = make_float4(sc, sh, mu, 0.f);
    }
    __syncthreads();

    const int lane = threadIdx.x & 63, wave = threadIdx.x >> 6;
    const int l = lane & 31, h = lane >> 5;
    const int tiles_per_b = (a.P + PF_COLS - 1) / PF_COLS;
    const long long ntiles = (long long)a.B * tiles_per_b;
    const long long wave_id = (long long)blockIdx.x * 4 + wave, nwaves = (long long)gridDim.x * 4;
    if (wave_id >= ntiles) return;
    const long long my_tiles = (ntiles - wave_id + nwaves - 1) / nwaves;
    const long long steps = my_tiles * nkc;
    const bool has_act = a.mean != nullptr, relu = a.relu != 0;

    f32x16 acc[OB][4];
#pragma unroll
    for (int ob = 0; ob < OB; ++ob)
#pragma unroll
        for (int j = 0; j < 4; ++j)
#pragma unroll
            for (int r = 0; r < 16; ++r) acc[ob][j][r] = 0.f;

    auto issue = [&](long long s, float4 (&buf)[KS]) {
        const long long t = wave_id + (s / nkc) * nwaves;
        const int kc = (int)(s % nkc);
        const int b = (int)(t / tiles_per_b);
        const int p = (int)(t - (long long)b * tiles_per_b) * PF_COLS + 4 * l;
        const T *src = a.x + ((size_t)b * a.Cin + kc * PF_KC + h) * a.P + p;
#pragma unroll
        for (int ks = 0; ks < KS; ++ks) {
            const int ch = kc * PF_KC + 2 * ks + h;
            buf[ks] = (ch < a.Cin && p < a.P) ? Payload<T>::ld4(src + (size_t)2 * ks * a.P)
                                              : make_float4(0.f, 0.f, 0.f, 0.f);
        }
    };
    auto compute = [&](long long s, float4 (&buf)[KS]) {
        const int kc = (int)(s % nkc);
#pragma unroll
        for (int ks = 0; ks < KS; ++ks) {
            const int ch = kc * PF_KC + 2 * ks + h;
            float4 v = buf[ks];
            if (has_act) {
                const float4 ac = *reinterpret_cast<const float4 *>(act + 4 * ch);
                const float sc = ac.x, sh = ac.y, mu = ac.z;
                v.x = (v.x - mu) * sc + sh; v.y = (v.y - mu) * sc + sh; v.z = (v.z - mu) * sc + sh; v.w = (v.w - mu) * sc + sh;
                if (relu) { v.x = fmaxf(v.x, 0.f); v.y = fmaxf(v.y, 0.f); v.z = fmaxf(v.z, 0.f); v.w = fmaxf(v.w, 0.f); }
                if (ch >= a.Cin) v = make_float4(0.f, 0.f, 0.f, 0.f);
            }
#pragma unroll
            for (int ob = 0; ob < OB; ++ob) {
                const float wa = wl[ch * WLD + ob * 32 + l];
                acc[ob][0] = __builtin_amdgcn_mfma_f32_32x32x2f32(wa, v.x, acc[ob][0], 0, 0, 0);
                acc[ob][1] = __builtin_amdgcn_mfma_f32_32x32x2f32(wa, v.y, acc[ob][1], 0, 0, 0);
                acc[ob][2] = __builtin_amdgcn_mfma_f32_32x32x2f32(wa, v.z, acc[ob][2], 0, 0, 0);
                acc[ob][3] = __builtin_amdgcn_mfma_f32_32x32x2f32(wa, v.w, acc[ob][3], 0, 0, 0);
            }
        }
        if (kc == nkc - 1) {
            const long long t = wave_id + (s / nkc) * nwaves;
            const int b = (int)(t / tiles_per_b);
            const int p = (int)(t - (long long)b * tiles_per_b) * PF_COLS + 4 * l;
            if (STATS) {
#pragma unroll
                for (int ob = 0; ob < OB; ++ob)
#pragma unroll
                    for (int r = 0; r < 16; ++r) {
                        const float v0 = acc[ob][0][r], v1 = acc[ob][1][r], v2 = acc[ob][2][r], v3 = acc[ob][3][r];
                        float sum = (v0 + v1) + (v2 + v3);
#pragma unroll
                        for (int d = 1; d < 32; d <<= 1) sum += __shfl_xor(sum, d, 32);
                        const float mean = sum * (1.f / PF_COLS);
                        const float d0 = v0 - mean, d1 = v1 - mean, d2 = v2 - mean, d3 = v3 - mean;
                        float m2 = (d0 * d0 + d1 * d1) + (d2 * d2 + d3 * d3);
#pragma unroll
                        for (int d = 1; d < 32; d <<= 1) m2 += __shfl_xor(m2, d, 32);
                        const int o = ob * 32 + (r & 3) + 8 * (r >> 2) + 4 * h;
                        if (l == 0 && o < a.Cout)
                            *reinterpret_cast<float2 *>(a.stats + ((size_t)o * ntiles + t) * 2) = make_float2(mean, m2);
                    }
            }
#pragma unroll
            for (int ob = 0; ob < OB; ++ob)
#pragma unroll
                for (int r = 0; r < 16; ++r) {
                    const int o = ob * 32 + (r & 3) + 8 * (r >> 2) + 4 * h;
                    if (o < a.Cout && p < a.P)
                        Payload<T>::st4(a.y + ((size_t)b * a.Cout + o) * a.P + p,
                                        make_float4(acc[ob][0][r], acc[ob][1][r], acc[ob][2][r], acc[ob][3][r]));
                    acc[ob][0][r] = 0.f; acc[ob][1][r] = 0.f; acc[ob][2][r] = 0.f; acc[ob][3][r] = 0.f;
                }
        }
    };

    float4 buf0[KS], buf1[KS];
    issue(0, buf0);
    for (long long s = 0; s < steps; s += 2) {
        if (s + 1 < steps) issue(s + 1, buf1);
        compute(s, buf0);
        if (s + 1 < steps) {
            if (s + 2 < steps) issue(s + 2, buf0);
            compute(s + 1, buf1);
        }
    }
}

template <int OB, typename T, bool STATS = false>
static void launch_pf(const PfArgs<T> &a, hipStream_t st) {
    constexpr int WLD = OB == 1 ? 32 : 96, PF_KC = PfSlab<OB>::KC;
    const int nkc = (a.Cin + PF_KC - 1) / PF_KC;
    const int lds = nkc * PF_KC * (WLD + 4) * (int)sizeof(float);
    static int attr_lds = 0;
    if (lds > 65536 && lds > attr_lds) {
        (void)hipFuncSetAttribute((const void *)pointwise_fwd_kernel<OB, T, STATS>, hipFuncAttributeMaxDynamicSharedMemorySize, lds);
        attr_lds = lds;
    }
    const long long ntiles = (long long)a.B * ((a.P + PF_COLS - 1) / PF_COLS);
    long long wgs = (ntiles + 3) / 4;
    if (wgs > 2048) wgs = 2048;
    hipLaunchKernelGGL((pointwise_fwd_kernel<OB, T, STATS>), dim3((unsigned)wgs), dim3(256), lds, st, a);
}

}

using namespace mgar;

template <typename T>
static int pointwise_conv_fwd_impl(const T *x, int B, int Cin, int P, const float *w, int w_row_stride, int w_col_stride, int Cout,
                                   const float *in_mean, const float *in_invstd, const float *in_gamma, const float *in_beta,
                                   int in_relu, T *y, void *stream, float *out_stats = nullptr) {
    MGAR_REQUIRE(B >= 0 && Cin >= 0 && Cout >= 0 && P >= 0, "pointwise_conv_fwd: negative size");
    if ((long long)B * P == 0 || Cout == 0) return MGAR_OK;
    MGAR_REQUIRE(x && w && y, "pointwise_conv_fwd: null pointer");
    MGAR_REQUIRE(in_mean == nullptr || in_invstd != nullptr, "pointwise_conv_fwd: in_mean without in_invstd");
    if (Cout > 64 || Cin > 256 || Cin == 0 || (P & 3) != 0) {
        set_error("pointwise_conv_fwd: needs 1 <= Cin <= 256, Cout <= 64 and P % 4 == 0 (use the library GEMM otherwise)");
        return MGAR_EUNSUPPORTED;
    }
    MGAR_REQUIRE(out_stats == nullptr || P % PF_COLS == 0, "pointwise_conv_fwd: output statistics need P % 128 == 0");
    PfArgs<T> a{x, w, in_mean, in_invstd, in_gamma, in_beta, y, B, Cin, Cout, P, w_row_stride, w_col_stride, in_relu, out_stats};
    hipStream_t st = (hipStream_t)stream;
    KtScope kt(KT_POINTWISE_FWD, st, (double)sizeof(T) * B * P * (Cin + Cout), 2.0 * (double)B * P * Cin * Cout);
    if (out_stats) {
        if constexpr (std::is_same<T, float>::value) launch_pf<1, float, true>(a, st);
    } else if (Cout <= 32) launch_pf<1, T>(a, st);
    else launch_pf<2, T>(a, st);
    return check_launch("pointwise_conv_fwd: launch failed");
}

#define PF_API extern "C" __attribute__((visibility("default")))
PF_API int mgar_pointwise_conv_fwd(const float *x, int B, int Cin, int P, const float *w, int w_row_stride, int w_col_stride, int Cout,
                                   const float *in_mean, const float *in_invstd, const float *in_gamma, const float *in_beta,
                                   int in_relu, float *y, void *stream) {
    return pointwise_conv_fwd_impl<float>(x, B, Cin, P, w, w_row_stride, w_col_stride, Cout, in_mean, in_invstd, in_gamma, in_beta,
                                          in_relu, y, stream);
}
PF_API int mgar_pointwise_conv_fwd_bf16(const void *x, int B, int Cin, int P, const float *w, int w_row_stride, int w_col_stride,
                                        int Cout, const float *in_mean, const float *in_invstd, const float *in_gamma,
                                        const float *in_beta, int in_relu, void *y, void *stream) {
    return pointwise_conv_fwd_impl<bf16_t>((const bf16_t *)x, B, Cin, P, w, w_row_stride, w_col_stride, Cout, in_mean, in_invstd,
                                           in_gamma, in_beta, in_relu, (bf16_t *)y, stream);
}

PF_API int mgar_pointwise_conv_fwd_stats(const float *x, int B, int Cin, int P, const float *w, int w_row_stride, int w_col_stride,
                                         int Cout, const float *in_mean, const float *in_invstd, const float *in_gamma,
                                         const float *in_beta, int in_relu, float *y, float *out_stats, void *stream) {
    MGAR_REQUIRE(out_stats, "pointwise_conv_fwd_stats: null pointer");
    if (Cout > 32) {
        set_error("pointwise_conv_fwd_stats: Cout <= 32 (run mgar_pointwise_conv_fwd and the BatchNorm's own statistics pass)");
        return MGAR_EUNSUPPORTED;
    }
    return pointwise_conv_fwd_impl<float>(x, B, Cin, P, w, w_row_stride, w_col_stride, Cout, in_mean, in_invstd, in_gamma, in_beta,
                                          in_relu, y, stream, out_stats);
}
```

multimodal_gar_amd/nn_utils.py:

```python
import torch
import torch.nn as nn


class _PointwiseConv(torch.autograd.Function):

    @staticmethod
    def forward(ctx, x3, w):
        ctx.save_for_backward(x3, w)
        return torch.bmm(w.unsqueeze(0).expand(x3.shape[0], -1, -1), x3)

    @staticmethod
    def backward(ctx, dy):
        from . import _lib as L
        x3, w = ctx.saved_tensors
        dy = dy.contiguous()
        dx = dw = None
        if ctx.needs_input_grad[0]:
            dx = torch.bmm(w.t().unsqueeze(0).expand(dy.shape[0], -1, -1), dy)
        if ctx.needs_input_grad[1]:
            dw = pointwise_dw(x3, dy)
        return dx, dw


_DW_MIN_COLUMNS = 1 << 16


def pointwise_dw(x3, dy):
    from . import _lib as L
    x3, dy = x3.contiguous(), dy.contiguous()
    b, cin, p = x3.shape
    cout = dy.shape[1]
    dw = torch.empty((cout, cin), dtype=torch.float32, device=dy.device)
    ws = torch.empty((max(1, L.raw("mgar_pointwise_dw_workspace_floats", b, cin, cout, p)),), dtype=torch.float32, device=dy.device)
    L.call("mgar_pointwise_conv_dw", L.fptr(x3), L.fptr(dy), b, cin, cout, p, L.fptr(ws), L.fptr(dw), L.stream_of(dy))
    return dw


def conv1x1(conv, x):
    w = conv.weight.view(1, conv.out_channels, conv.in_channels)
    x3 = x.flatten(2)
    if (x3.is_cuda and x3.dtype == torch.float32 and x3.shape[0] * x3.shape[2] >= _DW_MIN_COLUMNS
            and conv.out_channels <= 64 and conv.in_channels <= 128
            and torch.is_grad_enabled() and conv.weight.requires_grad):
        y = _PointwiseConv.apply(x3, w[0].contiguous())
    else:
        y = torch.bmm(w.expand(x3.shape[0], -1, -1), x3)
    if conv.bias is not None:
        y = y + conv.bias.view(1, -1, 1)
    return y.view(x.shape[0], conv.out_channels, *x.shape[2:])


def _is_pointwise(m):
    return isinstance(m, (nn.Conv1d, nn.Conv2d, nn.Conv3d)) and all(k == 1 for k in m.kernel_size) \
        and all(s == 1 for s in m.stride) and all(p == 0 for p in m.padding) and m.groups == 1


_BN_TYPES = (nn.BatchNorm1d, nn.BatchNorm2d, nn.BatchNorm3d)


class PointwiseSequential(nn.Sequential):

    fuse_bn_conv = True

    def _run(self, x, pool_last, start=0, rowmajor_input_grad=False, input_stats=None):
        from . import bn_ops
        layers = list(self)
        i, n = start, len(layers)
        pooled = False
        stats = input_stats
        while i < n:
            layer = layers[i]
            rm = rowmajor_input_grad and i == start and x.dim() == 4
            if _is_pointwise(layer):
                feeds_bn = i + 1 < n and isinstance(layers[i + 1], _BN_TYPES) and layers[i + 1].training
                y = bn_ops.plain_conv(x, layer, want_out_stats=feeds_bn) if x.is_cuda and self.fuse_bn_conv else None
                if y is not None:
                    x, stats = y if feeds_bn else (y, None)
                else:
                    x, stats = conv1x1(layer, x), None
                i += 1
            elif isinstance(layer, _BN_TYPES) and x.is_cuda:
                relu = i + 1 < n and isinstance(layers[i + 1], nn.ReLU)
                last = i + (2 if relu else 1) >= n
                y = None
                nxt = i + (2 if relu else 1)
                if nxt < n and _is_pointwise(layers[nxt]) and self.fuse_bn_conv:
                    feeds_bn = nxt + 1 < n and isinstance(layers[nxt + 1], _BN_TYPES) and layers[nxt + 1].training
                    y = bn_ops.bn_act_conv(x, layer, relu, layers[nxt], rowmajor_grad=rm, in_stats=stats, want_out_stats=feeds_bn)
                    if y is not None:
                        x, stats = y if feeds_bn else (y, None)
                        i = nxt + 1
                        continue
                if pool_last and last and x.dim() == 4:
                    y = bn_ops.bn_act_maxpool(x, layer, relu, in_stats=stats)
                    pooled = y is not None
                if y is None:
                    y = bn_ops.bn_act(x, layer, relu, rowmajor_grad=rm, in_stats=stats)
                if y is None:
                    y = layer(x)
                    relu = False
                x, stats = y, None
                i += 2 if relu else 1
            else:
                x = layer(x)
                stats = None
                i += 1
        return x, pooled

    def forward(self, x):
        return self._run(x, False)[0]

    def forward_maxpool(self, x, start=0, rowmajor_input_grad=False, input_stats=None):
        y, pooled = self._run(x, True, start, rowmajor_input_grad, input_stats)
        return y if pooled else y.max(dim=3).values

    def first_layer_foldable(self, c_in):
        conv = self[0] if len(self) else None
        return conv is not None and _is_pointwise(conv) and conv.bias is None and conv.in_channels == c_in \
            and conv.out_channels < c_in
```

Before: 45.19 clips/sec.

## Fuse BN-act-maxpool backward into pointwise conv dW and data-grad kernels

Adds a fused autograd path for the final BN→ReLU→conv→BN→ReLU→maxpool block of PointNet MLPs. In backward it computes only the BN coefficients of the last BN, then recomputes the maxpool/BN input gradient on the fly inside the pointwise conv dW and data-grad kernels. This avoids materialising the full-size dx tensor of the last BN. The cost is extra per-element recompute and extra loads of the per-group pool metadata in two kernels. The path is enabled by default through an environment flag.

```diff
diff --git a/include/mgar_ops.h b/include/mgar_ops.h
--- a/include/mgar_ops.h
+++ b/include/mgar_ops.h
@@ -210,6 +210,10 @@
 int mgar_bn_act_bwd_rowmajor(const float *dy, const float *x, int B, int C, int P, const float *mean, const float *invstd,
                              const float *gamma, const float *beta, int relu, float *workspace, float *dgamma,
                              float *dbeta, float *dx_t, void *stream);
+int mgar_bn_act_maxpool_bwd_coef(const float *dpool, long long sb, long long sc, long long sm, const float *pooled,
+                                 const unsigned char *arg, const float *x, const float *xarg, int B, int C, int M, int nsample,
+                                 const float *mean, const float *invstd, int relu, float *workspace, float *dgamma, float *dbeta,
+                                 float *coef, void *stream);
 int mgar_bn_act_maxpool_bwd(const float *dpool, const float *pooled, const unsigned char *arg, const float *x,
                             const float *xarg, int B, int C, int M, int nsample, const float *mean, const float *invstd,
                             const float *gamma, int relu, float *workspace, float *dgamma, float *dbeta,
@@ -233,6 +237,16 @@
 int mgar_pointwise_conv_fwd_stats(const float *x, int B, int Cin, int P, const float *w, int w_row_stride, int w_col_stride,
                                   int Cout, const float *in_mean, const float *in_invstd, const float *in_gamma,
                                   const float *in_beta, int in_relu, float *y, float *out_stats, void *stream);
+
+int mgar_pointwise_conv_bwd_data_maxpool(const float *xl, const float *dpool, long long sb, long long sc, long long sm,
+                                         const float *pooled, const unsigned char *arg, int nsample, const float *l_mean,
+                                         const float *l_invstd, const float *l_gamma, int l_relu, const float *l_coef, int B, int Cy,
+                                         int P, const float *w, int Cx, float *ga, void *stream);
+int mgar_pointwise_conv_dw_act_maxpool(const float *x, const float *xl, const float *dpool, long long sb, long long sc, long long sm,
+                                       const float *pooled, const unsigned char *arg, int nsample, const float *l_mean,
+                                       const float *l_invstd, const float *l_gamma, int l_relu, const float *l_coef, int B, int Cin,
+                                       int Cout, int P, const float *in_mean, const float *in_invstd, const float *in_gamma,
+                                       const float *in_beta, int in_relu, float *workspace, float *dw, void *stream);
 
 int mgar_maxpool3d_same_fwd(const float *x, int NC, int T, int H, int W, int kt, int kh, int kw, int st, int sh,
                             int sw, float *y, void *stream);
diff --git a/multimodal_gar_amd/_lib.py b/multimodal_gar_amd/_lib.py
--- a/multimodal_gar_amd/_lib.py
+++ b/multimodal_gar_amd/_lib.py
@@ -5,7 +5,7 @@
 
 _HERE = os.path.dirname(os.path.abspath(__file__))
 LIB_PATH = os.path.join(_HERE, "csrc", "libmgar_hip.so")
-ABI_VERSION = 12
+ABI_VERSION = 13
 
 if not os.path.exists(LIB_PATH):
     raise ImportError(
@@ -101,6 +101,10 @@
     "mgar_bn_act_bwd_apply": [_P, _P, _I, _I, _I, _P, _P, _P, _P, _I, _P, _I, _P, _P],
     "mgar_pointwise_conv_dw_act": [_P, _P, _I, _I, _I, _I, _P, _P, _P, _P, _I, _P, _P, _P],
     "mgar_pointwise_conv_fwd": [_P, _I, _I, _I, _P, _I, _I, _I, _P, _P, _P, _P, _I, _P, _P],
+    "mgar_pointwise_conv_bwd_data_maxpool": [_P, _P, _LL, _LL, _LL, _P, _P, _I, _P, _P, _P, _I, _P, _I, _I, _I, _P, _I, _P, _P],
+    "mgar_pointwise_conv_dw_act_maxpool": [_P, _P, _P, _LL, _LL, _LL, _P, _P, _I, _P, _P, _P, _I, _P, _I, _I, _I, _I, _P, _P, _P, _P,
+                                           _I, _P, _P, _P],
+    "mgar_bn_act_maxpool_bwd_coef": [_P, _LL, _LL, _LL, _P, _P, _P, _P, _I, _I, _I, _I, _P, _P, _I, _P, _P, _P, _P, _P],
     "mgar_stem_conv3d_workspace_floats": [],
     "mgar_stem_conv3d_set_minimal_filtering": [_I],
     "mgar_stem_conv3d_fwd": [_P, _I, _I, _I, _I, _P, _P, _P, _P],
diff --git a/multimodal_gar_amd/bn_ops.py b/multimodal_gar_amd/bn_ops.py
--- a/multimodal_gar_amd/bn_ops.py
+++ b/multimodal_gar_amd/bn_ops.py
@@ -1,3 +1,5 @@
+import os
+
 import torch
 import torch.nn as nn
 from torch.autograd import Function
@@ -193,6 +195,74 @@
         return dx, dgamma, dbeta, None, None, None, dw, None, None
 
 
+def _dpool_strides(dpool, b):
+    if dpool.dtype == torch.float32 and dpool.dim() == 3 and (b == 1 or dpool.stride(0) >= 0) and min(dpool.stride(1), dpool.stride(2)) >= 1:
+        return dpool, (dpool.stride(0) if b > 1 else 0), dpool.stride(1), dpool.stride(2)
+    d = dpool.contiguous().float()
+    return d, d.stride(0) if b > 1 else 0, d.stride(1), d.stride(2)
+
+
+class _BnActConvMaxPool(Function):
+
+    @staticmethod
+    def forward(ctx, x3, gamma, beta, mean, invstd, relu, w, rowmajor_grad, out_stats, bn2, relu2, gamma2, beta2, ns):
+        b, c, p = x3.shape
+        cout = w.shape[0]
+        ctx.rowmajor = bool(rowmajor_grad) and c <= ROWMAJOR_GRAD_MAX_CHANNELS
+        w = w.contiguous()
+        y = torch.empty((b, cout, p), dtype=torch.float32, device=x3.device)
+        if out_stats is not None:
+            L.call("mgar_pointwise_conv_fwd_stats", L.fptr(x3), b, c, p, L.fptr(w), c, 1, cout, L.fptr(mean), L.fptr(invstd),
+                   L.fptr(gamma), L.fptr(beta), int(relu), L.fptr(y), L.fptr(out_stats), L.stream_of(x3))
+        else:
+            L.call("mgar_pointwise_conv_fwd", L.fptr(x3), b, c, p, L.fptr(w), c, 1, cout, L.fptr(mean), L.fptr(invstd),
+                   L.fptr(gamma), L.fptr(beta), int(relu), L.fptr(y), L.stream_of(x3))
+        mean2, invstd2 = _stats(y, bn2, out_stats)
+        m = p // ns
+        out = torch.empty((b, cout, m), dtype=torch.float32, device=x3.device)
+        arg = torch.empty((b, cout, m), dtype=torch.uint8, device=x3.device)
+        xarg = torch.empty((b, cout, m), dtype=torch.float32, device=x3.device)
+        L.call("mgar_bn_act_maxpool_fwd", L.fptr(y), b, cout, m, ns, L.fptr(mean2), L.fptr(invstd2), L.fptr(gamma2), L.fptr(beta2),
+               int(relu2), L.fptr(out), _u8ptr(arg), L.fptr(xarg), L.stream_of(x3))
+        ctx.save_for_backward(x3, gamma, beta, mean, invstd, w, y, gamma2, mean2, invstd2, out, arg, xarg)
+        ctx.relu, ctx.relu2, ctx.ns = bool(relu), bool(relu2), ns
+        return out
+
+    @staticmethod
+    @once_differentiable
+    def backward(ctx, dpool):
+        x3, gamma, beta, mean, invstd, w, y, gamma2, mean2, invstd2, out, arg, xarg = ctx.saved_tensors
+        b, c, p = x3.shape
+        cout, ns = w.shape[0], ctx.ns
+        m = p // ns
+        st = L.stream_of(x3)
+        dp, sb, sc, sm = _dpool_strides(dpool, b)
+        dgamma2, dbeta2 = torch.empty_like(gamma2), torch.empty_like(gamma2)
+        coef2 = torch.empty((2 * cout,), dtype=torch.float32, device=x3.device)
+        ws = _workspace(y, b, cout, p)
+        L.call("mgar_bn_act_maxpool_bwd_coef", dp.data_ptr(), sb, sc, sm, L.fptr(out), _u8ptr(arg), L.fptr(y), L.fptr(xarg), b, cout, m,
+               ns, L.fptr(mean2), L.fptr(invstd2), int(ctx.relu2), L.fptr(ws), L.fptr(dgamma2), L.fptr(dbeta2), L.fptr(coef2), st)
+        mp = (L.fptr(y), dp.data_ptr(), sb, sc, sm, L.fptr(out), _u8ptr(arg), ns, L.fptr(mean2), L.fptr(invstd2), L.fptr(gamma2),
+              int(ctx.relu2), L.fptr(coef2))
+        dw = None
+        if ctx.needs_input_grad[6]:
+            dw = torch.empty_like(w)
+            wsd = torch.empty((max(1, L.raw("mgar_pointwise_dw_workspace_floats", b, c, cout, p)),), dtype=torch.float32, device=x3.device)
+            L.call("mgar_pointwise_conv_dw_act_maxpool", L.fptr(x3), *mp, b, c, cout, p, L.fptr(mean), L.fptr(invstd), L.fptr(gamma),
+                   L.fptr(beta), int(ctx.relu), L.fptr(wsd), L.fptr(dw), st)
+        ga = torch.empty_like(x3)
+        L.call("mgar_pointwise_conv_bwd_data_maxpool", *mp, b, cout, p, L.fptr(w), c, L.fptr(ga), st)
+        dgamma, dbeta = torch.empty_like(gamma), torch.empty_like(gamma)
+        ws1 = _workspace(x3, b, c, p)
+        if ctx.rowmajor:
+            dx = _bwd_rowmajor(ga, x3, mean, invstd, gamma, beta, ctx.relu, ws1, dgamma, dbeta)
+        else:
+            dx = torch.empty_like(x3)
+            L.call("mgar_bn_act_bwd", L.fptr(ga), L.fptr(x3), b, c, p, L.fptr(mean), L.fptr(invstd), L.fptr(gamma), L.fptr(beta),
+                   int(ctx.relu), L.fptr(ws1), L.fptr(dgamma), L.fptr(dbeta), L.fptr(dx), st)
+        return dx, dgamma, dbeta, None, None, None, dw, None, None, None, None, dgamma2, dbeta2, None
+
+
 class _PlainConv(Function):
 
     @staticmethod
@@ -252,6 +322,9 @@
 FUSED_DW_BN_REDUCE = False
 FUSED_CONV_MAX_CHANNELS = 64
 
+MLP_BWD_FUSION = os.environ.get("MGAR_MLP_BWD_FUSION", "1") != "0"
+MAXPOOL_GRAD_MAX_CHANNELS = 32
+
 
 FUSED_STATS_MAX_CHANNELS = 32
 
@@ -273,6 +346,23 @@
     y = _BnActConv.apply(x3, gamma, beta, mean, invstd, relu, _f32(conv.weight).view(cout, c), rowmajor_grad, out_stats)
     y = y.view(x.shape[0], cout, *x.shape[2:])
     return (y, out_stats) if want_out_stats else y
+
+
+def bn_act_conv_maxpool(x, bn, relu, conv, bn2, relu2, rowmajor_grad=False, in_stats=None):
+    if not (MLP_BWD_FUSION and not FUSED_DW_BN_REDUCE and x.is_cuda and x.dtype == torch.float32 and x.dim() == 4 and bn.training
+            and bn2.training and conv.bias is None and torch.is_grad_enabled()):
+        return None
+    b, c, m, ns = x.shape
+    cout = conv.out_channels
+    if c > MAXPOOL_GRAD_MAX_CHANNELS or cout > FUSED_CONV_MAX_CHANNELS or ns % 4 != 0 or ns > 255 or b * m * ns < (1 << 16):
+        return None
+    x3 = x.contiguous().flatten(2)
+    mean, invstd = _stats(x3, bn, in_stats)
+    gamma, beta = _affine(bn, c, x.device)
+    gamma2, beta2 = _affine(bn2, cout, x.device)
+    out_stats = stats_partial_buffer(x3, cout, b * m * ns) if cout <= FUSED_STATS_MAX_CHANNELS and (m * ns) % STATS_TILE == 0 else None
+    return _BnActConvMaxPool.apply(x3, gamma, beta, mean, invstd, relu, _f32(conv.weight).view(cout, c), rowmajor_grad, out_stats, bn2,
+                                   relu2, gamma2, beta2, ns)
 
 
 def _affine(bn, c, device):
diff --git a/multimodal_gar_amd/csrc/bn_act.hip b/multimodal_gar_amd/csrc/bn_act.hip
--- a/multimodal_gar_amd/csrc/bn_act.hip
+++ b/multimodal_gar_amd/csrc/bn_act.hip
@@ -642,22 +642,24 @@
 static int bn_act_maxpool_bwd_impl(const T *dpool, const T *pooled, const unsigned char *arg, const T *x,
                                    const T *xarg, int B, int C, int M, int nsample, const float *mean, const float *invstd,
                                    const float *gamma, int relu, float *workspace, float *dgamma, float *dbeta, T *dx,
-                                   void *stream, long long dp_bs = -1, long long dp_cs = -1, long long dp_ms = 1) {
+                                   void *stream, long long dp_bs = -1, long long dp_cs = -1, long long dp_ms = 1,
+                                   float *coef_only = nullptr) {
     MGAR_REQUIRE(bn_sizes_ok(B, C, (long long)M * nsample) && nsample >= 1 && nsample <= 255, "bn_act_maxpool_bwd: bad sizes");
     const DpoolStrides ds{dp_bs < 0 ? (long long)C * M : dp_bs, dp_cs < 0 ? (long long)M : dp_cs, dp_ms};
     MGAR_REQUIRE(ds.b >= 0 && ds.c >= 1 && ds.m >= 1, "bn_act_maxpool_bwd: bad dpool strides");
     if ((long long)B * C * M == 0) return MGAR_OK;
-    MGAR_REQUIRE(dpool && pooled && arg && x && mean && invstd && workspace && dx, "bn_act_maxpool_bwd: null pointer");
+    MGAR_REQUIRE(dpool && pooled && arg && x && mean && invstd && workspace && (dx || coef_only), "bn_act_maxpool_bwd: null pointer");
     MGAR_REQUIRE(C <= 65535 && (long long)M * nsample <= 65535LL * BN_THREADS * ((nsample & 3) == 0 ? 4 : 1),
                  "bn_act_maxpool_bwd: C > 65535 or M*nsample too large");
     const int chunk = bn_chunk_bwd(C, (long long)B * M), nchunk = (int)(((long long)B * M + chunk - 1) / chunk);
-    float *coef = workspace + (size_t)2 * C * nchunk;
+    float *coef = coef_only ? coef_only : workspace + (size_t)2 * C * nchunk;
     hipStream_t st = (hipStream_t)stream;
     { KtScope kt(KT_BN_MAX_BWD_REDUCE, st, (3.0 * sizeof(T) + 1.0) * (double)B * C * M);
     if (relu) hipLaunchKernelGGL((bn_max_bwd_partial_kernel<true, T>), dim3(nchunk, C), dim3(BN_THREADS), 0, st, dpool, pooled, arg, x, xarg, B, C, M, nsample, mean, invstd, workspace, ds, chunk);
     else hipLaunchKernelGGL((bn_max_bwd_partial_kernel<false, T>), dim3(nchunk, C), dim3(BN_THREADS), 0, st, dpool, pooled, arg, x, xarg, B, C, M, nsample, mean, invstd, workspace, ds, chunk);
     }
     hipLaunchKernelGGL(bn_bwd_finalize_kernel, dim3(C), dim3(64), 0, st, workspace, nchunk, C, (double)B * M * nsample, dgamma, dbeta, coef);
+    if (coef_only) return check_launch("bn_act_maxpool_bwd_coef: launch failed");
     dim3 grid(B * C, ceil_div((long long)M * nsample, BN_THREADS * ((nsample & 3) == 0 ? 4 : 1)));
     { KtScope kt(KT_BN_MAX_BWD_APPLY, st, (double)B * C * M * (2.0 * sizeof(T) * nsample + 2.0 * sizeof(T) + 1.0));
     if (relu) hipLaunchKernelGGL((bn_max_bwd_apply_kernel<true, T>), grid, dim3(BN_THREADS), 0, st, dpool, pooled, arg, x, C, M, nsample, mean, invstd, gamma, coef, dx, ds);
@@ -886,4 +888,14 @@
     return check_launch("bn_act_bwd_apply: launch failed");
 }
 
+BN_API int mgar_bn_act_maxpool_bwd_coef(const float *dpool, long long sb, long long sc, long long sm, const float *pooled,
+                                        const unsigned char *arg, const float *x, const float *xarg, int B, int C, int M, int nsample,
+                                        const float *mean, const float *invstd, int relu, float *workspace, float *dgamma,
+                                        float *dbeta, float *coef, void *stream) {
+    MGAR_REQUIRE(sb >= 0 && sc >= 1 && sm >= 1, "bn_act_maxpool_bwd_coef: bad strides");
+    MGAR_REQUIRE(coef, "bn_act_maxpool_bwd_coef: null coef");
+    return bn_act_maxpool_bwd_impl<float>(dpool, pooled, arg, x, xarg, B, C, M, nsample, mean, invstd, nullptr, relu, workspace, dgamma,
+                                          dbeta, nullptr, stream, sb, sc, sm, coef);
+}
+
 #include "channels_last.hpp"
diff --git a/multimodal_gar_amd/csrc/errors.hip b/multimodal_gar_amd/csrc/errors.hip
--- a/multimodal_gar_amd/csrc/errors.hip
+++ b/multimodal_gar_amd/csrc/errors.hip
@@ -51,7 +51,7 @@
 
 using namespace mgar;
 
-extern "C" __attribute__((visibility("default"))) int mgar_abi_version(void) { return 12; }
+extern "C" __attribute__((visibility("default"))) int mgar_abi_version(void) { return 13; }
 extern "C" __attribute__((visibility("default"))) const char *mgar_last_error(void) { return mgar::g_last_error; }
 
 extern "C" __attribute__((visibility("default"))) int mgar_ktimer_enable(int on) {
diff --git a/multimodal_gar_amd/csrc/maxpool_grad.hpp b/multimodal_gar_amd/csrc/maxpool_grad.hpp
--- /dev/null
+++ b/multimodal_gar_amd/csrc/maxpool_grad.hpp
@@ -0,0 +1,46 @@
+#pragma once
+
+namespace mgar {
+
+struct MpGrad {
+    const float *dpool;
+    long long sb, sc, sm;
+    const float *pooled;
+    const unsigned char *arg;
+    const float *mean, *invstd, *gamma, *coef;
+    int M, ns, relu;
+};
+
+struct MpGroup {
+    float d, pooled;
+    int arg;
+};
+
+__device__ __forceinline__ MpGroup mp_load_group(const MpGrad &g, int C, int b, int c, int p) {
+    const int m = p / g.ns;
+    const size_t go = ((size_t)b * C + c) * g.M + m;
+    return MpGroup{g.dpool[(long long)b * g.sb + (long long)c * g.sc + (long long)m * g.sm], g.pooled[go], (int)g.arg[go]};
+}
+
+struct MpChan {
+    float mu, is, k, m0, m1;
+};
+
+__device__ __forceinline__ MpChan mp_chan(const MpGrad &g, int c) {
+    const float is = g.invstd[c];
+    return MpChan{g.mean[c], is, (g.gamma ? g.gamma[c] : 1.f) * is, g.coef[2 * c], g.coef[2 * c + 1]};
+}
+
+__device__ __forceinline__ float4 mp_dz4(const MpChan &q, const MpGroup &gr, float4 xv, int s0, int relu) {
+    float d = gr.d;
+    if (relu && !(gr.pooled > 0.f)) d = 0.f;
+    const int a = gr.arg;
+    float4 r;
+    r.x = q.k * ((s0 + 0 == a ? d : 0.f) - q.m0 - (xv.x - q.mu) * q.is * q.m1);
+    r.y = q.k * ((s0 + 1 == a ? d : 0.f) - q.m0 - (xv.y - q.mu) * q.is * q.m1);
+    r.z = q.k * ((s0 + 2 == a ? d : 0.f) - q.m0 - (xv.z - q.mu) * q.is * q.m1);
+    r.w = q.k * ((s0 + 3 == a ? d : 0.f) - q.m0 - (xv.w - q.mu) * q.is * q.m1);
+    return r;
+}
+
+}
diff --git a/multimodal_gar_amd/csrc/pointwise_dw.hip b/multimodal_gar_amd/csrc/pointwise_dw.hip
--- a/multimodal_gar_amd/csrc/pointwise_dw.hip
+++ b/multimodal_gar_amd/csrc/pointwise_dw.hip
@@ -1,4 +1,5 @@
 #include "common.hpp"
+#include "maxpool_grad.hpp"
 
 namespace mgar {
 
@@ -13,16 +14,26 @@
     int pair;
 };
 
-template <int OB, int IB>
+template <int OB, int IB, bool MP = false>
 __global__ __launch_bounds__(256) void pointwise_dw_kernel(const float *__restrict__ x, const float *__restrict__ dy, int B, int Cin,
-                                                           int Cout, int P, DwAct act, float *__restrict__ partial) {
+                                                           int Cout, int P, DwAct act, float *__restrict__ partial, MpGrad mp) {
     extern __shared__ float lds[];
     __shared__ float act_sc[IB * 32], act_sh[IB * 32], act_mu[IB * 32];
     __shared__ float act_is[IB * 32];
+    __shared__ float4 mp_c4[MP ? OB * 32 : 1];
+    __shared__ float mp_c1[MP ? OB * 32 : 1];
     float *sy = lds;
     float *sx = lds + OB * 32 * DW_LD;
     const int o_base = blockIdx.y * OB * 32, i_base = blockIdx.z * IB * 32;
     const bool has_act = act.mean != nullptr;
+    if (MP) {
+        for (int r = threadIdx.x; r < OB * 32; r += 256) {
+            const MpChan q = o_base + r < Cout ? mp_chan(mp, o_base + r) : MpChan{0.f, 0.f, 0.f, 0.f, 0.f};
+            mp_c4[r] = make_float4(q.mu, q.is, q.k, q.m0);
+            mp_c1[r] = q.m1;
+        }
+        __syncthreads();
+    }
     const bool pair = act.pair != 0;
     const int CinV = pair ? 2 * Cin : Cin;
     if (has_act) {
@@ -62,6 +73,8 @@
 
     constexpr int NV = (OB + IB) * 32 * (DW_TP / 4) / 256;
     float4 pre[NV];
+    constexpr int NY = 4 * OB;
+    MpGroup gpre[MP ? NY : 1];
     auto fetch = [&](long long tile) {
         const int b = (int)(tile / tiles_per_b);
         const int p0 = (int)(tile - (long long)b * tiles_per_b) * DW_TP;
@@ -73,9 +86,10 @@
             const int chv = is_y ? o_base + row : i_base + row - OB * 32;
             const int ch = (!is_y && pair && chv >= Cin) ? chv - Cin : chv;
             const int cmax = is_y ? Cout : Cin;
-            pre[u] = (chv < (is_y ? Cout : CinV) && p0 + c4 < P)
-                         ? *reinterpret_cast<const float4 *>((is_y ? dy : x) + ((size_t)b * cmax + ch) * P + p0 + c4)
-                         : make_float4(0.f, 0.f, 0.f, 0.f);
+            const bool ok = chv < (is_y ? Cout : CinV) && p0 + c4 < P;
+            pre[u] = ok ? *reinterpret_cast<const float4 *>((is_y ? dy : x) + ((size_t)b * cmax + ch) * P + p0 + c4)
+                        : make_float4(0.f, 0.f, 0.f, 0.f);
+            if (MP && u < NY) gpre[MP ? u : 0] = ok ? mp_load_group(mp, Cout, b, ch, p0 + c4) : MpGroup{0.f, 0.f, -1};
         }
     };
     if (vec && (long long)blockIdx.x < total_tiles) fetch(blockIdx.x);
@@ -91,6 +105,11 @@
                 const bool is_y = row < OB * 32;
                 const int ch = is_y ? o_base + row : i_base + row - OB * 32;
                 float4 v = pre[u];
+                if (MP && u < NY && ch < Cout && p0 + c4 < P)
+                {
+                    const float4 q4 = mp_c4[row];
+                    v = mp_dz4(MpChan{q4.x, q4.y, q4.z, q4.w, mp_c1[row]}, gpre[MP ? u : 0], v, (p0 + c4) % mp.ns, mp.relu);
+                }
                 if (has_act && !is_y && ch < CinV && p0 + c4 < P) {
                     const int r = row - OB * 32;
                     if (pair) {
@@ -232,19 +251,19 @@
     ib = Cin <= 32 ? 1 : (Cin <= 64 ? 2 : 4);
 }
 
-template <int OB, int IB>
+template <int OB, int IB, bool MP = false>
 static void launch_dw(const float *x, const float *dy, int B, int Cin, int Cout, int P, const DwAct &act, float *partial,
-                      hipStream_t st) {
+                      hipStream_t st, const MpGrad &mp = MpGrad{}) {
     static bool attr_set = false;
     const int lds = (OB + IB) * 32 * DW_LD * (int)sizeof(float);
     if (!attr_set) {
-        (void)hipFuncSetAttribute((const void *)pointwise_dw_kernel<OB, IB>, hipFuncAttributeMaxDynamicSharedMemorySize, lds);
+        (void)hipFuncSetAttribute((const void *)pointwise_dw_kernel<OB, IB, MP>, hipFuncAttributeMaxDynamicSharedMemorySize, lds);
         attr_set = true;
     }
     const int CinV = act.pair ? 2 * Cin : Cin;
     const int gy = ceil_div(Cout, OB * 32), gz = ceil_div(CinV, IB * 32);
     const int gx = dw_grid_x(B, CinV, Cout, P, OB, IB);
-    hipLaunchKernelGGL((pointwise_dw_kernel<OB, IB>), dim3((unsigned)gx, gy, gz), dim3(256), lds, st, x, dy, B, Cin, Cout, P, act, partial);
+    hipLaunchKernelGGL((pointwise_dw_kernel<OB, IB, MP>), dim3((unsigned)gx, gy, gz), dim3(256), lds, st, x, dy, B, Cin, Cout, P, act, partial, mp);
 }
 
 }
@@ -335,3 +354,36 @@
                        in_beta, dw, dgamma, dbeta, coef);
     return check_launch("pointwise_conv_dw_bnbwd: launch failed");
 }
+
+extern "C" __attribute__((visibility("default"))) int mgar_pointwise_conv_dw_act_maxpool(
+    const float *x, const float *xl, const float *dpool, long long sb, long long sc, long long sm, const float *pooled,
+    const unsigned char *arg, int nsample, const float *l_mean, const float *l_invstd, const float *l_gamma, int l_relu,
+    const float *l_coef, int B, int Cin, int Cout, int P, const float *in_mean, const float *in_invstd, const float *in_gamma,
+    const float *in_beta, int in_relu, float *workspace, float *dw, void *stream) {
+    MGAR_REQUIRE(B >= 0 && Cin >= 1 && Cout >= 1 && P >= 0, "pointwise_conv_dw_act_maxpool: bad sizes");
+    if (Cin > 64 || Cout > 64) {
+        set_error("pointwise_conv_dw_act_maxpool: Cin <= 64 and Cout <= 64");
+        return MGAR_EUNSUPPORTED;
+    }
+    MGAR_REQUIRE(nsample >= 4 && nsample % 4 == 0 && nsample <= 255 && P % nsample == 0, "pointwise_conv_dw_act_maxpool: bad nsample");
+    MGAR_REQUIRE(sb >= 0 && sc >= 1 && sm >= 1, "pointwise_conv_dw_act_maxpool: bad dpool strides");
+    MGAR_REQUIRE((long long)B * P > 0, "pointwise_conv_dw_act_maxpool: empty input");
+    MGAR_REQUIRE(x && xl && dpool && pooled && arg && l_mean && l_invstd && l_coef && workspace && dw,
+                 "pointwise_conv_dw_act_maxpool: null pointer");
+    MGAR_REQUIRE(in_mean == nullptr || in_invstd != nullptr, "pointwise_conv_dw_act_maxpool: in_mean without in_invstd");
+    hipStream_t st = (hipStream_t)stream;
+    const DwAct act{in_mean, in_invstd, in_gamma, in_beta, in_relu, 0};
+    const MpGrad mp{dpool, sb, sc, sm, pooled, arg, l_mean, l_invstd, l_gamma, l_coef, P / nsample, nsample, l_relu};
+    int ob, ib;
+    dw_blocks(Cin, Cout, ob, ib);
+    {
+    KtScope kt(KT_POINTWISE_DW, st, 4.0 * (double)B * P * (Cin + Cout), 2.0 * (double)B * P * Cin * Cout);
+    if (ob == 1 && ib == 1) launch_dw<1, 1, true>(x, xl, B, Cin, Cout, P, act, workspace, st, mp);
+    else if (ob == 1 && ib == 2) launch_dw<1, 2, true>(x, xl, B, Cin, Cout, P, act, workspace, st, mp);
+    else if (ob == 2 && ib == 1) launch_dw<2, 1, true>(x, xl, B, Cin, Cout, P, act, workspace, st, mp);
+    else launch_dw<2, 2, true>(x, xl, B, Cin, Cout, P, act, workspace, st, mp);
+    }
+    const int gx = dw_grid_x(B, Cin, Cout, P, ob, ib), n_out = Cout * Cin;
+    hipLaunchKernelGGL(pointwise_dw_reduce_kernel, dim3(ceil_div(n_out, 64)), dim3(64 * DWR_SLICES), 0, st, workspace, gx, n_out, dw);
+    return check_launch("pointwise_conv_dw_act_maxpool: launch failed");
+}
diff --git a/multimodal_gar_amd/csrc/pointwise_fwd.hip b/multimodal_gar_amd/csrc/pointwise_fwd.hip
--- a/multimodal_gar_amd/csrc/pointwise_fwd.hip
+++ b/multimodal_gar_amd/csrc/pointwise_fwd.hip
@@ -1,6 +1,7 @@
 #include <type_traits>
 
 #include "common.hpp"
+#include "maxpool_grad.hpp"
 #include "payload.hpp"
 
 namespace mgar {
@@ -20,12 +21,14 @@
     int w_rs, w_cs;
     int relu;
     float *stats;
+    MpGrad mp;
 };
 
-template <int OB, typename T, bool STATS = false>
+template <int OB, typename T, bool STATS = false, bool MP = false>
 __global__ __launch_bounds__(256, 2) void pointwise_fwd_kernel(PfArgs<T> a) {
     constexpr int PF_KC = PfSlab<OB>::KC, KS = PF_KC / 2;
     constexpr int WLD = OB == 1 ? 32 : 96;
+    constexpr int AS = MP ? 8 : 4;
     extern __shared__ float lds[];
     const int nkc = (a.Cin + PF_KC - 1) / PF_KC;
     float *wl = lds;
@@ -35,6 +38,12 @@
         wl[e] = (ch < a.Cin && o < a.Cout) ? a.w[(size_t)o * a.w_rs + (size_t)ch * a.w_cs] : 0.f;
     }
     for (int ch = threadIdx.x; ch < nkc * PF_KC; ch += 256) {
+        if (MP) {
+            const MpChan q = ch < a.Cin ? mp_chan(a.mp, ch) : MpChan{0.f, 0.f, 0.f, 0.f, 0.f};
+            float *d = act + AS * ch;
+            d[0] = q.mu; d[1] = q.is; d[2] = q.k; d[3] = q.m0; d[4] = q.m1;
+            continue;
+        }
         float sc = 1.f, sh = 0.f, mu = 0.f;
         if (a.mean && ch < a.Cin) {
             sc = a.invstd[ch] * (a.gamma ? a.gamma[ch] : 1.f);
@@ -63,7 +72,7 @@
 #pragma unroll
             for (int r = 0; r < 16; ++r) acc[ob][j][r] = 0.f;
 
-    auto issue = [&](long long s, float4 (&buf)[KS]) {
+    auto issue = [&](long long s, float4 (&buf)[KS], MpGroup (&grp)[KS]) {
         const long long t = wave_id + (s / nkc) * nwaves;
         const int kc = (int)(s % nkc);
         const int b = (int)(t / tiles_per_b);
@@ -72,17 +81,27 @@
 #pragma unroll
         for (int ks = 0; ks < KS; ++ks) {
             const int ch = kc * PF_KC + 2 * ks + h;
-            buf[ks] = (ch < a.Cin && p < a.P) ? Payload<T>::ld4(src + (size_t)2 * ks * a.P)
-                                              : make_float4(0.f, 0.f, 0.f, 0.f);
+            const bool ok = ch < a.Cin && p < a.P;
+            buf[ks] = ok ? Payload<T>::ld4(src + (size_t)2 * ks * a.P) : make_float4(0.f, 0.f, 0.f, 0.f);
+            if (MP) grp[ks] = ok ? mp_load_group(a.mp, a.Cin, b, ch, p) : MpGroup{0.f, 0.f, -1};
         }
     };
-    auto compute = [&](long long s, float4 (&buf)[KS]) {
+    auto compute = [&](long long s, float4 (&buf)[KS], MpGroup (&grp)[KS]) {
         const int kc = (int)(s % nkc);
+        const long long t = wave_id + (s / nkc) * nwaves;
+        const int b = (int)(t / tiles_per_b);
+        const int p = (int)(t - (long long)b * tiles_per_b) * PF_COLS + 4 * l;
+        const int s0 = MP ? p % a.mp.ns : 0;
 #pragma unroll
         for (int ks = 0; ks < KS; ++ks) {
             const int ch = kc * PF_KC + 2 * ks + h;
             float4 v = buf[ks];
-            if (has_act) {
+            if (MP) {
+                const float *q = act + AS * ch;
+                const MpChan c{q[0], q[1], q[2], q[3], q[4]};
+                v = mp_dz4(c, grp[ks], v, s0, a.mp.relu);
+                if (ch >= a.Cin || p >= a.P) v = make_float4(0.f, 0.f, 0.f, 0.f);
+            } else if (has_act) {
                 const float4 ac = *reinterpret_cast<const float4 *>(act + 4 * ch);
                 const float sc = ac.x, sh = ac.y, mu = ac.z;
                 v.x = (v.x - mu) * sc + sh; v.y = (v.y - mu) * sc + sh; v.z = (v.z - mu) * sc + sh; v.w = (v.w - mu) * sc + sh;
@@ -99,9 +118,6 @@
             }
         }
         if (kc == nkc - 1) {
-            const long long t = wave_id + (s / nkc) * nwaves;
-            const int b = (int)(t / tiles_per_b);
-            const int p = (int)(t - (long long)b * tiles_per_b) * PF_COLS + 4 * l;
             if (STATS) {
 #pragma unroll
                 for (int ob = 0; ob < OB; ++ob)
@@ -135,31 +151,32 @@
     };
 
     float4 buf0[KS], buf1[KS];
-    issue(0, buf0);
+    MpGroup grp0[KS], grp1[KS];
+    issue(0, buf0, grp0);
     for (long long s = 0; s < steps; s += 2) {
-        if (s + 1 < steps) issue(s + 1, buf1);
-        compute(s, buf0);
+        if (s + 1 < steps) issue(s + 1, buf1, grp1);
+        compute(s, buf0, grp0);
         if (s + 1 < steps) {
-            if (s + 2 < steps) issue(s + 2, buf0);
-            compute(s + 1, buf1);
-        }
-    }
-}
-
-template <int OB, typename T, bool STATS = false>
+            if (s + 2 < steps) issue(s + 2, buf0, grp0);
+            compute(s + 1, buf1, grp1);
+        }
+    }
+}
+
+template <int OB, typename T, bool STATS = false, bool MP = false>
 static void launch_pf(const PfArgs<T> &a, hipStream_t st) {
-    constexpr int WLD = OB == 1 ? 32 : 96, PF_KC = PfSlab<OB>::KC;
+    constexpr int WLD = OB == 1 ? 32 : 96, PF_KC = PfSlab<OB>::KC, AS = MP ? 8 : 4;
     const int nkc = (a.Cin + PF_KC - 1) / PF_KC;
-    const int lds = nkc * PF_KC * (WLD + 4) * (int)sizeof(float);
+    const int lds = nkc * PF_KC * (WLD + AS) * (int)sizeof(float);
     static int attr_lds = 0;
     if (lds > 65536 && lds > attr_lds) {
-        (void)hipFuncSetAttribute((const void *)pointwise_fwd_kernel<OB, T, STATS>, hipFuncAttributeMaxDynamicSharedMemorySize, lds);
+        (void)hipFuncSetAttribute((const void *)pointwise_fwd_kernel<OB, T, STATS, MP>, hipFuncAttributeMaxDynamicSharedMemorySize, lds);
         attr_lds = lds;
     }
     const long long ntiles = (long long)a.B * ((a.P + PF_COLS - 1) / PF_COLS);
     long long wgs = (ntiles + 3) / 4;
     if (wgs > 2048) wgs = 2048;
-    hipLaunchKernelGGL((pointwise_fwd_kernel<OB, T, STATS>), dim3((unsigned)wgs), dim3(256), lds, st, a);
+    hipLaunchKernelGGL((pointwise_fwd_kernel<OB, T, STATS, MP>), dim3((unsigned)wgs), dim3(256), lds, st, a);
 }
 
 }
@@ -214,3 +231,24 @@
     return pointwise_conv_fwd_impl<float>(x, B, Cin, P, w, w_row_stride, w_col_stride, Cout, in_mean, in_invstd, in_gamma, in_beta,
                                           in_relu, y, stream, out_stats);
 }
+
+PF_API int mgar_pointwise_conv_bwd_data_maxpool(const float *xl, const float *dpool, long long sb, long long sc, long long sm,
+                                                const float *pooled, const unsigned char *arg, int nsample, const float *l_mean,
+                                                const float *l_invstd, const float *l_gamma, int l_relu, const float *l_coef, int B,
+                                                int Cy, int P, const float *w, int Cx, float *ga, void *stream) {
+    MGAR_REQUIRE(B >= 0 && Cy >= 0 && Cx >= 0 && P >= 0, "pointwise_conv_bwd_data_maxpool: negative size");
+    if ((long long)B * P == 0 || Cx == 0) return MGAR_OK;
+    if (Cx > 32 || Cy > 256 || Cy == 0 || (P & 3) != 0) {
+        set_error("pointwise_conv_bwd_data_maxpool: needs 1 <= Cy <= 256, Cx <= 32 and P % 4 == 0");
+        return MGAR_EUNSUPPORTED;
+    }
+    MGAR_REQUIRE(nsample >= 4 && nsample % 4 == 0 && nsample <= 255 && P % nsample == 0, "pointwise_conv_bwd_data_maxpool: bad nsample");
+    MGAR_REQUIRE(sb >= 0 && sc >= 1 && sm >= 1, "pointwise_conv_bwd_data_maxpool: bad dpool strides");
+    MGAR_REQUIRE(xl && w && ga && dpool && pooled && arg && l_mean && l_invstd && l_coef, "pointwise_conv_bwd_data_maxpool: null pointer");
+    PfArgs<float> a{xl, w, nullptr, nullptr, nullptr, nullptr, ga, B, Cy, Cx, P, 1, Cx, 0, nullptr};
+    a.mp = MpGrad{dpool, sb, sc, sm, pooled, arg, l_mean, l_invstd, l_gamma, l_coef, P / nsample, nsample, l_relu};
+    hipStream_t st = (hipStream_t)stream;
+    KtScope kt(KT_POINTWISE_FWD, st, 4.0 * B * P * (Cy + Cx), 2.0 * (double)B * P * Cy * Cx);
+    launch_pf<1, float, false, true>(a, st);
+    return check_launch("pointwise_conv_bwd_data_maxpool: launch failed");
+}
diff --git a/multimodal_gar_amd/nn_utils.py b/multimodal_gar_amd/nn_utils.py
--- a/multimodal_gar_amd/nn_utils.py
+++ b/multimodal_gar_amd/nn_utils.py
@@ -86,6 +86,14 @@
                 nxt = i + (2 if relu else 1)
                 if nxt < n and _is_pointwise(layers[nxt]) and self.fuse_bn_conv:
                     feeds_bn = nxt + 1 < n and isinstance(layers[nxt + 1], _BN_TYPES) and layers[nxt + 1].training
+                    if feeds_bn and pool_last and x.dim() == 4:
+                        relu2 = nxt + 2 < n and isinstance(layers[nxt + 2], nn.ReLU)
+                        if nxt + (3 if relu2 else 2) >= n:
+                            y = bn_ops.bn_act_conv_maxpool(x, layer, relu, layers[nxt], layers[nxt + 1], relu2, rowmajor_grad=rm,
+                                                           in_stats=stats)
+                            if y is not None:
+                                x, stats, pooled = y, None, True
+                                break
                     y = bn_ops.bn_act_conv(x, layer, relu, layers[nxt], rowmajor_grad=rm, in_stats=stats, want_out_stats=feeds_bn)
                     if y is not None:
                         x, stats = y if feeds_bn else (y, None)
```

Measured after the change: 45.85 clips/sec, median of 6. 1.5% higher.
